# polarsignals/frostdb

Hardware: AMD Instinct MI355X
Metric: rows/sec filter+group-by on 1B-row Prometheus Arrow (HBM-resident); achieved HBM GB/s vs peak (higher is better)
Workload: dtype f64; 1 GPU; headline: Prometheus schema, labels.code=='200' + SUM(value) GROUP BY labels.path; total_rows=1000000000, rows_per_gpu=1000000000, records_per_gpu=40, groups=1025, parallelism=1 GPU

## Files before the change

frostdb_amd/csrc/fdb_dense.cpp:

```cpp
#include "fdb_plan.h"
#include "fdb_jit.h"

#include "fdb_context.h"
#include "fdb_launch_plan.h"
#include "fdb_plan_internal.h"

#include <optional>

namespace fdb {

struct Plan::DenseLaunch {
  Plan& P;
  const DeviceBatch* const* bs;
  std::vector<Resolved>& Rs;
  std::vector<std::vector<int>>& part_gcols;
  const std::vector<int>& live;
  const bool fixed_order;
  PhaseTimer& pt;
  const bool jit_possible;
  const int sub;
  FdbScanArgs& args(int i) { return Rs[(size_t)i].args; }

  std::optional<StageScope> stage_scope;
  LutClasses luts;
  size_t lut_lds_max = 0;

  bool slots_ok = false;
  bool interp_ok = true;
  int two_phase = 0;

  LdsPlan lds;
  FoldFuncs funcs;

  struct Narrowed { int part, k, col; bool late; const void* wide; int64_t saved; const uint8_t* validity; bool folded; };
  std::vector<Narrowed> narrowed;

  hipFunction_t jit_fn = nullptr;
  std::string shape_key;
  int jit_block = 0;
  bool slot_kernel = false;
  int per_cu = 1;
  int tile_rows = 0;

  DenseLaunch(Plan& p, const DeviceBatch* const* b, std::vector<Resolved>& rs, std::vector<std::vector<int>>& gc, const std::vector<int>& lv, bool fixed, PhaseTimer& t)
      : P(p), bs(b), Rs(rs), part_gcols(gc), live(lv), fixed_order(fixed), pt(t), jit_possible(p.jit_possible()), sub(p.sub_tiles == 4 ? 0 : p.sub_tiles) {}

  void bind_group_columns();
  void stage_luts();
  void assign_all_slots();
  void plan_lds();
  bool specialisable() const { return slots_ok && P.sub_tiles != 4 && lds.lds_bytes <= 150 * 1024; }
  void narrow_slots();
  void narrow_pool(bool late);
  void widen_slots();
  bool choose_kernel();
  bool split_by_shape();
  void launch();
  void launch_slots();
  void launch_sequential();
  unsigned long long* alloc_partials(int grid);
  void fold_partials(unsigned long long* partials, int grid);
};

void Plan::DenseLaunch::bind_group_columns() {
  for (int i : live) {
    Resolved& R = Rs[(size_t)i];
    FdbScanArgs& a = R.args;
    for (const GroupRes& gr : R.groups) {
      FdbGroupCol& G = a.gcols[a.n_gcols];
      const DevColumn& c = bs[i]->cols[(size_t)gr.ci];
      G.idx = (const uint32_t*)c.d_values;
      G.validity = c.d_validity;
      const size_t null_entry = scan_cache_folded(*bs[i], (size_t)gr.ci) && gr.lut->size() <= c.dict->values.size() ? 1 : 0;
      G.lut_len = (uint32_t)(gr.lut->size() + null_entry);
      G.lut_lds = FDB_NO_LDS;
      G.slot = -1;
      R.gcol_col[a.n_gcols] = gr.ci;
      const size_t off = R.blob.add(gr.lut->data(), gr.lut->size() * 4);
      R.blob.bytes.resize(R.blob.bytes.size() + null_entry * 4, 0);
      R.luts.push_back(PendingLut{1, a.n_gcols, off, (gr.lut->size() + null_entry) * 4});
      part_gcols[(size_t)i].push_back(gr.gi);
      a.n_gcols++;
    }
  }
  std::vector<uint32_t> caps;
  for (const GroupColState& g : P.gcols_) caps.push_back((uint32_t)g.values.size() + 1);
  P.ensure_layout(caps);
  pt.mark("layout");
}

void Plan::DenseLaunch::stage_luts() {
  for (int i : live) luts.add(Rs[(size_t)i]);
  stage_scope.emplace(P.ctx_);
  unsigned char* d_blob = luts.blob.bytes.empty() ? nullptr : (unsigned char*)P.upload(luts.blob.bytes.data(), luts.blob.bytes.size());
  size_t k = 0;
  for (int i : live) lut_lds_max = std::max(lut_lds_max, luts.place(k++, d_blob, Rs[(size_t)i]));
}

void Plan::DenseLaunch::assign_all_slots() {
  slots_ok = P.rows_per_thread == 0;
  std::vector<int> layouts;
  for (int i : live) {
    Resolved& R = Rs[(size_t)i];
    FdbScanArgs& a = R.args;
    for (int g = 0; g < a.n_gcols; g++) a.gcols[g].stride = P.gcols_[(size_t)part_gcols[(size_t)i][(size_t)g]].stride;
    for (size_t j = 0; j < P.aggs_.size(); j++) a.aggs[j].acc = P.aggs_[j].d_acc;
    a.cnt = P.d_cnt_;
    a.n_slots = P.n_slots_;
    a.need_count = 0;
    for (size_t j = 0; j < P.aggs_.size(); j++) if (a.aggs[j].func == FDB_AGG_COUNT) a.need_count = 1;
    if (slots_ok) {
      bool strict = true;
      const int layout = assign_slots(*bs[i], R, 1, jit_possible, &strict);
      if (layout == 0) slots_ok = false;
      interp_ok = interp_ok && strict;
      layouts.push_back(layout);
    }
  }
  if (!slots_ok) return;
  for (int l : layouts) if (l == 2) two_phase = 1;
  if (two_phase) {
    size_t k = 0;
    for (int i : live)
      if (layouts[k++] == 1 && assign_slots(*bs[i], Rs[(size_t)i], 2, jit_possible) != 2) throw Error(FDB_ERR_INVALID, "internal: slot re-assignment failed");
  }
}

void Plan::DenseLaunch::plan_lds() {
  const size_t acc_bytes = align_up((size_t)P.n_slots_ * 4, 16) + (size_t)P.n_slots_ * 8 * P.aggs_.size();
  lds = fdb::plan_lds(lut_lds_max, acc_bytes, P.aggs_.size(), jit_possible, slots_ok, fixed_order, P.use_partials, P.grid_override,
                      P.grid_override > 0 ? P.grid_override : fdb_scan_default_grid(P.device_));
  if (!lds.refusal.empty()) throw Error(FDB_ERR_UNSUPPORTED, lds.refusal);
  int32_t func[FDB_MAX_AGGS], type[FDB_MAX_AGGS];
  for (size_t j = 0; j < P.aggs_.size(); j++) { func[j] = args(live[0]).aggs[j].func; type[j] = P.aggs_[j].type; }
  funcs = fold_funcs(func, type, P.aggs_.size());
  for (int i : live) { args(i).lds_lut_bytes = (uint32_t)lut_lds_max; args(i).lds_acc = lds.lds_acc; args(i).cache_slots = lds.cache_slots; }
  pt.mark("lut upload");
}

void Plan::DenseLaunch::narrow_slots() {
  if (!specialisable() || !jit_possible) return;
  narrow_pool(false);
  if (two_phase) narrow_pool(true);
}
static bool validity_leaf_reads(const FdbScanArgs& a, int k) {
  for (int l = 0; l < a.n_leaves; l++)
    if (a.leaves[l].kind == FDB_LEAF_VALIDITY && !a.leaves[l].wide && a.leaves[l].slot == k) return true;
  return false;
}
void Plan::DenseLaunch::narrow_pool(bool late) {
  const FdbScanArgs& a0 = args(live[0]);
  const int n4 = late ? a0.n_l4 : a0.n_c4;
  for (int i : live) if ((late ? args(i).n_l4 : args(i).n_c4) != n4) return;
  for (int k = 0; k < n4; k++) {
    int w = 0;
    for (int i : live) {
      const Resolved& R = Rs[(size_t)i];
      const int ci = late ? R.l4_col[k] : R.c4_col[k];
      const int wi = (late ? R.args.l4[k] : R.args.c4[k]).values == nullptr || ci < 0 ? 4 : scan_cache_width(*bs[i], (size_t)ci);
      w = w == 0 || w == wi ? wi : 4;
      if (w == 4) break;
    }
    if (w >= 4) continue;
    for (int i : live) {
      Resolved& R = Rs[(size_t)i];
      const int ci = late ? R.l4_col[k] : R.c4_col[k];
      FdbColSlot& sl = late ? R.args.l4[k] : R.args.c4[k];
      bool counted = false;
      for (const Narrowed& nw : narrowed) if (nw.part == i && nw.col == ci) counted = true;
      const int64_t saved = counted ? 0 : bs[i]->rows * (int64_t)(4 - w);
      const bool fold = sl.validity != nullptr && scan_cache_folded(*bs[i], (size_t)ci) && !(!late && validity_leaf_reads(R.args, k));
      narrowed.push_back(Narrowed{i, k, ci, late, sl.values, saved, sl.validity, fold});
      sl.values = scan_cache_get(*bs[i], (size_t)ci, P.stream_);
      if (fold) sl.validity = nullptr;
      (late ? R.args.wl4 : R.args.w4)[k] = (uint8_t)w;
      R.bytes -= saved;
    }
  }
}
void Plan::DenseLaunch::widen_slots() {
  for (const Narrowed& nw : narrowed) {
    Resolved& R = Rs[(size_t)nw.part];
    (nw.late ? R.args.l4 : R.args.c4)[nw.k].values = nw.wide;
    (nw.late ? R.args.l4 : R.args.c4)[nw.k].validity = nw.validity;
    (nw.late ? R.args.wl4 : R.args.w4)[nw.k] = 0;
    R.bytes += nw.saved;
  }
  narrowed.clear();
}

bool Plan::DenseLaunch::choose_kernel() {
  jit_block = fixed_order ? 256 : sub == 1 ? 512 : sub == 2 ? 256 : sub == 3 ? 1024 : 0;
  if (specialisable()) {
    JitShape shape;
    bool same = true, first = true;
    const FdbScanArgs& args0 = args(live[0]);
    for (int i : live) {
      if (first) { shape = jit_shape(args0, two_phase != 0, jit_block ? jit_block : 256); first = false; }
      else if (!jit_shape_merge_args(&shape, args0, args(i), two_phase != 0)) { same = false; break; }
    }
    if (!same && live.size() > 1 && jit_possible && split_by_shape()) return false;
    {
      int regs_per_slot = 2;
      for (const AggState& A : P.aggs_) if (A.func != FDB_AGG_COUNT || P.final_stage_) regs_per_slot += 2;
      if (P.n_slots_ >= 1 && P.n_slots_ <= 8 && (int)P.n_slots_ * regs_per_slot <= 48) shape.reg_slots = (int)P.n_slots_;
    }
    shape.wave_tables = fixed_order;
    shape.uniform_fold = !P.knobs_.no_uniform_fold;
    if (same) {
      JitDeferScope defer(interp_ok && !fixed_order);
      if (jit_block != 0) { jit_fn = jit_get(shape); if (jit_fn != nullptr) per_cu = jit_blocks_per_cu(jit_fn, jit_block, lds.lds_bytes); }
      else jit_fn = jit_select(shape, lds.lds_bytes, shape.row_bytes(), P.ordered_, &jit_block, &per_cu);
      if (jit_fn != nullptr) tile_rows = jit_block * (shape.quad ? 16 : 4);
      if (pt.on && jit_fn != nullptr) shape_key = shape.key(true);
    }
  }
  if (slots_ok && jit_fn == nullptr) widen_slots();
  slot_kernel = slots_ok && (jit_fn != nullptr || interp_ok);
  if (fixed_order && jit_fn == nullptr) throw Error(FDB_ERR_UNSUPPORTED, "deterministic float sums need the run-time specialised dense kernel (records of one shape, hiprtc available)");
  pt.mark("kernel select");
  if (slot_kernel && jit_fn == nullptr) fdb_slot_geometry(two_phase, sub, lds.lds_acc, lds.lds_bytes, P.device_, &tile_rows, &per_cu);
  return true;
}

bool Plan::DenseLaunch::split_by_shape() {
  std::vector<std::string> keys;
  std::vector<std::vector<const DeviceBatch*>> groups;
  for (int i : live) {
    const std::string k = jit_shape(args(i), two_phase != 0, 256).key(false);
    size_t g = 0;
    for (; g < keys.size(); g++) if (keys[g] == k) break;
    if (g == keys.size()) { keys.push_back(k); groups.emplace_back(); }
    groups[g].push_back(bs[i]);
  }
  if (groups.size() <= 1) return false;
  P.ctx_->defer_staging(false);
  for (auto& g : groups) P.push_batches(g.data(), (int)g.size());
  return true;
}

unsigned long long* Plan::DenseLaunch::alloc_partials(int grid) {
  if (!lds.lds_acc || !P.use_partials || grid <= 0) return nullptr;
  void* p = P.ctx_->dev_alloc((size_t)grid * (1 + P.aggs_.size()) * P.n_slots_ * 8);
  P.scratch_.push_back(p);
  return (unsigned long long*)p;
}

void Plan::DenseLaunch::fold_partials(unsigned long long* partials, int grid) {
  if (partials == nullptr) return;
  unsigned long long* host_out = P.mirror_target();
  hip_check(fdb_launch_reduce_partials(partials, grid, (int)(1 + P.aggs_.size()), P.n_slots_, P.d_state_, P.slots_alloc_, funcs.f, host_out, P.stream_), "reduce partials");
  P.mirror_valid_ = host_out != nullptr;
}

void Plan::DenseLaunch::launch() {
  if (slot_kernel) launch_slots(); else launch_sequential();
  pt.mark("reduce launch");
}

void Plan::DenseLaunch::launch_slots() {
  int grid = P.grid_override > 0 ? P.grid_override : (fdb_scan_default_grid(P.device_) / 2) * per_cu;
  std::vector<FdbScanArgs> parts;
  parts.reserve(live.size());
  for (int i : live) parts.push_back(args(i));
  const int64_t total_tiles = assign_tiles(parts.data(), parts.size(), tile_rows);
  if (grid > total_tiles) grid = (int)total_tiles;
  unsigned long long* partials = alloc_partials(grid);
  for (FdbScanArgs& a : parts) a.partials = partials;
  bool fill_rides = false;
  if (P.state_virgin_ && jit_fn != nullptr && partials != nullptr && (uint64_t)P.slots_alloc_ * (1 + P.aggs_.size()) < (1ull << 32)) {
    FdbScanArgs& a0 = parts[0];
    a0.fill_state = P.d_state_;
    a0.fill_words = (uint32_t)(P.slots_alloc_ * (1 + P.aggs_.size()));
    a0.fill_alloc = (uint32_t)P.slots_alloc_;
    P.state_idents(a0.fill_idents);
    fill_rides = true;
  } else {
    P.materialize_state();
  }
  P.trace("before scan");
  pt.mark("parts build");
  const FdbScanArgs* d_parts = (const FdbScanArgs*)P.upload(parts.data(), parts.size() * sizeof(FdbScanArgs));
  P.ctx_->flush_staging();
  pt.mark("parts upload");
  P.trace("after upload");
  if (pt.on) {
    std::vector<uint32_t> folded(parts.size(), 0u);
    for (const Narrowed& nw : narrowed)
      if (nw.folded) folded[(size_t)(std::find(live.begin(), live.end(), nw.part) - live.begin())] |= 1u << ((nw.late ? 16 : 0) + nw.k);
    print_dense_launch(jit_fn != nullptr ? "fdb_plan_kernel" : "scan_slots_kernel", shape_key, parts.data(), parts.size(), total_tiles, grid, jit_fn != nullptr ? jit_block : 0, lds.lds_bytes,
                       two_phase, lds.lds_acc, lds.cache_slots, lut_lds_max, per_cu, tile_rows, fill_rides, partials != nullptr, folded);
  }
  P.timed([&] {
    if (jit_fn != nullptr) hip_check(jit_launch(jit_fn, d_parts, (int)parts.size(), total_tiles, parts[0], grid, jit_block, lds.lds_bytes, P.stream_), "scan launch");
    else hip_check(fdb_launch_scan_slots(d_parts, (int)parts.size(), parts[0], total_tiles, grid, lds.lds_bytes, two_phase, sub, P.stream_), "scan launch");
  });
  if (fill_rides) P.state_virgin_ = false;
  P.last_kernel_ = jit_fn != nullptr ? "fdb_plan_kernel" : "scan_slots_kernel";
  pt.mark("scan launch");
  P.trace("after scan");
  fold_partials(partials, grid);
  P.trace("after reduce");
  P.stat_launches += 1;
}

void Plan::DenseLaunch::launch_sequential() {
  const int rpt = P.rows_per_thread == 8 ? 8 : 4;
  P.materialize_state();
  P.ctx_->flush_staging();
  for (int i : live) {
    FdbScanArgs& a = args(i);
    if (a.n_expr > 0) throw Error(FDB_ERR_UNSUPPORTED, "computed (projected) columns are not supported by the sequential kernel (too many referenced columns)");
    a.n_c4 = a.n_c8 = 0;
    const int grid = fdb_scan_grid(a, lds.base_grid, rpt);
    a.partials = alloc_partials(grid);
    if (pt.on) print_dense_launch("scan_dense_kernel", "", &a, 1, 0, grid, 0, lds.lds_bytes, 0, lds.lds_acc, lds.cache_slots, lut_lds_max, 0, rpt, false, a.partials != nullptr);
    P.timed([&] { hip_check(fdb_launch_scan_dense(a, grid, lds.lds_bytes, rpt, P.stream_), "scan launch"); });
    P.last_kernel_ = "scan_dense_kernel";
    P.mirror_valid_ = false;
    fold_partials(a.partials, grid);
    P.stat_launches += 1;
  }
}

bool Plan::push_dense(const DeviceBatch* const* bs, std::vector<Resolved>& Rs, std::vector<std::vector<int>>& part_gcols, const std::vector<int>& live, bool fixed_order,
                      PhaseTimer& pt) {
  DenseLaunch D(*this, bs, Rs, part_gcols, live, fixed_order, pt);
  D.bind_group_columns();
  D.stage_luts();
  D.assign_all_slots();
  D.plan_lds();
  D.narrow_slots();
  if (!D.choose_kernel()) return false;
  D.launch();
  return true;
}

}
```

frostdb_amd/csrc/fdb_jit.cpp:

```cpp
#include <hip/hip_runtime_api.h>
#include <hip/hiprtc.h>
#include <sys/stat.h>
#include <unistd.h>

#include <algorithm>
#include <chrono>
#include <atomic>
#include <cstdio>
#include <cstdlib>
#include <cstring>
#include <fstream>
#include <condition_variable>
#include <functional>
#include <memory>
#include <mutex>
#include <thread>
#include <sstream>
#include <string>
#include <unordered_map>
#include <vector>

#include "fdb_jit.h"
#include "../../include/frostdb_amd.h"

// ... 115 lines not shown
    if (!compiled) {
      std::fprintf(stderr, "[frostdb_amd] %s specialisation failed, using the interpreting kernel: %s\n", kernel_name, log.c_str());
      if (std::getenv("FDB_JIT_DEBUG")) std::fprintf(stderr, "%s\n", src.c_str());
      return nullptr;
    }
    if (!path.empty()) {
      const std::string tmp = path + "." + std::to_string((long)getpid());
      bool ok = false;
      {
        std::ofstream f(tmp, std::ios::binary);
        if (f) { f.write(code.data(), (std::streamsize)code.size()); f.close(); ok = !f.fail(); }
      }
      if (!ok || ::rename(tmp.c_str(), path.c_str()) != 0) (void)::unlink(tmp.c_str());
    }
  }
  if (fn == nullptr && !load(&fn)) {
    std::fprintf(stderr, "[frostdb_amd] could not load a specialised %s, using the interpreting kernel\n", kernel_name);
    fn = nullptr;
  }
  publish.fn = fn;
  return fn;
}

thread_local bool t_may_defer = false;
struct Builders {
  struct Slot { std::thread t; std::shared_ptr<std::atomic<bool>> done; };
  std::mutex m;
  std::vector<Slot> slots;
  void spawn(std::function<void()> job) {
    std::lock_guard<std::mutex> lk(m);
    for (size_t k = 0; k < slots.size();) {
      if (slots[k].done->load(std::memory_order_acquire)) { slots[k].t.join(); slots[k] = std::move(slots.back()); slots.pop_back(); }
      else k++;
    }
    auto done = std::make_shared<std::atomic<bool>>(false);
    slots.push_back(Slot{std::thread([job = std::move(job), done] { job(); done->store(true, std::memory_order_release); }), done});
  }
  ~Builders() { for (Slot& s : slots) if (s.t.joinable()) s.t.join(); }
} g_builders;

template <typename F>
hipFunction_t get_kernel(const std::string& key, const char* kernel_name, F make_source) {
  if (g_disabled || std::getenv("FDB_NO_JIT") != nullptr) return nullptr;
  int dev = 0;
  (void)hipGetDevice(&dev);
  const std::string ckey = std::to_string(dev) + "|" + kernel_name + "|" + key;
  std::shared_ptr<KernelEntry> entry;
  bool builder = false;
  {
    std::lock_guard<std::mutex> lk(g_mu);
    auto it = g_cache.find(ckey);
    if (it == g_cache.end()) { entry = std::make_shared<KernelEntry>(); g_cache.emplace(ckey, entry); builder = true; }
    else entry = it->second;
  }
  const char* as = t_may_defer ? std::getenv("FDB_JIT_ASYNC") : nullptr;
  const bool defer = as != nullptr && std::atoi(as) != 0;
  if (!builder) {
    std::unique_lock<std::mutex> lk(entry->m);
    if (defer && !entry->ready) return nullptr;
    entry->cv.wait(lk, [&] { return entry->ready; });
    return entry->fn;
  }
  std::string src;
  try { src = make_source(); }
  catch (...) { { std::lock_guard<std::mutex> lk(entry->m); entry->ready = true; } entry->cv.notify_all(); throw; }
  if (defer) {
    const std::string kn = kernel_name;
    g_builders.spawn([entry, kn, src, dev] { (void)hipSetDevice(dev); (void)build_kernel(entry.get(), kn, src); });
    return nullptr;
  }
  return build_kernel(entry.get(), kernel_name, src);
}
}

hipFunction_t jit_select_kernel_get(const JitShape& shape) {
  return get_kernel("select|" + shape.key() + "|f" + std::to_string(shape.fuse4) + "," + std::to_string(shape.fuse8), "fdb_select_kernel", [&] { return jit_select_source(shape); });
}
hipError_t jit_select_launch(hipFunction_t fn, const FdbScanArgs* d_parts, int n_parts, int64_t total_super_tiles, const FdbScanArgs& common, int grid, size_t lds_bytes,
                             uint32_t* masks, uint32_t* offsets, const FdbSelectArgs& sel, hipStream_t stream) {
  long long tt = total_super_tiles;
  void* args[] = {(void*)&d_parts, (void*)&n_parts, (void*)&tt, (void*)&common, (void*)&masks, (void*)&offsets, (void*)&sel};
  return hipModuleLaunchKernel(fn, (unsigned)grid, 1, 1, (unsigned)jit_select_block(), 1, 1, (unsigned)lds_bytes, stream, args, nullptr);
}

hipFunction_t jit_flags_get(const JitShape& shape) {
  return get_kernel("flags|" + shape.key(), "fdb_flags_kernel", [&] { return jit_flags_source(shape); });
}

hipError_t jit_flags_launch(hipFunction_t fn, const FdbScanArgs* d_parts, int n_parts, int64_t total_super_tiles, const FdbScanArgs& common, int grid, size_t lds_bytes,
                            uint32_t* masks, uint32_t* tile_counts, hipStream_t stream) {
  long long tt = total_super_tiles;
  void* args[] = {(void*)&d_parts, (void*)&n_parts, (void*)&tt, (void*)&common, (void*)&masks, (void*)&tile_counts};
  return hipModuleLaunchKernel(fn, (unsigned)grid, 1, 1, 256u, 1, 1, (unsigned)lds_bytes, stream, args, nullptr);
}

hipFunction_t jit_project_get(const JitShape& shape) {
  std::string roots;
  for (int r : shape.proj_roots) roots += std::to_string(r) + ",";
  return get_kernel("project|" + shape.key() + "|r" + roots, "fdb_project_kernel", [&] { return jit_project_source(shape); });
}
hipError_t jit_project_launch(hipFunction_t fn, const FdbScanArgs* d_parts, int n_parts, int64_t total_tiles, int grid, size_t lds_bytes, const FdbProjectPart* d_outs,
                              unsigned long long* d_nulls, hipStream_t stream) {
  long long tt = total_tiles;
  void* args[] = {(void*)&d_parts, (void*)&n_parts, (void*)&tt, (void*)&d_outs, (void*)&d_nulls};
  return hipModuleLaunchKernel(fn, (unsigned)grid, 1, 1, 256u, 1, 1, (unsigned)lds_bytes, stream, args, nullptr);
}

void jit_stats(int64_t* n_compiled, double* compile_ms, int64_t* n_disk_loads) {
  if (n_compiled) *n_compiled = g_stat_compiled.load();
  if (compile_ms) *compile_ms = (double)g_stat_compile_us.load() / 1000.0;
  if (n_disk_loads) *n_disk_loads = g_stat_disk_loads.load();
}

JitDeferScope::JitDeferScope(bool may_defer) : prev_(t_may_defer) { t_may_defer = may_defer; }
JitDeferScope::~JitDeferScope() { t_may_defer = prev_; }

hipFunction_t jit_get(const JitShape& shape) {
  return get_kernel(shape.key(), "fdb_plan_kernel", [&] { return jit_source(shape); });
}

hipFunction_t jit_hash_get(const JitHashShape& shape) {
  return get_kernel(shape.key(), "fdb_hash_kernel", [&] { return jit_hash_source(shape); });
}

hipError_t jit_hash_launch(hipFunction_t fn, const FdbHashArgs& args, int grid, size_t lds_bytes, hipStream_t stream) {
  void* kargs[] = {(void*)&args};
  return hipModuleLaunchKernel(fn, (unsigned)grid, 1, 1, 256, 1, 1, (unsigned)lds_bytes, stream, kargs, nullptr);
}

hipFunction_t jit_select(JitShape shape, size_t lds_bytes, int row_bytes, bool sorted_input, int* block_out, int* blocks_per_cu_out) {
  int waves = row_bytes > 0 ? (65536 / (64 * 4)) / row_bytes : 16;
  waves = std::max(8, std::min(32, waves));
  if (shape.quad) waves = std::max(8, std::min(16, row_bytes > 0 ? (sorted_input ? 144 : 96) / row_bytes : 8));
  const int block = shape.quad ? 256 : waves % 8 == 0 ? 512 : 256;
  shape.block = block;
  hipFunction_t fn = jit_get(shape);
  if (fn == nullptr) return nullptr;
  const int fit = jit_blocks_per_cu(fn, block, lds_bytes);
  *block_out = block;
  *blocks_per_cu_out = std::max(1, std::min(fit, (waves + block / 128) / (block / 64)));
  if (std::getenv("FDB_JIT_DEBUG"))
    std::fprintf(stderr, "[frostdb_amd] plan kernel %s: %d B/row, %zu B LDS -> %d-thread workgroups, %d per CU (%d fit)\n", shape.key().c_str(), row_bytes,
                 lds_bytes, block, *blocks_per_cu_out, fit);
  return fn;
}

hipError_t jit_launch(hipFunction_t fn, const FdbScanArgs* d_parts, int n_parts, int64_t total_tiles, const FdbScanArgs& common, int grid, int block,
                      size_t lds_bytes, hipStream_t stream) {
  long long tt = total_tiles;
  void* args[] = {(void*)&d_parts, (void*)&n_parts, (void*)&tt, (void*)&common};
  return hipModuleLaunchKernel(fn, (unsigned)grid, 1, 1, (unsigned)block, 1, 1, (unsigned)lds_bytes, stream, args, nullptr);
}

}
```

frostdb_amd/csrc/fdb_jit.h:

```cpp
#pragma once
#include <cstdlib>

#include <hip/hip_runtime_api.h>

#include <cstdint>
#include <string>
#include <vector>

#include "fdb_kernels.h"

namespace fdb {

struct JitSlot { bool has_values = false; int has_validity = 0; int width = 4; };
struct JitLeaf { int kind = 0, slot = -1, wide = 0, op = 0; bool lut_in_lds = false; };
struct JitGroup { int slot = -1; bool lut_in_lds = false; };
struct JitAgg { int func = 0, type = 0, slot = -1; int expr = 0; };
struct JitExprNode { int kind = 0, op = 0, left = -1, right = -1, slot = -1, type = 0; };

struct JitShape {
  int block = 512;
  bool lds_acc = true, need_count = false, two_phase = false;
  int n_c4 = 0, n_c8 = 0, n_l4 = 0, n_l8 = 0;
  JitSlot c4[FDB_ARG_C4], c8[FDB_ARG_C8], l4[FDB_ARG_L4], l8[FDB_ARG_L8];
  std::vector<JitLeaf> leaves;
  std::vector<uint8_t> code;
  std::vector<JitGroup> gcols;
  std::vector<JitAgg> aggs;
  std::vector<JitExprNode> exprs;
  int reg_slots = 0;
  bool cache = false;
  bool wave_tables = false;
  bool uniform_fold = true;
  bool quad = false;
  int fuse4 = 0, fuse8 = 0;
  std::vector<int> proj_roots;
  std::string key(bool with_validity = true) const;
  int row_bytes() const {
    int b = 0;
    for (int k = 0; k < n_c4; k++) b += c4[k].has_values ? c4[k].width : 0;
    for (int k = 0; k < n_l4; k++) b += l4[k].has_values ? l4[k].width : 0;
    for (int k = 0; k < n_c8; k++) b += c8[k].has_values ? 8 : 0;
    for (int k = 0; k < n_l8; k++) b += l8[k].has_values ? 8 : 0;
    return b;
  }
};

struct JitHashCol { int kind = 0; bool has_validity = false, lut_in_lds = false; int expr_root = -1; bool lut_identity = false; };
struct JitHashShape {
  std::vector<JitHashCol> cols;
  std::vector<JitLeaf> leaves;
  std::vector<bool> leaf_validity;
  std::vector<uint8_t> code;
  std::vector<JitAgg> aggs;
  std::vector<bool> agg_validity;
  std::vector<JitExprNode> exprs;
  int n_expr_cols = 0;
  bool need_count = true;
  int runs = 0;
  bool exact = false;
  std::string key() const;
};
JitHashShape jit_hash_shape(const FdbHashArgs& args, const FdbHashCol* hcols);
std::string jit_hash_source(const JitHashShape& shape);
hipFunction_t jit_hash_get(const JitHashShape& shape);
hipError_t jit_hash_launch(hipFunction_t fn, const FdbHashArgs& args, int grid, size_t lds_bytes, hipStream_t stream);

JitShape jit_shape(const FdbScanArgs& a, bool two_phase, int block);
bool jit_shape_merge(JitShape* into, const JitShape& other);
bool jit_shape_merge_args(JitShape* into, const FdbScanArgs& a, const FdbScanArgs& b, bool two_phase);
int jit_blocks_per_cu(hipFunction_t fn, int block, size_t lds_bytes);

void jit_stats(int64_t* n_compiled, double* compile_ms, int64_t* n_disk_loads);

std::string jit_flags_source(const JitShape& shape);
hipFunction_t jit_flags_get(const JitShape& shape);
hipError_t jit_flags_launch(hipFunction_t fn, const FdbScanArgs* d_parts, int n_parts, int64_t total_super_tiles, const FdbScanArgs& common, int grid, size_t lds_bytes,
                            uint32_t* masks, uint32_t* tile_counts, hipStream_t stream);

std::string jit_select_source(const JitShape& shape);
hipFunction_t jit_select_kernel_get(const JitShape& shape);
size_t jit_select_stage_bytes(const JitShape& shape);
int jit_select_block();
hipError_t jit_select_launch(hipFunction_t fn, const FdbScanArgs* d_parts, int n_parts, int64_t total_super_tiles, const FdbScanArgs& common, int grid, size_t lds_bytes,
                             uint32_t* masks, uint32_t* offsets, const FdbSelectArgs& sel, hipStream_t stream);

std::string jit_project_source(const JitShape& shape);
hipFunction_t jit_project_get(const JitShape& shape);
hipError_t jit_project_launch(hipFunction_t fn, const FdbScanArgs* d_parts, int n_parts, int64_t total_tiles, int grid, size_t lds_bytes, const FdbProjectPart* d_outs,
                              unsigned long long* d_nulls, hipStream_t stream);

std::string jit_source(const JitShape& shape);
class JitDeferScope {
 public:
  explicit JitDeferScope(bool may_defer);
  ~JitDeferScope();
  JitDeferScope(const JitDeferScope&) = delete;
  JitDeferScope& operator=(const JitDeferScope&) = delete;
 private:
  bool prev_;
};
hipFunction_t jit_get(const JitShape& shape);
hipFunction_t jit_select(JitShape shape, size_t lds_bytes, int row_bytes, bool sorted_input, int* block_out, int* blocks_per_cu_out);
hipError_t jit_launch(hipFunction_t fn, const FdbScanArgs* d_parts, int n_parts, int64_t total_tiles, const FdbScanArgs& common, int grid, int block,
                      size_t lds_bytes, hipStream_t stream);

}
```

frostdb_amd/csrc/fdb_jitgen.cpp:

```cpp
#include <algorithm>
#include <cstring>
#include <functional>
#include <sstream>
#include <string>
#include <vector>

#include "fdb_jit.h"
#include "../../include/frostdb_amd.h"

namespace fdb {

namespace {

const char* kPreamble = R"HIP(
typedef uint32_t u32x4 __attribute__((ext_vector_type(4)));
typedef unsigned long long u64x2 __attribute__((ext_vector_type(2)));
typedef uint32_t u32x2 __attribute__((ext_vector_type(2)));
#define G1 __attribute__((address_space(1)))
template <typename T> __device__ __forceinline__ const G1 T* as_global(const T* p) { return (const G1 T*)p; }
__device__ __forceinline__ long long f64_to_ordered(double d) { long long b = __double_as_longlong(d); return b ^ ((b >> 63) & 0x7FFFFFFFFFFFFFFFLL); }
// (a NaN contributes the identity of MIN / MAX, −0.0 counts as +0.0: see f64_minmax_key in fdb_kernels.hip)
__device__ __forceinline__ long long f64_minmax_key(double d, bool is_min) {
  d += 0.0;
  const long long k = f64_to_ordered(d);
  return d != d ? (is_min ? 0x7FFFFFFFFFFFFFFFLL : (-0x7FFFFFFFFFFFFFFFLL - 1)) : k;
}
// (FDB_LD_TEMPORAL: the kernel reads its columns twice — wide run records — so the first pass must leave them in the L2)
#ifdef FDB_LD_TEMPORAL
__device__ __forceinline__ u32x4 ld4(const void* base, uint32_t byte_off) {
  return *as_global(reinterpret_cast<const u32x4*>(reinterpret_cast<const char*>(base) + byte_off));
}
__device__ __forceinline__ u64x2 ld8(const void* base, uint32_t byte_off) {
  return *as_global(reinterpret_cast<const u64x2*>(reinterpret_cast<const char*>(base) + byte_off));
}
// (narrow-index caches, fdb_record.h: a lane's four indices at 1 / 2 bytes each — one 4- / 8-byte load, contiguous across the wave)
__device__ __forceinline__ uint32_t ld1raw(const void* base, uint32_t byte_off) {
  return *as_global(reinterpret_cast<const uint32_t*>(reinterpret_cast<const char*>(base) + byte_off));
}
__device__ __forceinline__ u32x2 ld2raw(const void* base, uint32_t byte_off) {
  return *as_global(reinterpret_cast<const u32x2*>(reinterpret_cast<const char*>(base) + byte_off));
}
#else
__device__ __forceinline__ uint32_t ld1raw(const void* base, uint32_t byte_off) {
  return __builtin_nontemporal_load(as_global(reinterpret_cast<const uint32_t*>(reinterpret_cast<const char*>(base) + byte_off)));
}
__device__ __forceinline__ u32x2 ld2raw(const void* base, uint32_t byte_off) {
  return __builtin_nontemporal_load(as_global(reinterpret_cast<const u32x2*>(reinterpret_cast<const char*>(base) + byte_off)));
}
__device__ __forceinline__ u32x4 ld4(const void* base, uint32_t byte_off) {
  return __builtin_nontemporal_load(as_global(reinterpret_cast<const u32x4*>(reinterpret_cast<const char*>(base) + byte_off)));
}
__device__ __forceinline__ u64x2 ld8(const void* base, uint32_t byte_off) {
  return __builtin_nontemporal_load(as_global(reinterpret_cast<const u64x2*>(reinterpret_cast<const char*>(base) + byte_off)));
}
#endif
// … unpacked into the register form the rest of the kernel consumes
__device__ __forceinline__ u32x4 ld1x4(const void* base, uint32_t byte_off) {
  const uint32_t v = ld1raw(base, byte_off);
  u32x4 r; r.x = v & 0xFFu; r.y = (v >> 8) & 0xFFu; r.z = (v >> 16) & 0xFFu; r.w = v >> 24;
  return r;
}
__device__ __forceinline__ u32x4 ld2x4(const void* base, uint32_t byte_off) {
  const u32x2 v = ld2raw(base, byte_off);
  u32x4 r; r.x = v.x & 0xFFFFu; r.y = v.x >> 16; r.z = v.y & 0xFFFFu; r.w = v.y >> 16;
  return r;
}
__device__ __forceinline__ uint32_t ldv(const uint8_t* bm, uint32_t byte_off, uint32_t shift) { return (as_global(bm)[byte_off] >> shift) & 0xFu; }
// dictionary truth table in a 64-bit immediate: 4 rows → 4-bit mask (NULL rows look up entry `null_at`)
__device__ __forceinline__ uint32_t leaf_bits(u32x4 idx, uint32_t valid, unsigned long long bits, uint32_t null_at) {
  const uint32_t i0 = (valid & 1u) ? idx.x : null_at, i1 = (valid & 2u) ? idx.y : null_at, i2 = (valid & 4u) ? idx.z : null_at, i3 = (valid & 8u) ? idx.w : null_at;
  return (uint32_t)((bits >> i0) & 1ull) | ((uint32_t)((bits >> i1) & 1ull) << 1) | ((uint32_t)((bits >> i2) & 1ull) << 2) | ((uint32_t)((bits >> i3) & 1ull) << 3);
}
template <typename LUT>
__device__ __forceinline__ uint32_t leaf_lut(u32x4 idx, uint32_t valid, LUT lut, uint32_t null_at) {
  const uint32_t i0 = (valid & 1u) ? idx.x : null_at, i1 = (valid & 2u) ? idx.y : null_at, i2 = (valid & 4u) ? idx.z : null_at, i3 = (valid & 8u) ? idx.w : null_at;
  return (uint32_t)lut[i0] | ((uint32_t)lut[i1] << 1) | ((uint32_t)lut[i2] << 2) | ((uint32_t)lut[i3] << 3);
}
// pre-aggregate arithmetic (project.go:163-399): Go int64 semantics — wrap-around, quotient truncated toward zero,
// MinInt64 / -1 wraps; a division by zero yields NULL, whose raw slot reads 0.
__device__ __forceinline__ long long i64_add(long long a, long long b) { return (long long)((unsigned long long)a + (unsigned long long)b); }
__device__ __forceinline__ long long i64_sub(long long a, long long b) { return (long long)((unsigned long long)a - (unsigned long long)b); }
__device__ __forceinline__ long long i64_mul(long long a, long long b) { return (long long)((unsigned long long)a * (unsigned long long)b); }
__device__ __forceinline__ long long i64_div(long long a, long long b) { return b == 0 ? 0 : b == -1 ? (long long)(0ull - (unsigned long long)a) : a / b; }
__device__ __forceinline__ long long u64_div(long long a, long long b) { return b == 0 ? 0 : (long long)((unsigned long long)a / (unsigned long long)b); }  // DivUint64s (project.go:379-395)
__device__ __forceinline__ double f64_div(double a, double b) { return b == 0.0 ? 0.0 : a / b; }
template <int OP, typename T> __device__ __forceinline__ bool cmp1(T a, T b) {
  return OP == 1 ? a == b : OP == 2 ? a != b : OP == 3 ? a < b : OP == 4 ? a <= b : OP == 5 ? a > b : a >= b;
}
template <int OP, typename T> __device__ __forceinline__ uint32_t cmp4(T a, T b, T c, T d, T lit, uint32_t valid) {
  return ((uint32_t)cmp1<OP, T>(a, lit) | ((uint32_t)cmp1<OP, T>(b, lit) << 1) | ((uint32_t)cmp1<OP, T>(c, lit) << 2) | ((uint32_t)cmp1<OP, T>(d, lit) << 3)) & valid;
}
)HIP";

const char* kQuadPreamble = R"HIP(
__device__ __forceinline__ u32x4 ldblock(const void* base, uint32_t byte_off) {
#ifdef FDB_LD_TEMPORAL
  return *as_global(reinterpret_cast<const u32x4*>(reinterpret_cast<const char*>(base) + byte_off));
#else
  return __builtin_nontemporal_load(as_global(reinterpret_cast<const u32x4*>(reinterpret_cast<const char*>(base) + byte_off)));
#endif
}
__device__ __forceinline__ uint32_t dword_of(u32x4 q, int k) { return k == 0 ? q.x : k == 1 ? q.y : k == 2 ? q.z : q.w; }
__device__ __forceinline__ u32x4 idx1x4(uint32_t v) {
  u32x4 r; r.x = v & 0xFFu; r.y = (v >> 8) & 0xFFu; r.z = (v >> 16) & 0xFFu; r.w = v >> 24;
  return r;
}
__device__ __forceinline__ u32x4 idx2x4(uint32_t lo, uint32_t hi) {
  u32x4 r; r.x = lo & 0xFFFFu; r.y = lo >> 16; r.z = hi & 0xFFFFu; r.w = hi >> 16;
  return r;
}
)HIP";

template <typename F, typename V>
std::string expr_valid(const std::vector<JitExprNode>& ex, int root, F col, V colvalid);
template <typename F, typename V>
std::string expr_value(const std::vector<JitExprNode>& ex, int ni, F col, V colvalid) {
  const JitExprNode& n = ex[(size_t)ni];
  const bool f = n.type == FDB_T_F64;
  if (n.kind == 0) return f ? ("__longlong_as_double((long long)" + col(ni) + ")") : ("(long long)" + col(ni));
  if (n.kind == 1) return f ? ("__longlong_as_double(K_elit" + std::to_string(ni) + ")") : ("K_elit" + std::to_string(ni));
  if (n.kind == 7) return "(long long)" + col(ni);
  if (n.kind == 4) return "(double)(" + expr_value(ex, n.left, col, colvalid) + ")";
  if (n.kind == 5) return "(" + colvalid(n.left) + " ? 0ll : 1ll)";
  if (n.kind == 6)
    return "((" + expr_value(ex, n.op, col, colvalid) + " != 0ll) ? " + expr_value(ex, n.left, col, colvalid) + " : " + expr_value(ex, n.right, col, colvalid) + ")";
  std::string a = expr_value(ex, n.left, col, colvalid), b = expr_value(ex, n.right, col, colvalid);
  if (n.kind == 3) {
    if (n.op == FDB_OP_AND || n.op == FDB_OP_OR) return "((" + a + (n.op == FDB_OP_AND ? " & " : " | ") + b + ") & 1ll)";
    if (ex[(size_t)n.left].type != ex[(size_t)n.right].type) { a = "(double)" + a; b = "(double)" + b; }
    const char* op = n.op == FDB_OP_EQ ? " == " : n.op == FDB_OP_NOT_EQ ? " != " : n.op == FDB_OP_LT ? " < " : n.op == FDB_OP_LT_EQ ? " <= " : n.op == FDB_OP_GT ? " > " : " >= ";
    return "((" + expr_valid(ex, n.left, col, colvalid) + " && " + expr_valid(ex, n.right, col, colvalid) + " && (" + a + op + b + ")) ? 1ll : 0ll)";
  }
  if (f) {
    if (n.op == FDB_OP_DIV) return "f64_div(" + a + ", " + b + ")";
    return "(" + a + (n.op == FDB_OP_ADD ? " + " : n.op == FDB_OP_SUB ? " - " : " * ") + b + ")";
  }
  return std::string(n.op == FDB_OP_ADD ? "i64_add(" : n.op == FDB_OP_SUB ? "i64_sub(" : n.op == FDB_OP_MUL ? "i64_mul(" : n.type == FDB_T_U64 ? "u64_div(" : "i64_div(") + a + ", " + b + ")";
}
template <typename F, typename V>
std::string expr_valid(const std::vector<JitExprNode>& ex, int root, F col, V colvalid) {
  const JitExprNode& n = ex[(size_t)root];
  if (n.kind == 0) return colvalid(root);
  if (n.kind == 2 && n.op == FDB_OP_DIV) {
    const std::string d = expr_value(ex, n.right, col, colvalid);
    return n.type == FDB_T_F64 ? ("(" + d + " != 0.0)") : ("(" + d + " != 0)");
  }
  return "true";
}
inline std::string expr_bits(const std::vector<JitExprNode>& ex, int root, const std::string& v) {
  if (ex[(size_t)root].type == FDB_T_BOOL) return "(unsigned long long)(" + v + " + 1ll)";
  return ex[(size_t)root].type == FDB_T_F64 ? ("(unsigned long long)__double_as_longlong(" + v + ")") : ("(unsigned long long)" + v);
}

inline std::string comp8(const std::string& r, int k) { return r + (k < 2 ? "a" : "b") + (k % 2 == 0 ? ".x" : ".y"); }

struct RowRefs {
  const std::vector<JitExprNode>& ex;
  int k;
  std::function<std::string(int)> reg8;
  std::string col(int ni) const {
    const JitExprNode& n = ex[(size_t)ni];
    return n.kind == 7 ? "((PM" + std::to_string(n.slot) + " >> " + std::to_string(k) + ") & 1u)" : comp8(reg8(n.slot), k);
  }
  std::string colvalid(int ni) const { return "((" + reg8(ex[(size_t)ni].slot) + "_m >> " + std::to_string(k) + ") & 1u)"; }
  std::string bits(int root) const {
    return expr_bits(ex, root, expr_value(ex, root, [&](int ni) { return col(ni); }, [&](int ni) { return colvalid(ni); }));
  }
  std::string valid(int root) const { return expr_valid(ex, root, [&](int ni) { return col(ni); }, [&](int ni) { return colvalid(ni); }); }
  std::string raw(int root) const { return "(" + valid(root) + " ? " + bits(root) + " : 0ull)"; }
};

struct AggCode {
  const bool sum, f64, is_min;
  explicit AggCode(const JitAgg& A) : sum(A.func == FDB_AGG_SUM), f64(A.type == FDB_T_F64), is_min(A.func == FDB_AGG_MIN) {}
  bool sum_f64() const { return sum && f64; }
  const char* ctype() const { return sum_f64() ? "double" : sum ? "unsigned long long" : "long long"; }
  const char* ident() const { return sum_f64() ? "0.0" : sum ? "0ull" : is_min ? "0x7FFFFFFFFFFFFFFFLL" : "(-0x7FFFFFFFFFFFFFFFLL - 1)"; }
  const char* ident_word() const { return sum ? "0ull" : is_min ? "0x7FFFFFFFFFFFFFFFull" : "0x8000000000000000ull"; }
  std::string from_word(const std::string& w) const { return sum_f64() ? "__longlong_as_double((long long)" + w + ")" : sum ? w : "(long long)" + w; }
  std::string to_word(const std::string& v) const { return sum_f64() ? "(unsigned long long)__double_as_longlong(" + v + ")" : sum ? v : "(unsigned long long)" + v; }
  std::string typed(const std::string& raw) const {
    return !sum && f64 ? "f64_minmax_key(__longlong_as_double((long long)" + raw + "), " + (is_min ? "true" : "false") + ")" : from_word(raw);
  }
  std::string fold(const std::string& acc, const std::string& y) const {
    return sum ? acc + " += " + y + ";" : acc + " = " + y + (is_min ? " < " : " > ") + acc + " ? " + y + " : " + acc + ";";
  }
  std::string fold_of(const std::string& acc, const std::string& y) const { return sum ? fold(acc, y) : "{ const long long y = " + y + "; " + fold(acc, "y") + " }"; }
  std::string fold_if(const std::string& acc, const std::string& on, const std::string& y) const {
    return sum ? acc + " += " + on + " ? " + y + " : " + ident() + ";" : acc + " = (" + on + " && " + y + (is_min ? " < " : " > ") + acc + ") ? " + y + " : " + acc + ";";
  }
  std::string shuffle_fold(const std::string& v) const {
    return fold_of(v, sum && !f64 ? "(unsigned long long)__shfl_xor((long long)" + v + ", sh, 64)" : "__shfl_xor(" + v + ", sh, 64)");
  }
  std::string atomic(const std::string& where, const std::string& v) const {
    return sum_f64() ? "atomicAdd(reinterpret_cast<double*>" + where + ", " + v + ");" : sum ? "atomicAdd(" + where + ", " + v + ");"
                     : std::string(is_min ? "atomicMin" : "atomicMax") + "(reinterpret_cast<long long*>" + where + ", " + v + ");";
  }
};

struct Gen {
  std::ostringstream o;
  const JitShape& s;
  explicit Gen(const JitShape& sh) : s(sh) {}

  static std::string reg(bool wide, bool late, int slot) { return std::string(late ? "l" : "e") + (wide ? "8_" : "4_") + std::to_string(slot); }

  bool full_block = false;
  void block_loads() {
    auto narrow = [&](const JitSlot& c, const std::string& r) {
      if (!c.has_values || c.width >= 4) return;
      if (c.width == 1) o << "      const u32x4 Q_" << r << " = ldblock(P_" << r << "_v + (size_t)wb, lane * 16u);\n";
      else o << "      const u32x4 Q_" << r << "a = ldblock(P_" << r << "_v + (size_t)wb * 2, lane * 16u), Q_" << r << "b = ldblock(P_" << r << "_v + (size_t)wb * 2 + 1024, lane * 16u);\n";
    };
    for (int i = 0; i < s.n_c4; i++) narrow(s.c4[i], reg(false, false, i));
    for (int i = 0; i < s.n_l4; i++) narrow(s.l4[i], reg(false, true, i));
    for (int i = 0; i < s.n_c4; i++) {
      const std::string r = reg(false, false, i);
      if (s.c4[i].has_values && s.c4[i].width >= 4) o << "      u32x4 A_" << r << "[4];\n";
      if (s.c4[i].has_validity != 0) o << "      uint32_t M_" << r << "[4];\n";
    }
    for (int i = 0; i < s.n_c8; i++) {
      const std::string r = reg(true, false, i);
      if (s.c8[i].has_values) o << "      u64x2 A_" << r << "a[4], A_" << r << "b[4];\n";
      if (s.c8[i].has_validity != 0) o << "      uint32_t M_" << r << "[4];\n";
    }
    o << "#pragma unroll\n      for (int u = 0; u < 4; u++) {\n        const size_t o0 = (size_t)(wb + 256 * u); (void)o0;\n";
    auto valid = [&](const JitSlot& c, const std::string& r) {
      if (c.has_validity == 1) o << "        M_" << r << "[u] = ldv(P_" << r << "_b + (o0 >> 3), lane_offb, lane_shb);\n";
      else if (c.has_validity == 2) o << "        M_" << r << "[u] = P_" << r << "_b != nullptr ? ldv(P_" << r << "_b + (o0 >> 3), lane_offb, lane_shb) : 0xFu;\n";
    };
    for (int i = 0; i < s.n_c4; i++) {
      const std::string r = reg(false, false, i);
      if (s.c4[i].has_values && s.c4[i].width >= 4) o << "        A_" << r << "[u] = ld4(P_" << r << "_v + o0 * 4, lane_off4);\n";
      valid(s.c4[i], r);
    }
    for (int i = 0; i < s.n_c8; i++) {
      const std::string r = reg(true, false, i);
      if (s.c8[i].has_values) o << "        A_" << r << "a[u] = ld8(P_" << r << "_v + o0 * 8, lane_off8);\n        A_" << r << "b[u] = ld8(P_" << r << "_v + o0 * 8, lane_off8 + 16u);\n";
      valid(s.c8[i], r);
    }
    o << "      }\n";
    std::string keep;
    auto use = [&](const std::string& v) { keep += (keep.empty() ? "\"v\"(" : ", \"v\"(") + v + ")"; };
    for (int i = 0; i < s.n_c4; i++) {
      const std::string r = reg(false, false, i);
      if (s.c4[i].has_values && s.c4[i].width >= 4) use("A_" + r + "[0]");
      if (s.c4[i].has_validity != 0) use("M_" + r + "[0]");
    }
    for (int i = 0; i < s.n_c8; i++) {
      const std::string r = reg(true, false, i);
      if (s.c8[i].has_values) { use("A_" + r + "a[0]"); use("A_" + r + "b[0]"); }
      if (s.c8[i].has_validity != 0) use("M_" + r + "[0]");
    }
    if (!keep.empty()) o << "      asm volatile(\"\" :: " << keep << ");\n";
  }

  void loads(bool late) {
    const int n4 = late ? s.n_l4 : s.n_c4, n8 = late ? s.n_l8 : s.n_c8;
    for (int i = 0; i < n4; i++) {
      const JitSlot& c = late ? s.l4[i] : s.c4[i];
      const std::string r = reg(false, late, i);
      if (full_block && c.has_values && c.width == 1) o << "    const u32x4 " << r << " = idx1x4(dword_of(Q_" << r << ", u));\n";
      else if (full_block && c.has_values && c.width == 2)
        o << "    const u32x4 " << r << " = idx2x4(dword_of(u < 2 ? Q_" << r << "a : Q_" << r << "b, 2 * (u & 1)), dword_of(u < 2 ? Q_" << r << "a : Q_" << r << "b, 2 * (u & 1) + 1));\n";
      else if (full_block && !late && c.has_values) o << "    const u32x4 " << r << " = A_" << r << "[u];\n";
      else if (c.has_values && c.width == 1) o << "    const u32x4 " << r << " = ld1x4(P_" << r << "_v + tile_off1, lane_off1);\n";
      else if (c.has_values && c.width == 2) o << "    const u32x4 " << r << " = ld2x4(P_" << r << "_v + tile_off2, lane_off2);\n";
      else if (c.has_values) o << "    const u32x4 " << r << " = ld4(P_" << r << "_v + tile_off4, lane_off4);\n";
      mask(c, r, late);
    }
    for (int i = 0; i < n8; i++) {
      const JitSlot& c = late ? s.l8[i] : s.c8[i];
      const std::string r = reg(true, late, i);
      if (full_block && !late && c.has_values) {
        o << "    const u64x2 " << r << "a = A_" << r << "a[u], " << r << "b = A_" << r << "b[u];\n";
      } else if (c.has_values) {
        o << "    const u64x2 " << r << "a = ld8(P_" << r << "_v + tile_off8, lane_off8);\n";
        o << "    const u64x2 " << r << "b = ld8(P_" << r << "_v + tile_off8, lane_off8 + 16u);\n";
      }
      mask(c, r, late);
    }
  }

  bool live_mask = false;
  void mask(const JitSlot& c, const std::string& r, bool late = false) {
    if (full_block && !late && c.has_validity != 0) { o << "    const uint32_t " << r << "_m = M_" << r << "[u];\n"; return; }
    const char* all = live_mask ? "live" : "0xFu";
    const char* cut = live_mask ? " & live" : "";
    if (c.has_validity == 1) o << "    const uint32_t " << r << "_m = ldv(P_" << r << "_b + tile_offb, lane_offb, lane_shb)" << cut << ";\n";
    else if (c.has_validity == 2) o << "    const uint32_t " << r << "_m = P_" << r << "_b != nullptr ? ldv(P_" << r << "_b + tile_offb, lane_offb, lane_shb)" << cut << " : " << all << ";\n";
    else o << "    const uint32_t " << r << "_m = " << all << ";\n";
  }

  std::string leaf_expr(int l) { return leaf_expr_of(s.leaves[l], l, reg(s.leaves[l].wide, false, s.leaves[l].slot)); }

  static std::string leaf_expr_of(const JitLeaf& L, int l, const std::string& r) {
    const std::string li = std::to_string(l);
    std::ostringstream e;
    switch (L.kind) {
      case FDB_LEAF_CONST: e << "(K_op" << li << " ? 0xFu : 0u)"; break;
      case FDB_LEAF_VALIDITY: e << "(K_op" << li << " ? " << r << "_m : (~" << r << "_m & 0xFu))"; break;
      case FDB_LEAF_DICT_BITS: e << "leaf_bits(" << r << ", " << r << "_m, (unsigned long long)K_lit" << li << ", K_len" << li << " - 1u)"; break;
      case FDB_LEAF_DICT_LUT:
        if (L.lut_in_lds) e << "leaf_lut(" << r << ", " << r << "_m, smem + K_lds" << li << ", K_len" << li << " - 1u)";
        else e << "leaf_lut(" << r << ", " << r << "_m, as_global(K_lut" << li << "), K_len" << li << " - 1u)";
        break;
      case FDB_LEAF_CMP_I64:
        e << "cmp4<" << L.op << ", long long>((long long)" << r << "a.x, (long long)" << r << "a.y, (long long)" << r << "b.x, (long long)" << r << "b.y, K_lit" << li << ", " << r << "_m)";
        break;
      case FDB_LEAF_CMP_U64:
        e << "cmp4<" << L.op << ", unsigned long long>(" << r << "a.x, " << r << "a.y, " << r << "b.x, " << r << "b.y, (unsigned long long)K_lit" << li << ", " << r << "_m)";
        break;
      case FDB_LEAF_CMP_F64:
        e << "cmp4<" << L.op << ", double>(__longlong_as_double((long long)" << r << "a.x), __longlong_as_double((long long)" << r << "a.y), __longlong_as_double((long long)"
          << r << "b.x), __longlong_as_double((long long)" << r << "b.y), __longlong_as_double(K_lit" << li << "), " << r << "_m)";
        break;
      case FDB_LEAF_CMP_I64_F64:
        e << "cmp4<" << L.op << ", double>((double)(long long)" << r << "a.x, (double)(long long)" << r << "a.y, (double)(long long)" << r << "b.x, (double)(long long)" << r
          << "b.y, __longlong_as_double(K_lit" << li << "), " << r << "_m)";
        break;
    }
    return e.str();
  }

  std::string filter_expr() {
    return filter_expr_of(s.code, [&](int l) { return leaf_expr(l); });
  }
  template <typename F>
  static std::string filter_expr_of(const std::vector<uint8_t>& code, F leaf) {
    std::vector<std::string> st;
    for (uint8_t c : code) {
      if (c < 0x80) { st.push_back(leaf(c)); continue; }
      const std::string b = st.back(); st.pop_back();
      const std::string a = st.back(); st.pop_back();
      st.push_back("(" + a + (c == FDB_CODE_AND ? " & " : " | ") + b + ")");
    }
    return st.empty() ? "0xFu" : st.back();
  }

  RowRefs row(int k, bool late) const { return {s.exprs, k, [late](int slot) { return reg(true, late, slot); }}; }
  template <typename F> void each_agg(F f) const {
    for (size_t j = 0; j < s.aggs.size(); j++) if (s.aggs[j].func != FDB_AGG_COUNT) f(j, AggCode(s.aggs[j]));
  }

  template <typename R>
  static void match_bits(std::ostringstream& o, const std::vector<JitExprNode>& exprs, const std::vector<JitLeaf>& leaves, R leaf_reg) {
    std::vector<int> seen;
    for (const JitExprNode& e : exprs)
      if (e.kind == 7 && std::find(seen.begin(), seen.end(), e.slot) == seen.end()) {
        seen.push_back(e.slot);
        o << "    const uint32_t PM" << e.slot << " = " << leaf_expr_of(leaves[(size_t)e.slot], e.slot, leaf_reg(e.slot)) << "; (void)PM" << e.slot << ";\n";
      }
  }

  struct Entry {
    bool late_pools;
    const char* var;
    int block;
    bool out_tile;
  };
  template <typename F> void each_slot(const Entry& e, F f) const {
    for (bool late : {false, true}) {
      if (late && !e.late_pools) break;
      const int n4 = late ? s.n_l4 : s.n_c4, n8 = late ? s.n_l8 : s.n_c8;
      for (int i = 0; i < n4; i++) f(reg(false, late, i), late ? "l4" : "c4", i);
      for (int i = 0; i < n8; i++) f(reg(true, late, i), late ? "l8" : "c8", i);
    }
  }
  void entry_decls(const Entry& e, const std::function<void()>& more = nullptr) {
    each_slot(e, [&](const std::string& r, const char*, int) { o << "  const char* P_" << r << "_v = nullptr; const uint8_t* P_" << r << "_b = nullptr;\n"; });
    for (size_t l = 0; l < s.leaves.size(); l++)
      o << "  long long K_lit" << l << " = 0; uint32_t K_len" << l << " = 1, K_lds" << l << " = 0; int K_op" << l << " = 0; const uint8_t* K_lut" << l << " = nullptr;\n";
    if (more) more();
    o << "  long long n_rows = 0, tile_begin = 0, tile_end = 0" << (e.out_tile ? ", out_tile = 0" : "") << "; int part = -1, lut_class = -1;\n";
  }
  void enter_record(const Entry& e, const std::function<void()>& per_record = nullptr, const std::function<void()>& luts = nullptr, const std::string& leaving = "") {
    o << "    if (part < 0 || " << e.var << " >= tile_end) {\n" << leaving;
    o << "      int np = part < 0 ? 0 : part;\n      while (np + 1 < n_parts && " << e.var << " >= parts[np].tile_end) np++;\n      part = np;\n";
    o << "      const FdbScanArgs& pa = parts[part];\n      n_rows = pa.n_rows; tile_begin = pa.tile_begin; tile_end = pa.tile_end;" << (e.out_tile ? " out_tile = pa.out_tile_base;" : "") << "\n";
    each_slot(e, [&](const std::string& r, const char* pool, int i) {
      o << "      P_" << r << "_v = (const char*)pa." << pool << "[" << i << "].values; P_" << r << "_b = pa." << pool << "[" << i << "].validity;\n";
    });
    for (size_t l = 0; l < s.leaves.size(); l++)
      o << "      K_lit" << l << " = pa.leaves[" << l << "].lit; K_len" << l << " = pa.leaves[" << l << "].lut_len; K_lds" << l << " = pa.leaves[" << l << "].lut_lds; K_op" << l
        << " = pa.leaves[" << l << "].op; K_lut" << l << " = pa.leaves[" << l << "].lut;\n";
    if (per_record) per_record();
    o << "      if (pa.lut_class != lut_class) {\n        lut_class = pa.lut_class;\n        __syncthreads();\n";
    for (size_t l = 0; l < s.leaves.size(); l++)
      if (s.leaves[l].kind == FDB_LEAF_DICT_LUT && s.leaves[l].lut_in_lds)
        o << "        for (uint32_t i = tid; i < K_len" << l << "; i += " << e.block << ") smem[K_lds" << l << " + i] = as_global(K_lut" << l << ")[i];\n";
    if (luts) luts();
    o << "        __syncthreads();\n      }\n    }\n";
  }

  std::string source() {
    const int BLK = s.block;
    const Entry entry{true, "tile", BLK, false};
    o << "#include \"fdb_kernels.h\"\n" << kPreamble;
    if (s.quad) o << kQuadPreamble;
    o << "extern \"C\" __global__ __launch_bounds__(" << BLK << ") void fdb_plan_kernel(const FdbScanArgs* __restrict__ parts, const int n_parts, const long long total_tiles, const FdbScanArgs c) {\n";
    o << "  extern __shared__ __align__(16) unsigned char smem[];\n  const uint32_t tid = threadIdx.x;\n  const uint32_t n_slots = c.n_slots;\n";
    o << "  if (c.fill_state != nullptr)  // (a fresh table: its identity fill rides on this launch, see FdbScanArgs)\n";
    o << "    for (uint32_t i = blockIdx.x * " << BLK << "u + tid; i < c.fill_words; i += gridDim.x * " << BLK << "u) c.fill_state[i] = c.fill_idents[i / c.fill_alloc];\n";
    table_setup();
    entry_decls(entry, [&] {
      for (size_t g = 0; g < s.gcols.size(); g++) o << "  uint32_t G_lds" << g << " = 0, G_stride" << g << " = 0; const uint32_t* G_lut" << g << " = nullptr;\n";
      for (size_t i = 0; i < s.exprs.size(); i++) if (s.exprs[i].kind == 1) o << "  long long K_elit" << i << " = 0;\n";
      for (int t = 0; t < s.reg_slots; t++) {
        o << "  unsigned long long R_cnt" << t << " = 0ull;\n";
        each_agg([&](size_t j, const AggCode& A) { o << "  " << A.ctype() << " R_a" << j << "_" << t << " = " << A.ident() << ";\n"; });
      }
    });
    if (s.quad) {
      o << "  const uint32_t lane = tid & 63u, wave = (uint32_t)__builtin_amdgcn_readfirstlane((int)(tid >> 6));\n";
      o << "  const uint32_t lane_off4 = lane * 16u, lane_off8 = lane * 32u, lane_offb = lane >> 1, lane_shb = (lane & 1u) * 4u; (void)lane_off4;\n";
      o << "  const uint32_t lane_off1 = lane * 4u, lane_off2 = lane * 8u; (void)lane_off1; (void)lane_off2;\n";
    } else {
      o << "  const uint32_t lane_off4 = tid * 16u, lane_off8 = tid * 32u, lane_offb = tid >> 1, lane_shb = (tid & 1u) * 4u;\n";
      o << "  const uint32_t lane_off1 = tid * 4u, lane_off2 = tid * 8u; (void)lane_off1; (void)lane_off2;\n";
    }
    o << "  for (long long tile = blockIdx.x; tile < total_tiles; tile += gridDim.x) {\n";
    enter_record(entry, [&] {
      for (size_t g = 0; g < s.gcols.size(); g++)
        o << "      G_lds" << g << " = pa.gcols[" << g << "].lut_lds; G_stride" << g << " = pa.gcols[" << g << "].stride; G_lut" << g << " = pa.gcols[" << g << "].lut;\n";
      for (size_t i = 0; i < s.exprs.size(); i++) if (s.exprs[i].kind == 1) o << "      K_elit" << i << " = pa.expr[" << i << "].lit;\n";
    }, [&] {
      for (size_t g = 0; g < s.gcols.size(); g++)
        if (s.gcols[g].lut_in_lds)
          o << "        for (uint32_t i = tid; i < pa.gcols[" << g << "].lut_len; i += " << BLK << ") reinterpret_cast<uint32_t*>(smem + G_lds" << g << ")[i] = as_global(G_lut" << g << ")[i];\n";
    });
    if (!s.quad) {
      tile_header("(tile - tile_begin) * " + std::to_string(BLK * 4) + "LL", "tid");
      live_mask = true;
      tile_body();
    } else {
      o << "    const long long wb = (tile - tile_begin) * " << BLK * 16 << "LL + (long long)wave * 1024;\n";
      o << "    if (wb + 1024 <= n_rows) {\n";
      full_block = true; live_mask = false;
      block_loads();
      o << "#pragma unroll\n      for (int u = 0; u < 4; u++) {\n";
      tile_header("wb + 256 * u", nullptr);
      tile_body();
      o << "      }\n    } else {\n";
      full_block = false; live_mask = true;
      o << "#pragma unroll 1\n      for (int u = 0; u < 4; u++) {\n";
      tile_header("wb + 256 * u", "lane");
      tile_body();
      o << "      }\n    }\n";
    }
    o << "  }\n";
    if (s.reg_slots > 0) wave_reduction();
    if (s.cache) cache_flush();
    if (s.lds_acc) lds_flush();
    o << "}\n";
    return o.str();
  }

  void table_setup() {
    o << "  const size_t TB = (((size_t)n_slots * 4 + 15) & ~(size_t)15) + (size_t)n_slots * 8 * (size_t)c.n_aggs;\n  (void)TB;\n";
    const std::string tbl = s.wave_tables ? "smem + c.lds_lut_bytes + (size_t)(tid >> 6) * TB" : "smem + c.lds_lut_bytes";
    o << "  uint32_t* l_cnt = reinterpret_cast<uint32_t*>(" << tbl << ");\n";
    o << "  unsigned long long* l_acc = reinterpret_cast<unsigned long long*>(" << tbl << " + (((size_t)n_slots * 4 + 15) & ~(size_t)15));\n";
    if (s.lds_acc) {
      const std::string i0 = s.wave_tables ? "(tid & 63u)" : "tid", step = s.wave_tables ? "64" : std::to_string(s.block);
      o << "  for (uint32_t i = " << i0 << "; i < n_slots; i += " << step << ") l_cnt[i] = 0;\n";
      each_agg([&](size_t j, const AggCode& A) {
        o << "  for (uint32_t i = " << i0 << "; i < n_slots; i += " << step << ") l_acc[(size_t)" << j << " * n_slots + i] = " << A.ident_word() << ";\n";
      });
    }
    if (s.cache) {
      o << "  const uint32_t CS = (uint32_t)c.cache_slots;\n";
      o << "  uint32_t* t_tag = reinterpret_cast<uint32_t*>(smem + c.lds_lut_bytes);\n  uint32_t* t_cnt = t_tag + CS;\n";
      o << "  unsigned long long* t_acc = reinterpret_cast<unsigned long long*>(t_cnt + CS);\n";
      o << "  for (uint32_t i = tid; i < CS; i += " << s.block << ") { t_tag[i] = 0u; t_cnt[i] = 0u; }\n";
      each_agg([&](size_t j, const AggCode& A) { o << "  for (uint32_t i = tid; i < CS; i += " << s.block << ") t_acc[(size_t)" << j << " * CS + i] = " << A.ident_word() << ";\n"; });
    }
  }

  void tile_header(const std::string& r0, const char* lane) {
    o << "    const long long r0 = " << r0 << ";\n";
    if (lane) o << "    const long long left = n_rows - r0 - (long long)" << lane << " * 4;\n    if (left <= 0) continue;\n";
    o << "    const size_t tile_off4 = (size_t)r0 * 4, tile_off8 = (size_t)r0 * 8, tile_offb = (size_t)(r0 >> 3);" << (lane ? "" : " (void)tile_off4; (void)tile_off8; (void)tile_offb;") << "\n";
    o << "    const size_t tile_off1 = (size_t)r0, tile_off2 = (size_t)r0 * 2; (void)tile_off1; (void)tile_off2;\n";
    o << "    const uint32_t live = " << (lane ? "left >= 4 ? 0xFu : ((1u << (int)left) - 1u)" : "0xFu") << ";\n";
  }

  std::string raw_input(size_t j, int k) const {
    const JitAgg& A = s.aggs[j];
    if (A.expr != 0) return row(k, s.two_phase).raw(A.expr - 1);
    const std::string r = reg(true, s.two_phase, A.slot);
    return "((" + r + "_m >> " + std::to_string(k) + ") & 1u ? " + comp8(r, k) + " : c.aggs[" + std::to_string(j) + "].null_value)";
  }

  bool uniform_fold() const { return s.uniform_fold && s.lds_acc && !s.cache && s.reg_slots == 0 && !s.wave_tables && !s.two_phase && !s.gcols.empty(); }

  void tile_body() {
    loads(false);
    o << "    uint32_t sel = live;\n";
    if (!s.code.empty()) o << "    sel &= " << filter_expr() << ";\n";
    match_bits(o, s.exprs, s.leaves, [&](int l) { return reg(s.leaves[(size_t)l].wide, false, s.leaves[(size_t)l].slot); });
    if (uniform_fold()) o << "    const unsigned long long has = __ballot(sel != 0u);\n    if (has == 0ull) continue;\n";
    else o << "    if (sel == 0u) continue;\n";
    loads(true);
    o << "    uint32_t gid0 = 0, gid1 = 0, gid2 = 0, gid3 = 0;\n";
    for (size_t g = 0; g < s.gcols.size(); g++) {
      const JitGroup& G = s.gcols[g];
      const std::string r = reg(false, s.two_phase, G.slot);
      const std::string lut = G.lut_in_lds ? ("reinterpret_cast<const uint32_t*>(smem + G_lds" + std::to_string(g) + ")") : ("as_global(G_lut" + std::to_string(g) + ")");
      const char* comp[4] = {"x", "y", "z", "w"};
      for (int k = 0; k < 4; k++)
        o << "    gid" << k << " += ((" << r << "_m >> " << k << ") & 1u ? " << lut << "[" << r << "." << comp[k] << "] : 0u) * G_stride" << g << ";\n";
    }
    if (uniform_fold()) fold_uniform();
    if (s.reg_slots > 0) fold_registers();
    else fold_rows();
  }

  void fold_uniform() {
    o << "    {\n      const uint32_t my_first = (sel & 1u) ? gid0 : (sel & 2u) ? gid1 : (sel & 4u) ? gid2 : gid3;\n";
    o << "      const uint32_t g0 = (uint32_t)__builtin_amdgcn_readlane((int)my_first, __builtin_ctzll(has));\n";
    o << "      if (__ballot(sel != 0u && my_first != g0) == 0ull && __ballot(1) == ~0ull &&\n";
    o << "          __ballot(((sel & 1u) && gid0 != g0) || ((sel & 2u) && gid1 != g0) || ((sel & 4u) && gid2 != g0) || ((sel & 8u) && gid3 != g0)) == 0ull) {\n";
    o << "        uint32_t u_cnt = (uint32_t)__builtin_popcount(sel);\n";
    each_agg([&](size_t j, const AggCode& A) {
      const std::string v = "u" + std::to_string(j);
      o << "        " << A.ctype() << " " << v << " = " << A.ident() << ";\n";
      for (int k = 0; k < 4; k++) o << "        if ((sel >> " << k << ") & 1u) " << A.fold_of(v, A.typed(raw_input(j, k))) << "\n";
    });
    o << "#pragma unroll\n        for (int sh = 32; sh > 0; sh >>= 1) {\n          u_cnt += (uint32_t)__shfl_xor((int)u_cnt, sh, 64);\n";
    each_agg([&](size_t j, const AggCode& A) { o << "          " << A.shuffle_fold("u" + std::to_string(j)) << "\n"; });
    o << "        }\n        if ((tid & 63u) == 0u) {\n";
    if (s.need_count) o << "          atomicAdd(&l_cnt[g0], u_cnt);\n";
    else o << "          l_cnt[g0] = 1u;\n";
    each_agg([&](size_t j, const AggCode& A) { o << "          " << A.atomic("(l_acc + (size_t)" + std::to_string(j) + " * n_slots + g0)", "u" + std::to_string(j)) << "\n"; });
    o << "        }\n        continue;\n      }\n    }\n";
  }

  void fold_registers() {
    for (int k = 0; k < 4; k++) {
      o << "    {\n      const bool on = (sel >> " << k << ") & 1u;\n";
      each_agg([&](size_t j, const AggCode& A) { o << "      const " << A.ctype() << " v" << j << " = " << A.typed(raw_input(j, k)) << ";\n"; });
      for (int t = 0; t < s.reg_slots; t++) {
        const std::string m = s.reg_slots == 1 ? std::string("on") : ("(on && gid" + std::to_string(k) + " == " + std::to_string(t) + "u)");
        o << "      R_cnt" << t << " += " << m << " ? 1ull : 0ull;\n";
        each_agg([&](size_t j, const AggCode& A) { o << "      " << A.fold_if("R_a" + std::to_string(j) + "_" + std::to_string(t), m, "v" + std::to_string(j)) << "\n"; });
      }
      o << "    }\n";
    }
  }

  void fold_rows() {
    for (int k = 0; k < 4; k++) {
      const std::string gidk = "gid" + std::to_string(k);
      o << "    if ((sel >> " << k << ") & 1u) {\n";
      if (s.cache) {
        o << "      const uint32_t ch = ((gid" << k << " * 0x9E3779B1u) >> 12) & (CS - 1u);\n";
        o << "      uint32_t tg = t_tag[ch];\n      if (tg == 0u) { tg = atomicCAS(&t_tag[ch], 0u, gid" << k << " + 1u); if (tg == 0u) tg = gid" << k << " + 1u; }\n";
        o << "      const bool cached = tg == gid" << k << " + 1u;\n";
        o << "      if (cached) atomicAdd(&t_cnt[ch], 1u);\n";
        if (s.need_count) o << "      else atomicAdd(&c.cnt[gid" << k << "], 1ull);\n";
        else o << "      else c.cnt[gid" << k << "] = 1ull;\n";
      } else if (s.lds_acc) {
        if (s.need_count) o << "      atomicAdd(&l_cnt[" << gidk << "], 1u);\n";
        else o << "      l_cnt[" << gidk << "] = 1u;\n";
      } else {
        o << "      atomicAdd(&c.cnt[gid" << k << "], 1ull);\n";
      }
      each_agg([&](size_t j, const AggCode& A) {
        const std::string v = A.typed(raw_input(j, k));
        const std::string gacc = "(c.aggs[" + std::to_string(j) + "].acc + gid" + std::to_string(k) + ")";
        if (s.cache) {
          o << "      if (cached) {\n        " << A.atomic("(t_acc + (size_t)" + std::to_string(j) + " * CS + ch)", v) << "\n      } else {\n        " << A.atomic(gacc, v) << "\n      }\n";
        } else {
          o << "      " << A.atomic(s.lds_acc ? "(l_acc + (size_t)" + std::to_string(j) + " * n_slots + " + gidk + ")" : gacc, v) << "\n";
        }
      });
      o << "    }\n";
    }
  }

  void wave_reduction() {
    o << "  for (int sh = 32; sh > 0; sh >>= 1) {\n";
// ... 559 lines not shown
      o << "        }\n";
      for (size_t c = c0; c < c1; c++) {
        const JitHashCol& C = s.cols[c];
        const std::string r = "w" + std::to_string(c);
        o << "        " << (in_quad[c] ? "if (!canon) " : "") << "{\n          const int W = hc[" << c << "].word;\n";
        if (C.kind == 0) {
          for (int k = 0; k < 4; k++) o << "          if (ins_mask & " << (1 << k) << "u) d_" << k << "[W] = i" << c << "_" << k << ";\n";
        } else if (C.kind == 1) {
          for (int k = 0; k < 4; k++)
            o << "          if (ins_mask & " << (1 << k) << "u) { const unsigned long long y = ((" << r << "_m >> " << k << ") & 1u) ? " << comp8(r, k) << " : 0ull; d_" << k << "[W] = (uint32_t)y; d_" << k
              << "[W + 1] = (uint32_t)(y >> 32); }\n";
        } else {
          for (int k = 0; k < 4; k++)
            o << "          if (ins_mask & " << (1 << k) << "u) { const unsigned long long y = " << row(k).valid(C.expr_root) << " ? " << row(k).bits(C.expr_root) << " : 0ull; d_" << k << "[W] = (uint32_t)y; d_" << k
              << "[W + 1] = (uint32_t)(y >> 32); }\n";
        }
        o << "        }\n";
      }
      o << "        asm volatile(\"\" ::: \"memory\");\n      }\n";
    }
    if (for_runs) {
      int used = 4;
      for (size_t c = 0; c < s.cols.size(); c++) used += s.cols[c].kind == 0 ? 1 : 2;
      if (used % 4 != 0) {
        o << "      if (canon) {\n";
        for (int k = 0; k < 4; k++) {
          o << "        if (ins_mask & " << (1 << k) << "u) {";
          for (int w = used; w < ((used + 3) & ~3); w++) o << " d_" << k << "[" << w << "] = 0u;";
          o << " }\n";
        }
        o << "      }\n";
      }
      for (int k = 0; k < 4; k++)
        o << "      if (ins_mask & " << (1 << k) << "u) *reinterpret_cast<u64x2*>(d_" << k << " + h.key_words) = u64x2{cnt_" << k << ", " << run_value(k) << "};\n";
    }
    o << "    }\n";
    };
    if (wide || medium) {
      o << "    {\n      const unsigned long long act2 = __ballot(1);\n      const int wl2 = (int)(tid & 63u), wv = (int)(tid >> 6), first2 = __builtin_ctzll(act2);\n";
      o << "      const unsigned long long b0 = __ballot((sel & 1u) != 0u), b1 = __ballot((sel & 2u) != 0u), b2 = __ballot((sel & 4u) != 0u), b3 = __ballot((sel & 8u) != 0u);\n";
      o << "      const uint32_t n_w = (uint32_t)(__popcll(b0) + __popcll(b1) + __popcll(b2) + __popcll(b3));\n";
      o << "      if (n_w != 0u) {\n        const unsigned long long lt = (1ull << wl2) - 1ull;\n";
      o << "        const uint32_t before = (uint32_t)(__popcll(b0 & lt) + __popcll(b1 & lt) + __popcll(b2 & lt) + __popcll(b3 & lt));\n";
      o << "        uint32_t rb = s_runs[wv * 4], rp = s_runs[wv * 4 + 1], ps = s_runs[wv * 4 + 2];\n";
      o << "        const uint32_t RW = " << (medium ? std::to_string(FDB_RUN_MEDIUM_BYTES / 4) + "u" : std::string("(uint32_t)h.runs.run_words")) << ", RQ = RW >> 2, CAP = (uint32_t)h.runs.stage_cap;\n";
      o << "        u32x4* stage = reinterpret_cast<u32x4*>(smem + a.lds_lut_bytes + (size_t)wv * " << FDB_RUN_WAVE_LDS << ");\n";
      o << "        const uint32_t n_act = (uint32_t)__popcll(act2), my_act = (uint32_t)__popcll(act2 & lt);\n";
      o << "        const bool sw = rp + n_w > " << FDB_RUN_CHUNK << "u, direct = n_w > CAP;\n";
      o << "        if (sw || direct || (rp - ps) + n_w > CAP) {\n";
      o << "          u32x4* out = reinterpret_cast<u32x4*>(h.runs.tuples) + (size_t)(rb + ps) * RQ;\n";
      o << "          for (uint32_t q = my_act; q < (rp - ps) * RQ; q += n_act) out[q] = stage[q];\n";
      o << "          __builtin_amdgcn_wave_barrier();\n          ps = rp;\n        }\n";
      o << "        if (sw) {\n          uint32_t nc = 0u;\n          if (wl2 == first2) nc = atomicAdd(h.runs.chunk_cursor, 1u);\n          rb = (uint32_t)__shfl((int)nc, first2, 64) * " << FDB_RUN_CHUNK
        << "u; rp = 0u; ps = 0u;\n        }\n";
      o << "        const uint32_t base = rb + rp, sbase = rp - ps;\n        __builtin_amdgcn_wave_barrier();\n";
      o << "        if (wl2 == first2) { s_runs[wv * 4] = rb; s_runs[wv * 4 + 1] = rp + n_w; s_runs[wv * 4 + 2] = direct ? rp + n_w : ps; *reinterpret_cast<uint2*>(h.runs.dir + ((size_t)tile * 4 + wv) * 2) = make_uint2(base, n_w); }\n";
      for (int k = 0; k < 4; k++)
        o << "        uint32_t* d_" << k << " = direct ? reinterpret_cast<uint32_t*>(h.runs.tuples) + (size_t)(base + before + (uint32_t)__builtin_popcount(sel & " << ((1 << k) - 1) << "u)) * RW"
          << " : reinterpret_cast<uint32_t*>(stage) + (size_t)(sbase + before + (uint32_t)__builtin_popcount(sel & " << ((1 << k) - 1) << "u)) * RW;\n";
      if (wide) {
        o << "        const uint32_t ins_mask = sel;\n";
        emit_tuple_stores(true);
      } else {
        for (int k = 0; k < 4; k++) {
          o << "        if (sel & " << (1 << k) << "u) {\n          u32x4* d = reinterpret_cast<u32x4*>(d_" << k << ");\n";
          o << "          d[0] = ta_" << k << "; d[1] = tb_" << k << "; d[2] = tc_" << k << "; d[3] = td_" << k << ";\n";
          o << "          *reinterpret_cast<u64x2*>(d + 4) = u64x2{cnt_" << k << ", " << run_value(k) << "};\n        }\n";
        }
      }
      o << "        __builtin_amdgcn_wave_barrier();\n      }\n    }\n    continue;\n";
    }
    if (narrow) {
      o << "    {\n      const unsigned long long act2 = __ballot(1);\n      const int wl2 = (int)(tid & 63u), wv = (int)(tid >> 6), first2 = __builtin_ctzll(act2);\n";
      o << "      const unsigned long long b0 = __ballot((sel & 1u) != 0u), b1 = __ballot((sel & 2u) != 0u), b2 = __ballot((sel & 4u) != 0u), b3 = __ballot((sel & 8u) != 0u);\n";
      o << "      const uint32_t n_w = (uint32_t)(__popcll(b0) + __popcll(b1) + __popcll(b2) + __popcll(b3));\n";
      o << "      if (n_w != 0u) {\n        const unsigned long long lt = (1ull << wl2) - 1ull;\n";
      o << "        const uint32_t before = (uint32_t)(__popcll(b0 & lt) + __popcll(b1 & lt) + __popcll(b2 & lt) + __popcll(b3 & lt));\n";
      o << "        uint32_t rb = s_runs[wv * 4], rp = s_runs[wv * 4 + 1], ps = s_runs[wv * 4 + 2];\n";
      o << "        u32x4* stage = reinterpret_cast<u32x4*>(smem + a.lds_lut_bytes + (size_t)wv * " << FDB_RUN_WAVE_LDS << ");\n";
      o << "        const uint32_t n_act = (uint32_t)__popcll(act2), my_act = (uint32_t)__popcll(act2 & lt);\n";
      o << "        const bool sw = rp + n_w > " << FDB_RUN_CHUNK << "u;\n";
      o << "        if (sw || (rp - ps) + n_w > " << FDB_RUN_STAGE << "u) {\n";
      o << "          u32x4* out = reinterpret_cast<u32x4*>(h.runs.tuples) + (size_t)(rb + ps) * 3;\n";
      o << "          for (uint32_t q = my_act; q < (rp - ps) * 3u; q += n_act) out[q] = stage[q];\n";
      o << "          __builtin_amdgcn_wave_barrier();\n          ps = rp;\n        }\n";
      o << "        if (sw) {\n          uint32_t nc = 0u;\n          if (wl2 == first2) nc = atomicAdd(h.runs.chunk_cursor, 1u);\n          rb = (uint32_t)__shfl((int)nc, first2, 64) * " << FDB_RUN_CHUNK
        << "u; rp = 0u; ps = 0u;\n        }\n";
      o << "        const uint32_t base = rb + rp, sbase = rp - ps;\n        __builtin_amdgcn_wave_barrier();\n";
      o << "        if (wl2 == first2) { s_runs[wv * 4] = rb; s_runs[wv * 4 + 1] = rp + n_w; s_runs[wv * 4 + 2] = ps; *reinterpret_cast<uint2*>(h.runs.dir + ((size_t)tile * 4 + wv) * 2) = make_uint2(base, n_w); }\n";
      for (int k = 0; k < 4; k++) {
        o << "        if (sel & " << (1 << k) << "u) {\n          const uint32_t at = sbase + before + (uint32_t)__builtin_popcount(sel & " << ((1 << k) - 1) << "u);\n";
        o << "          stage[at * 3] = ta_" << k << "; stage[at * 3 + 1] = tb_" << k << ";\n";
        o << "          *reinterpret_cast<u64x2*>(stage + at * 3 + 2) = u64x2{cnt_" << k << ", " << run_value(k) << "};\n        }\n";
      }
      o << "        __builtin_amdgcn_wave_barrier();\n      }\n    }\n    continue;\n";
    }
    for (int k = 0; k < 4; k++) o << "    uint64_t slot_" << k << " = h1_" << k << " & h.mask; unsigned long long p_" << k << " = 0, q_" << k << " = 0;\n";
    for (int k = 0; k < 4; k++)
      o << "    if ((sel >> " << k << ") & 1u) { const u64x2 pq = *as_global(reinterpret_cast<const u64x2*>(h.table + slot_" << k << " * (uint64_t)ew)); p_" << k << " = pq.x; q_" << k
        << " = pq.y; }\n";
    o << "    uint32_t ins_mask = 0;\n";
    for (int k = 0; k < 4; k++) o << "    unsigned long long c_" << k << " = ~0ull;\n";
    for (int k = 0; k < 4; k++)
      o << "    if (((sel >> " << k << ") & 1u) && p_" << k << " == 0ull) c_" << k << " = atomicCAS(h.table + slot_" << k << " * (uint64_t)ew, 0ull, h1_" << k << ");\n";
    for (int k = 0; k < 4; k++)
      o << "    if (c_" << k << " == 0ull) { __hip_atomic_store(h.table + slot_" << k << " * (uint64_t)ew + 1, h2_" << k << ", __ATOMIC_RELAXED, __HIP_MEMORY_SCOPE_AGENT); ins_mask |= " << (1 << k) << "u; }\n";
    for (int k = 0; k < 4; k++) {
      o << "    if ((sel >> " << k << ") & 1u) {\n";
      o << "      if (c_" << k << " != 0ull && !(p_" << k << " == h1_" << k << " && q_" << k << " == h2_" << k << ")) { bool ins; slot_" << k << " = hash_find_or_insert(h.table, h.mask, ew, h1_" << k << ", h2_" << k
        << ", ins); if (ins) ins_mask |= " << (1 << k) << "u; }\n";
      o << "      unsigned long long* e = h.table + slot_" << k << " * (uint64_t)ew;\n";
      if (s.need_count) o << "      atomicAdd(e + 2, cnt_" << k << ");\n";
      for (size_t j : folded)
        if (!exact_agg(j)) o << "      " << agg(j).atomic("(e + " + std::to_string(3 + j) + ")", val(j, k)) << "\n";
      o << "    }\n";
    }
    emit_tuple_stores(false);
    if (s.exact) {
      o << "    x_slot0 = slot_0; x_slot1 = slot_1; x_slot2 = slot_2; x_slot3 = slot_3; x_sel = sel;\n";
      o << "    } while (0);\n";
      for (size_t j = 0; j < s.aggs.size(); j++) {
        if (!exact_agg(j)) continue;
        o << "    {\n      unsigned long long* XL = a.aggs[" << j << "].acc;\n";
        for (int k = 0; k < 4; k++) o << "      fdb_exact_add_wave(XL, x_slot" << k << ", xv" << j << "_" << k << ", ((x_sel >> " << k << ") & 1u) != 0u);\n";
        o << "    }\n";
      }
    }
    o << "  }\n";
    if (wide || medium) {
      o << "  {  // the runs that still wait in the waves' stages\n    const int wv = (int)(tid >> 6), wl2 = (int)(tid & 63u);\n    __builtin_amdgcn_wave_barrier();\n";
      o << "    const uint32_t rb = s_runs[wv * 4], rp = s_runs[wv * 4 + 1], ps = s_runs[wv * 4 + 2], RQ = " << (medium ? std::to_string(FDB_RUN_MEDIUM_BYTES / 16) + "u" : std::string("(uint32_t)h.runs.run_words >> 2")) << ";\n";
      o << "    if (rp != " << FDB_RUN_CHUNK << "u || ps != " << FDB_RUN_CHUNK << "u) {\n";
      o << "      const u32x4* stage = reinterpret_cast<const u32x4*>(smem + a.lds_lut_bytes + (size_t)wv * " << FDB_RUN_WAVE_LDS << ");\n";
      o << "      u32x4* out = reinterpret_cast<u32x4*>(h.runs.tuples) + (size_t)(rb + ps) * RQ;\n";
      o << "      for (uint32_t q = (uint32_t)wl2; q < (rp - ps) * RQ; q += 64u) out[q] = stage[q];\n    }\n  }\n";
    }
    if (narrow) {
      o << "  {  // the runs that still wait in the waves' stages\n    const int wv = (int)(tid >> 6), wl2 = (int)(tid & 63u);\n    __builtin_amdgcn_wave_barrier();\n";
      o << "    const uint32_t rb = s_runs[wv * 4], rp = s_runs[wv * 4 + 1], ps = s_runs[wv * 4 + 2];\n";
      o << "    if (rp != " << FDB_RUN_CHUNK << "u || ps != " << FDB_RUN_CHUNK << "u) {\n";
      o << "      const u32x4* stage = reinterpret_cast<const u32x4*>(smem + a.lds_lut_bytes + (size_t)wv * " << FDB_RUN_WAVE_LDS << ");\n";
      o << "      u32x4* out = reinterpret_cast<u32x4*>(h.runs.tuples) + (size_t)(rb + ps) * 3;\n";
      o << "      for (uint32_t q = (uint32_t)wl2; q < (rp - ps) * 3u; q += 64u) out[q] = stage[q];\n    }\n  }\n";
    }
    o << "  __syncthreads();\n  if (tid == 0 && s_new != 0) atomicAdd(h.n_groups, (unsigned long long)s_new);\n}\n";
    return o.str();
  }
};

}

std::string JitShape::key(bool with_validity) const {
  std::ostringstream k;
  k << "b" << block << "l" << lds_acc << "c" << need_count << "t" << two_phase << "r" << reg_slots << "h" << cache << (wave_tables ? "w" : "") << (uniform_fold ? "u" : "") << (quad ? "q" : "") << "|";
  auto slots = [&](const JitSlot* p, int n) { for (int i = 0; i < n; i++) { k << (p[i].has_values ? 'v' : '-') << (with_validity ? p[i].has_validity : 0); if (p[i].width != 4) k << 'w' << p[i].width; } k << '|'; };
  slots(c4, n_c4); slots(c8, n_c8); slots(l4, n_l4); slots(l8, n_l8);
  for (const JitLeaf& L : leaves) k << L.kind << ',' << L.slot << ',' << L.wide << ',' << (L.kind >= FDB_LEAF_CMP_I64 && L.kind <= FDB_LEAF_CMP_I64_F64 ? L.op : 0) << ',' << L.lut_in_lds << ';';
  k << '|';
  for (uint8_t c : code) k << (int)c << ',';
  k << '|';
  for (const JitGroup& G : gcols) k << G.slot << ',' << G.lut_in_lds << ';';
  k << '|';
  for (const JitAgg& A : aggs) k << A.func << ',' << A.type << ',' << A.slot << ',' << A.expr << ';';
  k << '|';
  for (const JitExprNode& e : exprs) k << e.kind << ',' << e.op << ',' << e.left << ',' << e.right << ',' << e.slot << ',' << e.type << ';';
  return k.str();
}

std::string jit_source(const JitShape& shape) { return Gen(shape).source(); }

JitShape jit_shape(const FdbScanArgs& a, bool two_phase, int block) {
  JitShape s;
  s.block = block;
  s.lds_acc = a.lds_acc != 0;
  s.need_count = a.need_count != 0;
  s.two_phase = two_phase;
  s.n_c4 = a.n_c4; s.n_c8 = a.n_c8;
  s.n_l4 = two_phase ? a.n_l4 : 0; s.n_l8 = two_phase ? a.n_l8 : 0;
  auto slots = [](JitSlot* dst, const FdbColSlot* src, int n) {
    for (int i = 0; i < n; i++) { dst[i].has_values = src[i].values != nullptr; dst[i].has_validity = src[i].validity != nullptr ? 1 : 0; }
  };
  slots(s.c4, a.c4, s.n_c4); slots(s.c8, a.c8, s.n_c8); slots(s.l4, a.l4, s.n_l4); slots(s.l8, a.l8, s.n_l8);
  for (int i = 0; i < s.n_c4; i++) s.c4[i].width = a.w4[i] == 1 || a.w4[i] == 2 ? a.w4[i] : 4;
  for (int i = 0; i < s.n_l4; i++) s.l4[i].width = a.wl4[i] == 1 || a.wl4[i] == 2 ? a.wl4[i] : 4;
  for (int i = 0; i < s.n_c4; i++) s.quad |= s.c4[i].has_values && s.c4[i].width < 4;
  for (int i = 0; i < s.n_l4; i++) s.quad |= s.l4[i].has_values && s.l4[i].width < 4;
  for (int l = 0; l < a.n_leaves; l++) {
    const FdbLeaf& L = a.leaves[l];
    s.leaves.push_back({L.kind, L.slot, L.wide, L.op, L.kind == FDB_LEAF_DICT_LUT && L.lut_lds != FDB_NO_LDS});
  }
  s.code.assign(a.code, a.code + a.n_code);
  for (int g = 0; g < a.n_gcols; g++) s.gcols.push_back({a.gcols[g].slot, a.gcols[g].lut_lds != FDB_NO_LDS});
  for (int j = 0; j < a.n_aggs; j++) s.aggs.push_back({a.aggs[j].func, a.aggs[j].type, a.aggs[j].slot, a.aggs[j].expr});
  for (int i = 0; i < a.n_expr; i++) s.exprs.push_back({a.expr[i].kind, a.expr[i].op, a.expr[i].left, a.expr[i].right, a.expr[i].slot, a.expr[i].type});
  s.cache = !s.lds_acc && a.cache_slots > 0;
  return s;
}

bool jit_shape_merge(JitShape* into, const JitShape& other) {
  if (into->key(false) != other.key(false)) return false;
  auto slots = [](JitSlot* a, const JitSlot* b, int n) { for (int i = 0; i < n; i++) if (a[i].has_validity != b[i].has_validity) a[i].has_validity = 2; };
  slots(into->c4, other.c4, into->n_c4); slots(into->c8, other.c8, into->n_c8); slots(into->l4, other.l4, into->n_l4); slots(into->l8, other.l8, into->n_l8);
  return true;
}

bool jit_shape_merge_args(JitShape* into, const FdbScanArgs& a, const FdbScanArgs& b, bool two_phase) {
  if (a.lds_acc != b.lds_acc || a.need_count != b.need_count || a.n_c4 != b.n_c4 || a.n_c8 != b.n_c8) return false;
  if (two_phase && (a.n_l4 != b.n_l4 || a.n_l8 != b.n_l8)) return false;
  if ((a.lds_acc == 0 && a.cache_slots > 0) != (b.lds_acc == 0 && b.cache_slots > 0)) return false;
  auto values_same = [](const FdbColSlot* x, const FdbColSlot* y, int n) { for (int i = 0; i < n; i++) if ((x[i].values != nullptr) != (y[i].values != nullptr)) return false; return true; };
  if (!values_same(a.c4, b.c4, a.n_c4) || !values_same(a.c8, b.c8, a.n_c8)) return false;
  if (two_phase && (!values_same(a.l4, b.l4, a.n_l4) || !values_same(a.l8, b.l8, a.n_l8))) return false;
  if (std::memcmp(a.w4, b.w4, sizeof a.w4) != 0 || (two_phase && std::memcmp(a.wl4, b.wl4, sizeof a.wl4) != 0)) return false;
  if (a.n_leaves != b.n_leaves || a.n_code != b.n_code || a.n_gcols != b.n_gcols || a.n_aggs != b.n_aggs || a.n_expr != b.n_expr) return false;
  for (int l = 0; l < a.n_leaves; l++) {
    const FdbLeaf& x = a.leaves[l]; const FdbLeaf& y = b.leaves[l];
    if (x.kind != y.kind || x.slot != y.slot || x.wide != y.wide) return false;
    if (x.kind >= FDB_LEAF_CMP_I64 && x.kind <= FDB_LEAF_CMP_I64_F64 && x.op != y.op) return false;
    if ((x.kind == FDB_LEAF_DICT_LUT && x.lut_lds != FDB_NO_LDS) != (y.kind == FDB_LEAF_DICT_LUT && y.lut_lds != FDB_NO_LDS)) return false;
  }
  if (std::memcmp(a.code, b.code, (size_t)a.n_code) != 0) return false;
  for (int g = 0; g < a.n_gcols; g++)
    if (a.gcols[g].slot != b.gcols[g].slot || (a.gcols[g].lut_lds != FDB_NO_LDS) != (b.gcols[g].lut_lds != FDB_NO_LDS)) return false;
  for (int j = 0; j < a.n_aggs; j++)
    if (a.aggs[j].func != b.aggs[j].func || a.aggs[j].type != b.aggs[j].type || a.aggs[j].slot != b.aggs[j].slot || a.aggs[j].expr != b.aggs[j].expr) return false;
  for (int i = 0; i < a.n_expr; i++) {
    const auto& x = a.expr[i]; const auto& y = b.expr[i];
    if (x.kind != y.kind || x.op != y.op || x.left != y.left || x.right != y.right || x.slot != y.slot || x.type != y.type) return false;
  }
  auto merge = [](JitSlot* s, const FdbColSlot* y, int n) { for (int i = 0; i < n; i++) if (s[i].has_validity != (y[i].validity != nullptr ? 1 : 0)) s[i].has_validity = 2; };
  merge(into->c4, b.c4, into->n_c4); merge(into->c8, b.c8, into->n_c8); merge(into->l4, b.l4, into->n_l4); merge(into->l8, b.l8, into->n_l8);
  return true;
}

std::string jit_select_source(const JitShape& shape) { return Gen(shape).select_source(); }
size_t jit_select_stage_bytes(const JitShape& shape) { size_t n = 0; (void)Gen(shape).fused(&n); return n; }
int jit_select_block() { return Gen::kSelectBlock; }

std::string jit_flags_source(const JitShape& shape) { return Gen(shape).flags_source(); }
std::string jit_project_source(const JitShape& shape) { return Gen(shape).project_source(); }

std::string JitHashShape::key() const {
  std::ostringstream k;
  k << "c" << need_count << (runs == 1 ? "R" : runs == 2 ? "W" : runs == 3 ? "M" : "") << (exact ? "X" : "") << "|";
  for (const JitHashCol& C : cols) k << C.kind << (C.has_validity ? 'n' : '-') << (C.lut_identity ? 'i' : C.lut_in_lds ? 'l' : 'g') << (C.kind == 2 ? std::to_string(C.expr_root) : std::string());
  k << '|';
  for (size_t l = 0; l < leaves.size(); l++) {
    const JitLeaf& L = leaves[l];
    k << L.kind << ',' << L.wide << ',' << (L.kind >= FDB_LEAF_CMP_I64 && L.kind <= FDB_LEAF_CMP_I64_F64 ? L.op : 0) << ',' << L.lut_in_lds << ',' << leaf_validity[l] << ';';
  }
  k << '|';
  for (uint8_t c : code) k << (int)c << ',';
  k << '|';
  for (size_t j = 0; j < aggs.size(); j++) k << aggs[j].func << ',' << aggs[j].type << ',' << agg_validity[j] << ',' << aggs[j].expr << ';';
  k << '|' << n_expr_cols << '|';
  for (const JitExprNode& e : exprs) k << e.kind << ',' << e.op << ',' << e.left << ',' << e.right << ',' << e.slot << ',' << e.type << ';';
  return k.str();
}

JitHashShape jit_hash_shape(const FdbHashArgs& h, const FdbHashCol* hcols) {
  JitHashShape s;
  const FdbScanArgs& a = h.base;
  for (int c = 0; c < h.n_hcols; c++)
    s.cols.push_back({hcols[c].kind, hcols[c].validity != nullptr, hcols[c].kind == 0 && hcols[c].lut_lds != FDB_NO_LDS, hcols[c].kind == 2 ? hcols[c].src_word : -1,
                      hcols[c].kind == 0 && hcols[c].lut == nullptr});
  for (int i = 0; i < a.n_expr; i++) s.exprs.push_back({a.expr[i].kind, a.expr[i].op, a.expr[i].left, a.expr[i].right, a.expr[i].slot, a.expr[i].type});
  s.n_expr_cols = a.n_l8;
  s.need_count = a.need_count != 0;
  s.runs = h.runs.tuples == nullptr ? 0 : h.runs.run_words == 0 ? 1 : h.runs.run_words == FDB_RUN_MEDIUM_WORDS ? 3 : 2;
  for (int l = 0; l < a.n_leaves; l++) {
    const FdbLeaf& L = a.leaves[l];
    const bool wide = L.kind >= FDB_LEAF_CMP_I64 && L.kind <= FDB_LEAF_CMP_I64_F64;
    s.leaves.push_back({L.kind, 0, wide ? 1 : 0, L.op, L.kind == FDB_LEAF_DICT_LUT && L.lut_lds != FDB_NO_LDS});
    s.leaf_validity.push_back(L.validity != nullptr);
  }
  s.code.assign(a.code, a.code + a.n_code);
  for (int j = 0; j < a.n_aggs; j++) {
    s.aggs.push_back({a.aggs[j].func, a.aggs[j].type, -1, a.aggs[j].expr});
    s.agg_validity.push_back(a.aggs[j].validity != nullptr);
    if (AggCode(s.aggs.back()).sum_f64() && a.aggs[j].acc != nullptr) s.exact = true;
  }
  return s;
}

std::string jit_hash_source(const JitHashShape& shape) { return HashGen(shape).source(); }

}
```

frostdb_amd/csrc/fdb_launch_plan.h:

```cpp
#pragma once

#include <cstddef>
#include <cstdint>
#include <string>

#include "../../include/frostdb_amd.h"
#include "fdb_kernels.h"

namespace fdb {

struct LdsPlan {
  int lds_acc = 0;
  size_t lds_bytes = 0;
  int cache_slots = 0;
  int base_grid = 0;
  std::string refusal;
};
inline LdsPlan plan_lds(size_t lut_lds_max, size_t acc_bytes, size_t n_aggs, bool jit_possible, bool slots_ok, bool fixed_order, bool use_partials, int grid_override, int base_grid) {
  LdsPlan p;
  p.lds_bytes = lut_lds_max;
  p.base_grid = base_grid;
  if (fixed_order) {
    if (!jit_possible || !slots_ok || !use_partials) { p.refusal = "deterministic float sums need the run-time specialised dense kernel"; return p; }
    if (lut_lds_max + 4 * acc_bytes > 150 * 1024) { p.refusal = "deterministic float sums: four per-wave tables of " + std::to_string(acc_bytes) + " bytes do not fit LDS"; return p; }
    p.lds_acc = 1; p.lds_bytes += 4 * acc_bytes;
  }
  else if (lut_lds_max + acc_bytes <= FDB_LDS_BUDGET) { p.lds_acc = 1; p.lds_bytes += acc_bytes; }
  else if (lut_lds_max + acc_bytes <= 150 * 1024) { p.lds_acc = 1; p.lds_bytes += acc_bytes; if (grid_override <= 0) p.base_grid /= 2; }
  if (!p.lds_acc && jit_possible) {
    const size_t entry = 8 + 8 * n_aggs;
    p.cache_slots = 1;
    while ((size_t)p.cache_slots * 2 * entry <= 48 * 1024) p.cache_slots *= 2;
    p.lds_bytes = lut_lds_max + (size_t)p.cache_slots * entry;
  }
  return p;
}

inline int64_t assign_tiles(FdbScanArgs* parts, size_t n, int64_t tile_rows) {
  int64_t total_tiles = 0;
  for (size_t k = 0; k < n; k++) {
    parts[k].tile_begin = total_tiles;
    total_tiles += (parts[k].n_rows + tile_rows - 1) / tile_rows;
    parts[k].tile_end = total_tiles;
  }
  return total_tiles;
}

struct FoldFuncs { int32_t f[1 + FDB_MAX_AGGS]; };
inline FoldFuncs fold_funcs(const int32_t* func, const int32_t* type, size_t n_aggs) {
  FoldFuncs F = {{0}};
  F.f[0] = 1;
  for (size_t j = 0; j < n_aggs; j++)
    F.f[1 + j] = func[j] == FDB_AGG_COUNT ? 0 : func[j] == FDB_AGG_SUM ? (type[j] == FDB_T_F64 ? 2 : 1) : func[j] == FDB_AGG_MIN ? 3 : 4;
  return F;
}

}
```

frostdb_amd/csrc/fdb_plan.cpp:

```cpp
#include "fdb_plan.h"
#include "fdb_jit.h"

#include "fdb_context.h"
#include "fdb_hostpool.h"
#include "fdb_plan_internal.h"

#include <algorithm>
#include <cstring>
#include <functional>

#include <atomic>
#include <chrono>
#include <cstdio>
#include <cstdlib>

namespace fdb {


void hip_check(hipError_t e, const char* what) {
  if (e != hipSuccess) throw Error(e == hipErrorOutOfMemory ? FDB_ERR_OOM : FDB_ERR_DEVICE, std::string(what) + ": " + hipGetErrorString(e));
}

void copy_stream(void* dst, const void* src, size_t n);
uint32_t copy_stream_max_u32(uint32_t* dst, const uint32_t* src, size_t n);
// ... 553 lines not shown
void Plan::trace(const char* what) {
  if (std::getenv("FDB_PROFILE") == nullptr) return;
  hipEvent_t e = nullptr;
  if (hipEventCreate(&e) != hipSuccess) return;
  if (hipEventRecord(e, stream_) != hipSuccess) { (void)hipEventDestroy(e); return; }
  trace_.emplace_back(what, e);
}

void Plan::collect_timing() {
  if (!trace_.empty()) {
    for (size_t i = 1; i < trace_.size(); i++) {
      float ms = 0;
      if (hipEventElapsedTime(&ms, trace_[i - 1].second, trace_[i].second) == hipSuccess)
        std::fprintf(stderr, "[fdb] stream: %-24s → %-24s %8.1f us\n", trace_[i - 1].first, trace_[i].first, ms * 1e3);
    }
    for (auto& t : trace_) (void)hipEventDestroy(t.second);
    trace_.clear();
  }
  for (auto& p : pending_events_) {
    float ms = 0;
    if (hipEventElapsedTime(&ms, p.first, p.second) == hipSuccess) stat_ms += ms;
    ctx_->put_event(p.first);
    ctx_->put_event(p.second);
  }
  pending_events_.clear();
  for (auto& p : merge_events_) {
    float ms = 0;
    if (hipEventElapsedTime(&ms, p.first, p.second) == hipSuccess) stat_merge_ms += ms;
    ctx_->put_event(p.first);
    ctx_->put_event(p.second);
  }
  merge_events_.clear();
}

void* Plan::upload(const void* host, size_t bytes) { return ctx_->stage(host, bytes); }

const char* Plan::draw() {
  if (draw_.empty()) {
    std::function<std::string(int)> show = [&](int i) -> std::string {
      const ExprNode& e = filter_[(size_t)i];
      if (e.op == FDB_OP_AND) return "(" + show(e.left) + " AND " + show(e.right) + ")";
      if (e.op == FDB_OP_OR) return "(" + show(e.left) + " OR " + show(e.right) + ")";
      if (e.op == FDB_OP_REGEX_MATCH) return e.column + " =~ \"" + e.lit.bytes + "\"";
      if (e.op == FDB_OP_REGEX_NOT_MATCH) return e.column + " !~ \"" + e.lit.bytes + "\"";
      return e.column + " " + op_str(e.op) + " " + e.lit.str();
    };
    std::string s;
    if (filter_root_ >= 0) s += "PredicateFilter (" + show(filter_root_) + ")";
    if (!aggs_.empty() && ordered_) {
      if (!s.empty()) s += " - ";
      s += "OrderedAggregate (" + aggs_[0].column + " by ";
      for (size_t i = 0; i < matchers_.size(); i++) s += (i ? "," : "") + matchers_[i].name;
      s += ")";
    } else if (!aggs_.empty()) {
      if (!s.empty()) s += " - ";
      s += "HashAggregate (";
      for (size_t i = 0, shown = 0; i < aggs_.size(); i++) if (aggs_[i].role != 2) s += (shown++ ? "," : "") + aggs_[i].result_name;
      s += " by ";
      for (size_t i = 0; i < matchers_.size(); i++) s += (i ? "," : "") + matchers_[i].name;
      s += ")";
    } else if (!matchers_.empty()) {
      if (!s.empty()) s += " - ";
      s += "Distinction (";
      for (size_t i = 0; i < matchers_.size(); i++) s += (i ? "," : "") + matchers_[i].name;
      s += ")";
    }
    draw_ = s + (exact_ ? " [gfx950, exact float64 sums]" : " [gfx950]");
  }
  return draw_.c_str();
}

namespace {

typedef std::vector<uint8_t> Truth;

Truth leaf_truth(const ExprNode& e, const HostDict& dict) {
  const size_t n = dict.values.size();
  Truth t(n + 1, 0);
  if (!dict.plain && !e.lit.valid() && (e.op == FDB_OP_EQ || e.op == FDB_OP_NOT_EQ || e.op == FDB_OP_CONTAINS || e.op == FDB_OP_NOT_CONTAINS)) {
    const bool on_value = e.op != FDB_OP_EQ;
    for (size_t i = 0; i < n; i++) t[i] = on_value;
    t[n] = e.op == FDB_OP_EQ;
    return t;
  }
  for (size_t i = 0; i < n; i++) {
    const std::string& v = dict.values[i];
    bool m = false;
    switch (e.op) {
      case FDB_OP_EQ: m = (v == e.lit.bytes); break;
      case FDB_OP_NOT_EQ: m = (v != e.lit.bytes); break;
      case FDB_OP_CONTAINS: m = v.find(e.lit.bytes) != std::string::npos; break;
      case FDB_OP_NOT_CONTAINS: m = v.find(e.lit.bytes) == std::string::npos; break;
      case FDB_OP_LT: m = v.compare(e.lit.bytes) < 0; break;
      case FDB_OP_LT_EQ: m = v.compare(e.lit.bytes) <= 0; break;
      case FDB_OP_GT: m = v.compare(e.lit.bytes) > 0; break;
      case FDB_OP_GT_EQ: m = v.compare(e.lit.bytes) >= 0; break;
      case FDB_OP_REGEX_MATCH: m = e.regex_matches(v); break;
      case FDB_OP_REGEX_NOT_MATCH: m = !e.regex_matches(v); break;
    }
    t[i] = m ? 1 : 0;
  }
  t[n] = 0;
  return t;
}

bool dict_leaf_op(int32_t op) {
  return op == FDB_OP_EQ || op == FDB_OP_NOT_EQ || op == FDB_OP_CONTAINS || op == FDB_OP_NOT_CONTAINS || op == FDB_OP_REGEX_MATCH ||
         op == FDB_OP_REGEX_NOT_MATCH;
}

bool single_dict_subtree(const std::vector<ExprNode>& nodes, int idx, const DeviceBatch& b, int* col, int* n_leaves) {
  const ExprNode& e = nodes[(size_t)idx];
  if (e.op == FDB_OP_AND || e.op == FDB_OP_OR)
    return single_dict_subtree(nodes, e.left, b, col, n_leaves) && single_dict_subtree(nodes, e.right, b, col, n_leaves);
  if (!dict_leaf_op(e.op)) return false;
  const int ci = b.find(e.column);
  if (ci < 0 || b.cols[(size_t)ci].kind != ColKind::DICT || b.cols[(size_t)ci].d_values == nullptr) return false;
  const bool is_regex = e.op == FDB_OP_REGEX_MATCH || e.op == FDB_OP_REGEX_NOT_MATCH;
  const HostDict& d = *b.cols[(size_t)ci].dict;
  if (is_regex && !d.plain && d.utf8()) return false;
  if (d.plain && (e.op == FDB_OP_EQ || e.op == FDB_OP_NOT_EQ) && e.lit.type != FDB_LIT_STRING && e.lit.type != FDB_LIT_BINARY) return false;
  if (*col >= 0 && *col != ci) return false;
  *col = ci;
  (*n_leaves)++;
  return true;
}

Truth subtree_truth(const std::vector<ExprNode>& nodes, int idx, const HostDict& dict) {
  const ExprNode& e = nodes[(size_t)idx];
  if (e.op == FDB_OP_AND || e.op == FDB_OP_OR) {
    Truth l = subtree_truth(nodes, e.left, dict);
    const Truth r = subtree_truth(nodes, e.right, dict);
    for (size_t i = 0; i < l.size(); i++) l[i] = e.op == FDB_OP_AND ? (l[i] & r[i]) : (l[i] | r[i]);
    return l;
  }
  return leaf_truth(e, dict);
}

}

static void resolve_leaf(const ExprNode& e, const DeviceBatch& b, Plan::Resolved* R, FdbLeaf* L);

template <typename F>
static std::shared_ptr<const Truth> cached_truth(Plan::Resolved* R, int node, const std::shared_ptr<HostDict>& dict, F make) {
  if (R->truths != nullptr && node >= 0) {
    std::shared_ptr<const Truth> t = R->truths->find(node, dict.get());
    if (t) return t;
  }
  std::shared_ptr<const Truth> t = std::make_shared<const Truth>(make());
  if (R->truths != nullptr && node >= 0) R->truths->put(node, dict, t);
  return t;
}

static void emit_truth_leaf(const Truth& t, const DeviceBatch& b, int ci, Plan::Resolved* R, FdbLeaf* L) {
  const int li = (int)(L - R->args.leaves);
  const DevColumn& c = b.cols[(size_t)ci];
  L->values = c.d_values;
  L->validity = c.d_validity;
  L->wide = 0;
  L->lut_len = (uint32_t)t.size();
  R->leaf_col[li] = ci;
  R->count(b, ci);
  if (t.size() <= 64) {
    unsigned long long bits = 0;
    for (size_t i = 0; i < t.size(); i++) if (t[i]) bits |= 1ull << i;
    L->kind = FDB_LEAF_DICT_BITS;
    L->lit = (int64_t)bits;
    return;
  }
  L->kind = FDB_LEAF_DICT_LUT;
  const size_t off = R->blob.add(t.data(), t.size());
  R->luts.push_back(PendingLut{0, li, off, t.size()});
}

static void emit_filter(const std::vector<ExprNode>& nodes, int idx, const DeviceBatch& b, Plan::Resolved* R, int depth, int* max_depth) {
  const ExprNode& e = nodes[(size_t)idx];
  FdbScanArgs& a = R->args;
  if (e.op == FDB_OP_AND || e.op == FDB_OP_OR) {
    int col = -1, n_sub = 0;
    if (single_dict_subtree(nodes, idx, b, &col, &n_sub) && n_sub >= 2) {
      if (a.n_leaves >= FDB_MAX_LEAVES || a.n_code >= FDB_MAX_CODE) throw Error(FDB_ERR_UNSUPPORTED, "filter expression too large");
      if (depth + 1 > *max_depth) *max_depth = depth + 1;
      if (*max_depth > 8) throw Error(FDB_ERR_UNSUPPORTED, "filter expression too deep");
      const int li = a.n_leaves++;
      FdbLeaf& L = a.leaves[li];
      std::memset(&L, 0, sizeof(L));
      L.lut_lds = FDB_NO_LDS;
      L.slot = -1;
      const std::shared_ptr<HostDict>& dict = b.cols[(size_t)col].dict;
      emit_truth_leaf(*cached_truth(R, idx, dict, [&] { return subtree_truth(nodes, idx, *dict); }), b, col, R, &L);
      a.code[a.n_code++] = (uint8_t)li;
      return;
    }
    const int leaves0 = a.n_leaves, code0 = a.n_code;
    const size_t luts0 = R->luts.size();
    emit_filter(nodes, e.left, b, R, depth, max_depth);
    try {
      emit_filter(nodes, e.right, b, R, depth + 1, max_depth);
    } catch (const Error& err) {
      if (e.op != FDB_OP_AND || err.code != FDB_ERR_UNSUPPORTED || !R->count_selected || b.rows == 0 || R->count_selected(e.left) != 0) throw;
      a.n_leaves = leaves0; a.n_code = code0;
      R->luts.resize(luts0);
      if (a.n_leaves >= FDB_MAX_LEAVES || a.n_code >= FDB_MAX_CODE) throw Error(FDB_ERR_UNSUPPORTED, "filter expression too large");
      FdbLeaf& L = a.leaves[a.n_leaves];
      std::memset(&L, 0, sizeof(L));
      L.lut_lds = FDB_NO_LDS; L.slot = -1; L.kind = FDB_LEAF_CONST; L.op = 0;
      a.code[a.n_code++] = (uint8_t)a.n_leaves++;
      return;
    }
    if (a.n_code >= FDB_MAX_CODE) throw Error(FDB_ERR_UNSUPPORTED, "filter expression too large");
    a.code[a.n_code++] = e.op == FDB_OP_AND ? FDB_CODE_AND : FDB_CODE_OR;
    return;
  }
  if (a.n_leaves >= FDB_MAX_LEAVES || a.n_code >= FDB_MAX_CODE) throw Error(FDB_ERR_UNSUPPORTED, "filter expression too large");
  if (depth + 1 > *max_depth) *max_depth = depth + 1;
  if (*max_depth > 8) throw Error(FDB_ERR_UNSUPPORTED, "filter expression too deep");
  FdbLeaf L;
  std::memset(&L, 0, sizeof(L));
  L.lut_lds = FDB_NO_LDS;
  L.slot = -1;
  const int li = a.n_leaves;
  a.leaves[li] = L;
  a.n_leaves++;
  R->cur_node = idx;
  resolve_leaf(e, b, R, &a.leaves[li]);
  a.code[a.n_code++] = (uint8_t)li;
}

static void resolve_leaf(const ExprNode& e, const DeviceBatch& b, Plan::Resolved* R, FdbLeaf* L) {
  const int li = (int)(L - R->args.leaves);
  const bool is_regex = e.op == FDB_OP_REGEX_MATCH || e.op == FDB_OP_REGEX_NOT_MATCH;
  const int ci = b.find(e.column);
  auto set_const = [&](bool v) { L->kind = FDB_LEAF_CONST; L->op = v ? 1 : 0; };
  if (ci < 0) {
    if (is_regex) {
      const bool empty_match = e.regex_matches(std::string());
      const bool neg = e.op == FDB_OP_REGEX_NOT_MATCH;
      set_const((neg && !empty_match) || (!neg && empty_match));
      return;
    }
    switch (e.op) {
      case FDB_OP_EQ:
        if (e.lit.valid() && (e.lit.type == FDB_LIT_STRING || e.lit.type == FDB_LIT_BINARY) && !e.lit.bytes.empty()) { set_const(false); return; }
        break;
      case FDB_OP_NOT_EQ:
        if (!e.lit.valid()) { set_const(false); return; }
        break;
      case FDB_OP_LT: case FDB_OP_LT_EQ: case FDB_OP_GT: case FDB_OP_GT_EQ:
        set_const(false);
        return;
    }
    set_const(true);
    return;
  }
  const DevColumn& c = b.cols[(size_t)ci];
  const bool is_contains = e.op == FDB_OP_CONTAINS || e.op == FDB_OP_NOT_CONTAINS;
  if (c.kind == ColKind::DICT && c.dict->plain) {
    if (c.d_values == nullptr && b.rows > 0) throw Error(FDB_ERR_INVALID, "column not staged: " + c.name);
    if (!is_regex && !is_contains) {
      if (!(e.op >= FDB_OP_EQ && e.op <= FDB_OP_GT_EQ)) throw Error(FDB_ERR_UNSUPPORTED, "unsupported binary operation");
      if (!e.lit.valid()) { set_const(false); return; }
      if (e.lit.type != FDB_LIT_STRING && e.lit.type != FDB_LIT_BINARY)
        throw Error(FDB_ERR_UNSUPPORTED, "unsupported binary operation (column/literal type combination) on " + c.name);
    }
    emit_truth_leaf(*cached_truth(R, R->cur_node, c.dict, [&] { return leaf_truth(e, *c.dict); }), b, ci, R, L);
    return;
  }
  if (c.kind == ColKind::DICT) {
    if (c.d_values == nullptr && b.rows > 0) throw Error(FDB_ERR_INVALID, "column not staged: " + c.name);
    if (is_regex && c.dict->utf8())
      throw Error(FDB_ERR_UNSUPPORTED, "ArrayScalarRegexMatch: unsupported dictionary type: *array.String");
    if (!is_regex && !is_contains && e.op != FDB_OP_EQ && e.op != FDB_OP_NOT_EQ)
      throw Error(FDB_ERR_UNSUPPORTED, std::string("unsupported operator: ") + op_str(e.op));
    L->values = c.d_values;
    L->validity = c.d_validity;
    L->wide = 0;
    R->leaf_col[li] = ci;
    if (!is_regex && !e.lit.valid()) {
      if (c.d_validity == nullptr) { R->leaf_col[li] = -1; set_const(e.op != FDB_OP_EQ); return; }
      L->kind = FDB_LEAF_VALIDITY;
      L->op = (e.op == FDB_OP_EQ) ? 0 : 1;
      R->count(b, ci, false);
      return;
    }
    emit_truth_leaf(*cached_truth(R, R->cur_node, c.dict, [&] { return leaf_truth(e, *c.dict); }), b, ci, R, L);
    return;
  }
  if (is_regex) throw Error(FDB_ERR_UNSUPPORTED, "ArrayScalarRegexMatch: unsupported type on the device path: " + c.format);
  if (is_contains) throw Error(FDB_ERR_UNSUPPORTED, "contains on a non-dictionary column is not supported on the device path: " + c.name);
  if (!(e.op >= FDB_OP_EQ && e.op <= FDB_OP_GT_EQ)) throw Error(FDB_ERR_UNSUPPORTED, "unsupported binary operation");
  if (c.kind != ColKind::I64 && c.kind != ColKind::U64 && c.kind != ColKind::F64 && c.kind != ColKind::BOOL)
    throw Error(FDB_ERR_UNSUPPORTED, "unsupported binary operation: compare on column type " + c.format + " (" + c.name + ")");
  if (c.d_values == nullptr && b.rows > 0) throw Error(FDB_ERR_INVALID, "column not staged: " + c.name);
  if (!e.lit.valid()) { set_const(false); return; }
  R->count(b, ci);
  L->values = c.d_values;
  L->validity = c.d_validity;
  L->op = e.op;
  L->wide = 1;
  R->leaf_col[li] = ci;
  auto dbits = [](double d) { int64_t v; std::memcpy(&v, &d, 8); return v; };
  if (c.kind == ColKind::BOOL) {
    if (e.lit.type == FDB_LIT_BOOL) { L->kind = FDB_LEAF_CMP_I64; L->lit = e.lit.i64 ? 2 : 1; return; }
  } else if (c.kind == ColKind::I64) {
    if (e.lit.type == FDB_LIT_INT64) { L->kind = FDB_LEAF_CMP_I64; L->lit = e.lit.i64; return; }
    if (e.lit.type == FDB_LIT_FLOAT64) { L->kind = FDB_LEAF_CMP_I64_F64; L->lit = dbits(e.lit.f64); return; }
  } else if (c.kind == ColKind::U64) {
    if (e.lit.type == FDB_LIT_UINT64) { L->kind = FDB_LEAF_CMP_U64; L->lit = (int64_t)e.lit.u64; return; }
    if (e.lit.type == FDB_LIT_INT64 && e.lit.i64 >= 0) { L->kind = FDB_LEAF_CMP_U64; L->lit = e.lit.i64; return; }
  } else {
    if (e.lit.type == FDB_LIT_FLOAT64) { L->kind = FDB_LEAF_CMP_F64; L->lit = dbits(e.lit.f64); return; }
    if (e.lit.type == FDB_LIT_INT64) { L->kind = FDB_LEAF_CMP_F64; L->lit = dbits((double)e.lit.i64); return; }
  }
  throw Error(FDB_ERR_UNSUPPORTED, "unsupported binary operation (column/literal type combination) on " + c.name);
}

void GroupColState::build_ids() {
  if (ids_built_ == values.size()) return;
  ids_.reserve(values.size() * 2);
  for (; ids_built_ < values.size(); ids_built_++) ids_.emplace(values[ids_built_], (uint32_t)ids_built_ + 1);
}

uint32_t GroupColState::intern(std::string_view v) {
  build_ids();
  auto it = ids_.find(v);
  if (it != ids_.end()) return it->second;
  values.push_back(v);
  ids_.emplace(v, (uint32_t)values.size());
  ids_built_ = values.size();
  return (uint32_t)values.size();
}

std::shared_ptr<const std::vector<uint32_t>> GroupColState::lut_for(const std::shared_ptr<HostDict>& d) {
  auto range = lut_cache_.equal_range(d->hash);
  for (auto it = range.first; it != range.second; ++it)
    if (it->second.dict.get() == d.get() || it->second.dict->same_content(*d)) return it->second.lut;
  auto lut = std::make_shared<std::vector<uint32_t>>(std::max<size_t>(d->values.size(), 1), 0u);
  owners.push_back(d);
  if (values.empty() && d->unique) {
    values.reserve(d->values.size());
    for (size_t e = 0; e < d->values.size(); e++) { values.emplace_back(d->values[e]); (*lut)[e] = (uint32_t)e + 1; }
    adopted = d;
  } else {
    for (size_t e = 0; e < d->values.size(); e++) (*lut)[e] = intern(std::string_view(d->values[e]));
  }
  lut_cache_.emplace(d->hash, Cached{d, lut});
  return lut;
}

void Plan::ensure_layout(const std::vector<uint32_t>& new_caps) {
  uint64_t n_new = 1;
  std::vector<uint32_t> new_strides(new_caps.size());
  for (size_t c = 0; c < new_caps.size(); c++) {
    new_strides[c] = (uint32_t)n_new;
    n_new *= new_caps[c];
    if (n_new > (1ull << 26)) throw Error(FDB_ERR_UNSUPPORTED, "group-key space exceeds the dense table limit (2^26 slots); high-cardinality hash path not built yet");
  }
  bool remap = false;
  for (size_t c = 0; c < gcols_.size(); c++)
    if (gcols_[c].cap > 1 && gcols_[c].stride != new_strides[c]) remap = true;
  const bool need_alloc = n_new > slots_alloc_ || d_state_ == nullptr || (remap && state_dirty_);
  if (need_alloc) {
    const uint64_t cap = std::max<uint64_t>(n_new, 64);
    const uint64_t alloc = (remap && state_dirty_) ? cap : std::max<uint64_t>(cap, slots_alloc_ * 2);
    const size_t n_arrays = 1 + aggs_.size();
    unsigned long long* n_state = (unsigned long long*)ctx_->dev_alloc(alloc * 8 * n_arrays);
    mirror_valid_ = false;
    const bool carry = state_dirty_ && d_state_ != nullptr;
    if (carry) {
      unsigned long long idents[1 + FDB_MAX_AGGS];
      state_idents(idents);
      hip_check(fdb_launch_fill_state(n_state, (int64_t)alloc, (int)n_arrays, idents, stream_), "fill state");
    }
    state_virgin_ = !carry;
    if (carry) {
      const uint32_t* d_map = nullptr;
      std::vector<uint32_t> map;
      if (remap) {
        map.resize(n_slots_);
        for (uint32_t s = 0; s < n_slots_; s++) {
          uint64_t t = 0;
          for (size_t c = 0; c < gcols_.size(); c++) {
            if (gcols_[c].cap <= 1) continue;
            const uint32_t digit = (s / gcols_[c].stride) % gcols_[c].cap;
            t += (uint64_t)digit * new_strides[c];
          }
          map[s] = (uint32_t)t;
        }
        d_map = (const uint32_t*)upload(map.data(), map.size() * 4);
      }
      hip_check(fdb_launch_merge_u64(n_state, d_cnt_, d_map, n_slots_, FDB_AGG_SUM, 0, stream_), "remap cnt");
      for (size_t j = 0; j < aggs_.size(); j++) {
        const int32_t f = (aggs_[j].func == FDB_AGG_COUNT) ? FDB_AGG_SUM : aggs_[j].func;
        hip_check(fdb_launch_merge_u64(n_state + (1 + j) * alloc, aggs_[j].d_acc, d_map, n_slots_, f,
                                       aggs_[j].type == FDB_T_F64 && f == FDB_AGG_SUM, stream_), "remap acc");
      }
      hip_check(hipStreamSynchronize(stream_), "sync(remap)");
    }
    ctx_->dev_free(d_state_);
    d_state_ = n_state;
    d_cnt_ = n_state;
    for (size_t j = 0; j < aggs_.size(); j++) aggs_[j].d_acc = n_state + (1 + j) * alloc;
    slots_alloc_ = alloc;
  }
  for (size_t c = 0; c < gcols_.size(); c++) { gcols_[c].cap = new_caps[c]; gcols_[c].stride = new_strides[c]; }
  n_slots_ = (uint32_t)n_new;
}

namespace {
constexpr size_t kCoalesceMaxBytes = (size_t)8 << 20;
constexpr int64_t kFlushRows = 2 << 20;
constexpr size_t kFlushBytes = (size_t)96 << 20;
constexpr size_t kFlushRecords = 1024;
}

bool Plan::jit_possible() const { return sub_tiles != 4 && !knobs_.no_jit; }

Plan::Knobs::Knobs() {
  no_jit = std::getenv("FDB_NO_JIT") != nullptr;
  runs_always = std::getenv("FDB_RUNS_ALWAYS") != nullptr;
  runs_no_sort = std::getenv("FDB_RUNS_NO_SORT") != nullptr;
  no_uniform_fold = std::getenv("FDB_NO_UNIFORM_FOLD") != nullptr;
  no_present_ids = std::getenv("FDB_NO_PRESENT_IDS") != nullptr;
  const char* w = std::getenv("FDB_RUNS_WIDE");
  runs_wide = w != nullptr ? (w[0] == '1' ? '1' : 'm') : 0;
  const char* e = std::getenv("FDB_ORDERED_SORT_MIN");
  ordered_sort_min = e != nullptr ? std::max<long long>(0, std::atoll(e)) : 4096;
  const char* pm = std::getenv("FDB_PRESENT_IDS_MIN_BYTES");
  present_ids_min_bytes = pm != nullptr ? std::max<long long>(0, std::atoll(pm)) : (long long)32 << 20;
  const char* mk = std::getenv("FDB_TEST_MAX_KEY_BYTES");
  max_key_bytes = mk != nullptr ? std::max<long long>(1, std::atoll(mk)) : 0x7FFFFFFFll;
  const char* fs = std::getenv("FDB_FINISH_SLICE_SHIFT");
  finish_slice_shift = fs != nullptr ? std::max(6, std::min(20, std::atoi(fs))) : 20;
  const char* en = std::getenv("FDB_TEST_EXACT_NORMALIZE_ROWS");
  exact_normalize_rows = en != nullptr ? std::max<long long>(1024, std::min<long long>(std::atoll(en), (1ll << 31) - (1ll << 24))) : (1ll << 31) - (1ll << 24);
}

void Plan::push(const ArrowArray* array, const ArrowSchema* schema) {
  if (finished_) throw Error(FDB_ERR_STATE, "push after finish");
  if (aggs_.empty() && matchers_.empty()) throw Error(FDB_ERR_STATE, "filter-only plan: use fdb_plan_filter / fdb_plan_select");
  started_ = true;
  static const bool prof = std::getenv("FDB_PROFILE_PUSH") != nullptr;
  auto now = [] { return std::chrono::steady_clock::now(); };
  auto lap = [&](std::chrono::steady_clock::time_point& t, double& acc) { if (prof) { const auto n = now(); acc += std::chrono::duration<double, std::micro>(n - t).count(); t = n; } };
  std::chrono::steady_clock::time_point tp = now();
  HostRecordView view;
  view_record(array, schema, &view);
  std::function<bool(const std::string&)> want = [this](const std::string& n) { return references(n); };
  hip_check(hipSetDevice(device_), "hipSetDevice");
  lap(tp, prof_push_[0]);
  size_t payload = 0;
  for (const HostColView& c : view.cols)
    if (want(c.name)) payload += (size_t)c.length * (c.kind == ColKind::DICT ? 4 : 8) + (size_t)(c.length + 7) / 8;
  if (payload > kCoalesceMaxBytes) {
    settle();
    std::unique_ptr<DeviceBatch> b = import_batch(view, device_, &want, stream_, ctx_);
    push_batch(*b);
    sync();
    return;
  }
  const RecordSink sink = [this](size_t bytes, void** dev, unsigned char** pinned) { slab_reserve(bytes, dev, pinned); };
  std::unique_ptr<DeviceBatch> b = import_batch(view, device_, &want, stream_, ctx_, true, &sink);
  constexpr size_t kShipBytes = (size_t)2 << 20;
  if (slab_.used - slab_.shipped >= kShipBytes) slab_ship();
  lap(tp, prof_push_[1]);
  {
    Resolved R;
    std::vector<int> gc;
    resolve_batch(*b, &R, &gc);
    if (R.args.n_expr > 0 && !jit_possible())
      throw Error(FDB_ERR_UNSUPPORTED, "computed (projected) columns need the run-time specialised kernel (hiprtc unavailable or disabled)");
  }
  lap(tp, prof_push_[2]);
  pending_rows_ += b->rows;
  pending_bytes_ += b->arena_bytes;
  pending_.push_back(std::move(b));
  if (pending_rows_ >= kFlushRows || pending_bytes_ >= kFlushBytes || pending_.size() >= kFlushRecords) settle();
  lap(tp, prof_push_[3]);
  prof_push_n_++;
}

void Plan::slab_reserve(size_t bytes, void** dev, unsigned char** pinned) {
  constexpr size_t kSlabBytes = (size_t)32 << 20;
  bytes = (bytes + 255) / 256 * 256;
  if (slab_.d != nullptr && slab_.used + bytes > slab_.cap) {
    settle();
    inflight_slabs_.push_back(slab_);
    slab_ = RecordSlab();
    if (inflight_slabs_.size() >= 8) sync();
  }
  if (slab_.d == nullptr) {
    slab_.cap = std::max(kSlabBytes, bytes);
    slab_.d = ctx_->dev_alloc(slab_.cap);
    slab_.h = (unsigned char*)ctx_->host_alloc(slab_.cap);
    slab_.used = slab_.shipped = 0;
  }
  *dev = (unsigned char*)slab_.d + slab_.used;
  *pinned = slab_.h + slab_.used;
  slab_.used += bytes;
}

void Plan::slab_ship() {
  if (slab_.d == nullptr || slab_.used <= slab_.shipped) return;
  hip_check(hipMemcpyAsync((unsigned char*)slab_.d + slab_.shipped, slab_.h + slab_.shipped, slab_.used - slab_.shipped, hipMemcpyHostToDevice, stream_), "hipMemcpyAsync(record slab)");
  slab_.shipped = slab_.used;
}

void Plan::settle() {
  if (pending_.empty()) return;
  slab_ship();
  std::vector<std::unique_ptr<DeviceBatch>> batch = std::move(pending_);
  pending_.clear();
  pending_rows_ = 0;
  pending_bytes_ = 0;
  std::vector<const DeviceBatch*> ptrs;
  for (const auto& b : batch) ptrs.push_back(b.get());
  try {
    push_batches(ptrs.data(), (int)ptrs.size());
  } catch (...) {
    (void)hipStreamSynchronize(stream_);
    throw;
  }
  for (auto& b : batch) inflight_.push_back(std::move(b));
}

void Plan::push_batch(const DeviceBatch& b) {
  const DeviceBatch* p = &b;
  push_batches(&p, 1);
}

void Plan::resolve_predicate(const DeviceBatch& b, int root, Resolved* R) {
  std::memset(&R->args, 0, sizeof(R->args));
  R->args.n_rows = b.rows;
  R->truths = &truth_cache_;
  R->count_selected = [this, &b](int n) { return count_subtree(b, n); };
  int max_depth = 0;
  if (root >= 0) emit_filter(filter_, root, b, R, 0, &max_depth);
}

void Plan::resolve_batch(const DeviceBatch& b, Resolved* Rp, std::vector<int>* batch_gcols) {
  Resolved& R = *Rp;
  resolve_predicate(b, filter_root_, &R);
  FdbScanArgs& a = R.args;

  for (size_t ci = 0; ci < b.cols.size(); ci++) {
    const DevColumn& c = b.cols[ci];
    bool matched = false;
    for (const GroupMatcher& m : matchers_) if (match_group(m, c.name)) { matched = true; break; }
    if (!matched) continue;
    if (c.kind != ColKind::DICT && c.kind != ColKind::I64 && c.kind != ColKind::U64 && c.kind != ColKind::BOOL)
      throw Error(FDB_ERR_UNSUPPORTED, "group by on column type " + c.format + " (" + c.name + ") is not supported");
    if (c.d_values == nullptr) throw Error(FDB_ERR_INVALID, "column not staged: " + c.name);
    const int kind = c.kind == ColKind::DICT ? 0 : 1;
    const bool key_bool = c.kind == ColKind::BOOL, key_u64 = c.kind == ColKind::U64;
    size_t gi = 0;
    for (; gi < gcols_.size(); gi++) if (gcols_[gi].name == c.name) break;
    if (gi == gcols_.size()) {
      if (gcols_.size() >= FDB_MAX_HASH_GCOLS) throw Error(FDB_ERR_UNSUPPORTED, "more than 64 group-by columns");
      GroupColState g;
      g.name = c.name;
      g.kind = kind;
      if (kind == 0) { g.value_format = c.dict->value_format; g.plain = c.dict->plain; }
      g.is_bool = key_bool; g.is_u64 = key_u64;
      g.cap = 1;
      g.stride = 0;
      gcols_.push_back(std::move(g));
    }
    GroupColState& g = gcols_[gi];
    if (g.kind != kind || g.is_bool != key_bool || g.is_u64 != key_u64 || (kind == 0 && g.plain != c.dict->plain))
      throw Error(FDB_ERR_UNSUPPORTED, "group column " + c.name + " changed type between batches");
    GroupRes gr;
    gr.gi = (int)gi; gr.ci = (int)ci; gr.kind = kind;
    if (kind == 0) gr.lut = g.lut_for(c.dict);
    R.groups.push_back(std::move(gr));
    R.count(b, (int)ci);
    (void)batch_gcols;
  }

  for (const GroupMatcher& m : matchers_) {
    if (m.dynamic) continue;
    const Projection* P = find_projection(m.name);
    if (P == nullptr) continue;
    const int root = resolve_projection(*P, b, &R);
    if (a.expr[root].type != FDB_T_I64 && a.expr[root].type != FDB_T_BOOL && a.expr[root].type != FDB_T_U64)
      throw Error(FDB_ERR_UNSUPPORTED, "group by on a float64 expression (" + m.name + ") is not supported");
    const bool is_bool = a.expr[root].type == FDB_T_BOOL, is_u64 = a.expr[root].type == FDB_T_U64;
// ... 657 lines not shown
```

frostdb_amd/csrc/fdb_plan.h:

```cpp
#pragma once

#include <hip/hip_runtime_api.h>

#include <cstdint>
#include <functional>
#include <memory>
#include <mutex>
#include <string>
#include <string_view>
#include <unordered_map>
#include <vector>

#include "fdb_arrow.h"
#include "fdb_regex.h"
#include "fdb_kernels.h"
#include "fdb_record.h"

namespace fdb {

void hip_check(hipError_t e, const char* what);
void check_desc_shape(const fdb_plan_desc* d);

struct DeviceBatch {
  int device = 0;
// ... 127 lines not shown
  int kind = 0;
  bool is_bool = false, is_u64 = false, plain = false;
  std::string value_format = "z";
  std::vector<std::string> values;
};
struct GroupSchema { std::vector<GroupSchemaCol> cols; std::vector<int32_t> agg_types; };

struct PhaseTimer;

class Plan {
 public:
  Plan(const fdb_plan_desc* desc, int device, bool explain_only = false);
  struct CloneTag {};
  Plan(const Plan& proto, CloneTag);
  Plan(const Plan&) = delete;
  Plan& operator=(const Plan&) = delete;
  ~Plan();

  void push(const ArrowArray* array, const ArrowSchema* schema);
  void settle();
  void push_batch(const DeviceBatch& batch);
  void push_batches(const DeviceBatch* const* batches, int n);
  void finish(ArrowArray* out, ArrowSchema* out_schema, int64_t* n_rows);
  bool finish_next(ArrowArray* out, ArrowSchema* out_schema, int64_t* n_rows);
  std::vector<std::pair<std::vector<OutColumn>, int64_t>> pending_out_;
  std::unique_ptr<DeviceBatch> finish_batch(int64_t* n_rows);
  int64_t finish_columns(std::vector<OutColumn>* cols);
  size_t n_key_columns() const { return gcols_.size(); }
  void merge_from(Plan& src);
  void select(const ArrowArray* array, const ArrowSchema* schema, uint32_t* indices, int64_t capacity, int64_t* n_selected);
  void filter(const ArrowArray* array, const ArrowSchema* schema, ArrowArray* out, ArrowSchema* out_schema, int64_t* n_selected);
  std::unique_ptr<DeviceBatch> filter_batch(const DeviceBatch& in, int64_t* n_selected);
  int64_t select_batch(const DeviceBatch& in, uint32_t* d_indices, int64_t capacity);
  std::vector<std::unique_ptr<DeviceBatch>> filter_batches(const DeviceBatch* const* in, int n, int64_t* n_selected);
  std::unique_ptr<DeviceBatch> project_batch(const fdb_project_col* cols, int n_cols, const DeviceBatch& in);
  std::vector<std::unique_ptr<DeviceBatch>> project_batches(const fdb_project_col* cols, int n_cols, const DeviceBatch* const* in, int n);
  void project(const fdb_project_col* cols, int n_cols, const ArrowArray* array, const ArrowSchema* schema, ArrowArray* out, ArrowSchema* out_schema);
  const char* draw();
  int64_t num_groups();
  void partial_keys(ArrowArray* out, ArrowSchema* out_schema);
  void partial_state(int32_t agg, void* dst, int64_t capacity_bytes);
  char agg_format(int32_t agg) const;
  uint64_t state_signature(int64_t* n_slots);
  void state_read(int32_t array, void* dst, int64_t capacity_bytes);
  void state_pointers(void** base, int64_t* array_stride, int64_t* n_slots);
  void state_write(int32_t array, const void* src, int64_t bytes);
  int32_t state_array_op(int32_t array) const;
  int32_t num_state_arrays() const { return (int32_t)(1 + aggs_.size()); }
  bool has_composite_aggs() const { for (const AggState& a : aggs_) if (a.role != 0) return true; return false; }

  void group_schema(ArrowArray* out, ArrowSchema* out_schema);
  void seed_groups(const ArrowArray* array, const ArrowSchema* schema);
  void hash_export(Plan& layout, int n_parts, void** dev_rows, int64_t* counts, int32_t* row_words32);
  void hash_import(const void* dev_rows, int64_t n_rows, bool unique_rows = false);
  bool comm_allreduce(Comm& comm);
  void comm_exchange(Comm& comm, Plan& shard);
  GroupSchema export_schema() const;
  void adopt_schema(const GroupSchema& s);

  std::string error;
  int device() const { return device_; }
  hipStream_t stream() const { return stream_; }
  bool timing = false;
  int64_t stat_bytes = 0, stat_launches = 0, stat_rows = 0;
  double stat_ms = 0;
  double stat_merge_ms = 0;
  int rows_per_thread = 0;
  int grid_override = 0;
  int sub_tiles = 0;
  const char* last_kernel() const { return last_kernel_; }
  bool deterministic = false;
  bool use_partials = true;
  void set_exact_sums(bool on);
  bool exact_sums() const { return exact_; }
  bool started() const { return started_; }
  void refuse_exact(const char* what) const;
  struct Resolved;
  void sync();

 private:
  const char* last_kernel_ = "";
  bool started_ = false;
  bool exact_ = false;
  unsigned long long* d_limbs_ = nullptr;
  int n_exact_ = 0;
  int exact_q(size_t j) const;
  bool exact_f64(size_t j) const;
  uint64_t exact_adds_ = 0;
  void exact_finalize();
  void exact_normalize_now();
  unsigned long long* exact_limbs_alloc(uint64_t capacity);
  bool references(const std::string& column) const;
  TruthCache truth_cache_;
  std::vector<Projection> projs_;
  const Projection* find_projection(const std::string& name) const;
  int resolve_projection(const Projection& p, const DeviceBatch& b, Resolved* R);
  void resolve_batch(const DeviceBatch& b, Resolved* R, std::vector<int>* batch_gcols);
  void resolve_predicate(const DeviceBatch& b, int root, Resolved* R);
  void resolve_filter_only(const DeviceBatch& b, int root, Resolved* R);
  int64_t count_subtree(const DeviceBatch& b, int node);
  int64_t run_flags(const FdbScanArgs& a, uint8_t** d_masks, uint32_t** d_offsets);
  std::unique_ptr<DeviceBatch> filter_batch_interp(const DeviceBatch& in, int64_t* n_selected);
  struct SelectStall {};
  struct FilterRun;
  struct DenseLaunch;
  std::vector<std::unique_ptr<DeviceBatch>> filter_batches_impl(const DeviceBatch* const* in, int n, int64_t* n_selected, bool force_two_pass);
  template <class F> void timed(F&& launch, bool merge = false);
  void ensure_layout(const std::vector<uint32_t>& new_caps);
  void collect_timing();
  void fetch_state(std::vector<unsigned long long>* cnt, std::vector<std::vector<unsigned long long>>* acc);
  void fetch_compact(CompactState* cs);
  void build_key_columns(const CompactState& cs, std::vector<OutColumn>* cols) const;
  void build_agg_columns(const CompactState& cs, std::vector<OutColumn>* cols) const;
  void sort_compact(CompactState* cs) const;
  void switch_to_hash();
  void hash_layout();
  void hash_reserve(uint64_t extra_groups, uint64_t expected_groups = 0);
  bool push_dense(const DeviceBatch* const* bs, std::vector<Resolved>& Rs, std::vector<std::vector<int>>& part_gcols, const std::vector<int>& live, bool fixed_order, PhaseTimer& pt);
  void push_hash(const DeviceBatch* const* bs, std::vector<Resolved>& Rs, const std::vector<int>& live, bool runs = false);
  struct RunSegment {
    void* block = nullptr;
    unsigned char* tuples = nullptr; uint32_t* dir = nullptr; uint32_t* cursor = nullptr;
    int64_t n_entries = 0, capacity = 0;
    int32_t run_words = 0;
  };
  struct RunsView {
    FdbRunSegs segs;
    unsigned long long* phys = nullptr; uint32_t* flags = nullptr; uint32_t* out_idx = nullptr;
    int64_t n_runs = 0, n_groups = 0;
    const FdbRunCol* d_cols = nullptr; const uint32_t* d_rank32 = nullptr;
  };
  struct RecordSlab { void* d = nullptr; unsigned char* h = nullptr; size_t cap = 0, used = 0, shipped = 0; };
  RecordSlab slab_;
  std::vector<RecordSlab> inflight_slabs_;
  void slab_reserve(size_t bytes, void** dev, unsigned char** pinned);
  void slab_ship();
  double prof_push_[4] = {0, 0, 0, 0};
  int64_t prof_push_n_ = 0;
  std::vector<RunSegment> runs_;
  bool runs_wanted(const DeviceBatch* const* bs, const std::vector<Resolved>& Rs, const std::vector<int>& live) const;
  int runs_format(const Resolved& R) const;
  void runs_free();
  void runs_to_table();
  bool runs_prepare(RunsView* v, bool check_order, std::vector<void*>* owned);
  void runs_rank_tables(RunsView* v, std::vector<void*>* owned);
  bool runs_sort(RunsView* v, std::vector<void*>* owned);
  struct Knobs {
    bool no_jit, runs_always, runs_no_sort, no_uniform_fold, no_present_ids;
    char runs_wide;
    long long ordered_sort_min;
    long long present_ids_min_bytes;
    long long max_key_bytes;
    int finish_slice_shift;
    long long exact_normalize_rows;
    Knobs();
  } knobs_;
  int64_t fresh_groups_ = -1;
  bool ordered_finish_on_device();
  unsigned long long* sort_by_group_columns(unsigned long long* order, int64_t n_things, const FdbRunSegs* segs, const uint32_t* rows, int row_kw, RunsView* tables,
                                            std::vector<void*>* owned);
  int32_t runs_func() const;
  void hash_merge_device(const unsigned long long* d_entries, const uint32_t* d_keys, int64_t n, int in_kw, const std::vector<FdbHashCol>& cols, bool unique_source);
  void hash_merge_args(FdbHashMergeArgs* m, const std::vector<FdbHashCol>& cols, int in_stride_words);
  void merge_hash_tables(Plan& src);
  bool merge_runs(Plan& src);
  int64_t finish_columns_runs(std::vector<OutColumn>* cols, DeviceBatch* resident, bool* ok);
  void fetch_compact_hash(CompactState* cs);
  int64_t finish_columns_hash(std::vector<OutColumn>* cols, DeviceBatch* resident = nullptr, const RunsView* runs = nullptr);
  void merge_hash(Plan& src);
  uint64_t hash_groups();
  void hash_insert_entries(const std::vector<unsigned long long>& entries, const std::vector<uint32_t>& keys, int64_t n, int in_kw,
                           const std::vector<FdbHashCol>& cols);
  void* upload(const void* host, size_t bytes);

  int device_;
  hipStream_t stream_ = nullptr;
  std::vector<ExprNode> filter_;
  int32_t filter_root_ = -1;
  std::vector<AggState> aggs_;
  std::vector<GroupMatcher> matchers_;
  bool final_stage_ = false;
  bool ordered_ = false;
  bool finished_ = false;

  std::vector<GroupColState> gcols_;
  uint32_t n_slots_ = 1;
  uint64_t slots_alloc_ = 0;
  unsigned long long* d_state_ = nullptr;
  unsigned long long* d_cnt_ = nullptr;
  bool state_dirty_ = false;
  bool state_virgin_ = false;
  void materialize_state();
  unsigned long long* h_mirror_ = nullptr;
  size_t mirror_bytes_ = 0;
  bool mirror_valid_ = false;
  unsigned long long* mirror_target();
  void state_idents(unsigned long long* idents) const;
  TableMode mode_ = TableMode::DENSE;
  unsigned long long* h_table_ = nullptr;
  uint32_t* h_keys_ = nullptr;
  unsigned long long* h_count_dev_ = nullptr;
  uint64_t h_capacity_ = 0;
  int h_entry_words_ = 0, h_key_words_ = 4, h_key_used_ = 4;
  uint64_t h_groups_bound_ = 0;
  bool h_bound_stale_ = false;
  uint64_t h_rows_seen_ = 0;

  Context* ctx_ = nullptr;
  std::vector<std::pair<hipEvent_t, hipEvent_t>> pending_events_;
  std::vector<std::pair<const char*, hipEvent_t>> trace_;
  void trace(const char* what);
  std::vector<std::pair<hipEvent_t, hipEvent_t>> merge_events_;
  std::vector<void*> scratch_;
  std::vector<std::unique_ptr<DeviceBatch>> pending_;
  std::vector<std::unique_ptr<DeviceBatch>> inflight_;
  int64_t pending_rows_ = 0;
  size_t pending_bytes_ = 0;
  bool jit_possible() const;
  std::string draw_;
};

}
```

frostdb_amd/csrc/fdb_plan_internal.h:

```cpp
#pragma once

#include <algorithm>
#include <chrono>
#include <cstdio>
#include <cstdlib>
#include <cstring>
#include <exception>
#include <functional>
#include <memory>
#include <string>
#include <vector>

#include "fdb_context.h"
#include "fdb_plan.h"

namespace fdb {

bool is_leaf_op(int32_t op);

struct PhaseTimer {
  bool on;
  std::chrono::steady_clock::time_point t;
  PhaseTimer() : on(std::getenv("FDB_PROFILE") != nullptr), t(std::chrono::steady_clock::now()) {}
  void mark(const char* what) {
    if (!on) return;
    auto n = std::chrono::steady_clock::now();
    std::fprintf(stderr, "[fdb] %-20s %8.1f us\n", what, std::chrono::duration<double, std::micro>(n - t).count());
    t = n;
  }
};

inline void print_dense_launch(const char* kernel, const std::string& shape_key, const FdbScanArgs* parts, size_t n_parts, int64_t total_tiles, int grid, int block,
                               size_t lds_bytes, int two_phase, int lds_acc, int cache_slots, size_t lut_lds_max, int per_cu, int tile_rows, bool fill_rides, bool partials,
                               const std::vector<uint32_t>& folded = std::vector<uint32_t>()) {
  std::string s;
  for (size_t p = 0; p < n_parts; p++) {
    s += " " + std::to_string(parts[p].lut_class) + ":";
    const uint32_t f = p < folded.size() ? folded[p] : 0u;
    for (int k = 0; k < parts[p].n_c4; k++) s += std::to_string((int)parts[p].w4[k]) + ((f >> k) & 1u ? "n" : "");
    s += "/";
    for (int k = 0; k < parts[p].n_l4; k++) s += std::to_string((int)parts[p].wl4[k]) + ((f >> (16 + k)) & 1u ? "n" : "");
  }
  std::fprintf(stderr, "[fdb] dense launch %s shape=%s parts=%zu total_tiles=%lld grid=%d block=%d lds_bytes=%zu two_phase=%d lds_acc=%d cache_slots=%d lut_lds_max=%zu "
               "per_cu=%d tile_rows=%d fill=%d partials=%d class:w4/wl4=%s\n", kernel, shape_key.empty() ? "-" : shape_key.c_str(), n_parts, (long long)total_tiles, grid, block,
               lds_bytes, two_phase, lds_acc, cache_slots, lut_lds_max, per_cu, tile_rows, (int)fill_rides, (int)partials, s.c_str());
}

struct Blob {
  std::vector<uint8_t> bytes;
  size_t add(const void* p, size_t n) {
    const size_t off = align_up(bytes.size(), 16);
    bytes.resize(off + std::max<size_t>(n, 1), 0);
    if (n) std::memcpy(bytes.data() + off, p, n);
    return off;
  }
};

struct PendingLut { int kind; int index; size_t blob_off; size_t len_bytes; };

inline size_t place_luts(const std::vector<PendingLut>& luts, unsigned char* d_blob, size_t lds_off, FdbScanArgs* a) {
  for (const PendingLut& p : luts) {
    const bool in_lds = p.len_bytes <= 16384 && lds_off + p.len_bytes <= 32768;
    uint32_t lds = FDB_NO_LDS;
    if (in_lds) { lds = (uint32_t)lds_off; lds_off = align_up(lds_off + p.len_bytes, 16); }
    unsigned char* at = d_blob + p.blob_off;
    if (p.kind == 0) { a->leaves[p.index].lut = at; a->leaves[p.index].lut_lds = lds; }
    else { a->gcols[p.index].lut = (const uint32_t*)at; a->gcols[p.index].lut_lds = lds; }
  }
  return align_up(lds_off, 16);
}

struct StageScope {
  Context* c;
  explicit StageScope(Context* ctx) : c(ctx) { c->defer_staging(true); }
  ~StageScope() { try { c->defer_staging(false); } catch (...) {} }
};

template <class F>
void Plan::timed(F&& launch, bool merge) {
  hipEvent_t e0 = nullptr, e1 = nullptr;
  if (timing) { e0 = ctx_->get_event(); e1 = ctx_->get_event(); hip_check(hipEventRecord(e0, stream_), "hipEventRecord"); }
  launch();
  if (timing) { hip_check(hipEventRecord(e1, stream_), "hipEventRecord"); (merge ? merge_events_ : pending_events_).emplace_back(e0, e1); }
}


struct GroupRes {
  int gi, ci, kind;
  int expr_root = -1;
  std::shared_ptr<const std::vector<uint32_t>> lut;
};

struct Plan::Resolved {
  TruthCache* truths = nullptr;
  int cur_node = -1;
  FdbScanArgs args;
  Blob blob;
  std::vector<PendingLut> luts;
  std::vector<char> counted;
  int64_t bytes = 0;
  int leaf_col[FDB_MAX_LEAVES];
  int gcol_col[FDB_MAX_DENSE_GCOLS];
  int agg_col[FDB_MAX_AGGS];
  int expr_col[FDB_MAX_EXPR_NODES];
  int c4_col[FDB_ARG_C4], l4_col[FDB_ARG_L4];
  std::vector<GroupRes> groups;
  std::function<int64_t(int node)> count_selected;
  Resolved() {
    for (int& v : leaf_col) v = -1;
    for (int& v : gcol_col) v = -1;
    for (int& v : agg_col) v = -1;
    for (int& v : expr_col) v = -1;
    for (int& v : c4_col) v = -1;
    for (int& v : l4_col) v = -1;
  }
  void count(const DeviceBatch& b, int ci, bool values = true) {
    if (counted.empty()) counted.assign(b.cols.size(), 0);
    char& c = counted[(size_t)ci];
    if (values && !(c & 1)) { c |= 1; bytes += b.cols[(size_t)ci].value_bytes; }
    if (!(c & 2)) { c |= 2; bytes += b.cols[(size_t)ci].validity_bytes; }
  }
};

inline bool same_lut_set(const Plan::Resolved& q, const Plan::Resolved& r) {
  if (q.blob.bytes != r.blob.bytes || q.luts.size() != r.luts.size()) return false;
  for (size_t k = 0; k < r.luts.size(); k++)
    if (q.luts[k].kind != r.luts[k].kind || q.luts[k].index != r.luts[k].index || q.luts[k].blob_off != r.luts[k].blob_off ||
        q.luts[k].len_bytes != r.luts[k].len_bytes)
      return false;
  return true;
}

struct LutClasses {
  Blob blob;
  std::vector<size_t> blob_base;
  std::vector<int> cls;
  void add(const Plan::Resolved& R) {
    size_t found = 0;
    while (found < reps_.size() && !same_lut_set(*reps_[found].first, R)) found++;
    if (found == reps_.size()) reps_.emplace_back(&R, R.blob.bytes.empty() ? 0 : blob.add(R.blob.bytes.data(), R.blob.bytes.size()));
    blob_base.push_back(reps_[found].second);
    cls.push_back((int)found);
  }
  size_t place(size_t k, unsigned char* d_blob, Plan::Resolved& R) const {
    R.args.lut_class = cls[k];
    return place_luts(R.luts, d_blob + blob_base[k], 0, &R.args);
  }
 private:
  std::vector<std::pair<const Plan::Resolved*, size_t>> reps_;
};

int assign_slots(const DeviceBatch& b, Plan::Resolved& R, int first_layout = 1, bool relaxed = false, bool* interp_ok = nullptr);


}
```

Before: 567.1 billion rows/s.

## Pack per-record kernel args into compact part table and dedupe LUT staging

Adds a compact packed per-record parameter table, used when the JIT kernel is uniform across more than one record. The kernel reads only the varying fields of each part, made wave-uniform via readfirstlane, so it no longer loads a full FdbScanArgs struct per record. It also skips rebuilding LUT blobs for records whose LUT sources match an earlier record, and replaces a quadratic search over narrowed slots with a per-part linked list. These cut host planning and upload cost and per-tile argument loads in the kernel, at the cost of more complex generated code and a new size-capped table path.

```diff
diff --git a/frostdb_amd/csrc/fdb_dense.cpp b/frostdb_amd/csrc/fdb_dense.cpp
--- a/frostdb_amd/csrc/fdb_dense.cpp
+++ b/frostdb_amd/csrc/fdb_dense.cpp
@@ -32,8 +32,9 @@
   LdsPlan lds;
   FoldFuncs funcs;
 
-  struct Narrowed { int part, k, col; bool late; const void* wide; int64_t saved; const uint8_t* validity; bool folded; };
+  struct Narrowed { int part, k, col; bool late; const void* wide; int64_t saved; const uint8_t* validity; bool folded; size_t prev_of_part; };
   std::vector<Narrowed> narrowed;
+  std::vector<size_t> narrowed_by_part;
 
   hipFunction_t jit_fn = nullptr;
   std::string shape_key;
@@ -41,6 +42,9 @@
   bool slot_kernel = false;
   int per_cu = 1;
   int tile_rows = 0;
+  JitShape shape;
+  int ptab_words = 0;
+  std::vector<PartField> part_fields;
 
   DenseLaunch(Plan& p, const DeviceBatch* const* b, std::vector<Resolved>& rs, std::vector<std::vector<int>>& gc, const std::vector<int>& lv, bool fixed, PhaseTimer& t)
       : P(p), bs(b), Rs(rs), part_gcols(gc), live(lv), fixed_order(fixed), pt(t), jit_possible(p.jit_possible()), sub(p.sub_tiles == 4 ? 0 : p.sub_tiles) {}
@@ -63,25 +67,52 @@
 };
 
 void Plan::DenseLaunch::bind_group_columns() {
+  struct Src {
+    const void* lut; bool null_entry;
+    bool operator==(const Src& o) const { return lut == o.lut && null_entry == o.null_entry; }
+  };
+  struct First { int rec; size_t n_leaf_luts; std::vector<Src> src; };
+  std::vector<First> firsts;
+  std::vector<Src> src;
   for (int i : live) {
     Resolved& R = Rs[(size_t)i];
     FdbScanArgs& a = R.args;
+    src.clear();
+    for (const auto& p : R.lut_src) src.push_back(Src{p.get(), false});
+    auto null_entry_of = [&](const GroupRes& gr) {
+      return scan_cache_folded(*bs[i], (size_t)gr.ci) && gr.lut->size() <= bs[i]->cols[(size_t)gr.ci].dict->values.size();
+    };
+    for (const GroupRes& gr : R.groups) src.push_back(Src{gr.lut.get(), null_entry_of(gr)});
+    const First* like = nullptr;
+    for (const First& f : firsts) {
+      const Resolved& Q = Rs[(size_t)f.rec];
+      if (f.src != src || f.n_leaf_luts != R.luts.size()) continue;
+      bool same = true;
+      for (size_t k = 0; same && k < R.luts.size(); k++)
+        same = Q.luts[k].kind == R.luts[k].kind && Q.luts[k].index == R.luts[k].index && Q.luts[k].blob_off == R.luts[k].blob_off && Q.luts[k].len_bytes == R.luts[k].len_bytes;
+      if (same) { like = &f; break; }
+    }
+    if (like == nullptr) firsts.push_back(First{i, R.luts.size(), src});
     for (const GroupRes& gr : R.groups) {
       FdbGroupCol& G = a.gcols[a.n_gcols];
       const DevColumn& c = bs[i]->cols[(size_t)gr.ci];
       G.idx = (const uint32_t*)c.d_values;
       G.validity = c.d_validity;
-      const size_t null_entry = scan_cache_folded(*bs[i], (size_t)gr.ci) && gr.lut->size() <= c.dict->values.size() ? 1 : 0;
+      const size_t null_entry = null_entry_of(gr) ? 1 : 0;
       G.lut_len = (uint32_t)(gr.lut->size() + null_entry);
       G.lut_lds = FDB_NO_LDS;
       G.slot = -1;
       R.gcol_col[a.n_gcols] = gr.ci;
-      const size_t off = R.blob.add(gr.lut->data(), gr.lut->size() * 4);
-      R.blob.bytes.resize(R.blob.bytes.size() + null_entry * 4, 0);
-      R.luts.push_back(PendingLut{1, a.n_gcols, off, (gr.lut->size() + null_entry) * 4});
+      if (like == nullptr) {
+        const size_t off = R.blob.add(gr.lut->data(), gr.lut->size() * 4);
+        R.blob.bytes.resize(R.blob.bytes.size() + null_entry * 4, 0);
+        R.luts.push_back(PendingLut{1, a.n_gcols, off, (gr.lut->size() + null_entry) * 4});
+        R.lut_src.push_back(gr.lut);
+      }
       part_gcols[(size_t)i].push_back(gr.gi);
       a.n_gcols++;
     }
+    if (like != nullptr) { R.lut_like = like->rec; R.luts = Rs[(size_t)like->rec].luts; }
   }
   std::vector<uint32_t> caps;
   for (const GroupColState& g : P.gcols_) caps.push_back((uint32_t)g.values.size() + 1);
@@ -90,7 +121,13 @@
 }
 
 void Plan::DenseLaunch::stage_luts() {
-  for (int i : live) luts.add(Rs[(size_t)i]);
+  std::vector<size_t> at(Rs.size(), 0);
+  size_t n_added = 0;
+  for (int i : live) {
+    const Resolved& R = Rs[(size_t)i];
+    if (R.lut_like >= 0) luts.add_like(at[(size_t)R.lut_like]); else luts.add(R);
+    at[(size_t)i] = n_added++;
+  }
   stage_scope.emplace(P.ctx_);
   unsigned char* d_blob = luts.blob.bytes.empty() ? nullptr : (unsigned char*)P.upload(luts.blob.bytes.data(), luts.blob.bytes.size());
   size_t k = 0;
@@ -140,6 +177,7 @@
 
 void Plan::DenseLaunch::narrow_slots() {
   if (!specialisable() || !jit_possible) return;
+  narrowed_by_part.assign(Rs.size(), SIZE_MAX);
   narrow_pool(false);
   if (two_phase) narrow_pool(true);
 }
@@ -167,10 +205,11 @@
       const int ci = late ? R.l4_col[k] : R.c4_col[k];
       FdbColSlot& sl = late ? R.args.l4[k] : R.args.c4[k];
       bool counted = false;
-      for (const Narrowed& nw : narrowed) if (nw.part == i && nw.col == ci) counted = true;
+      for (size_t at = narrowed_by_part[(size_t)i]; at != SIZE_MAX; at = narrowed[at].prev_of_part) if (narrowed[at].col == ci) counted = true;
       const int64_t saved = counted ? 0 : bs[i]->rows * (int64_t)(4 - w);
       const bool fold = sl.validity != nullptr && scan_cache_folded(*bs[i], (size_t)ci) && !(!late && validity_leaf_reads(R.args, k));
-      narrowed.push_back(Narrowed{i, k, ci, late, sl.values, saved, sl.validity, fold});
+      narrowed.push_back(Narrowed{i, k, ci, late, sl.values, saved, sl.validity, fold, narrowed_by_part[(size_t)i]});
+      narrowed_by_part[(size_t)i] = narrowed.size() - 1;
       sl.values = scan_cache_get(*bs[i], (size_t)ci, P.stream_);
       if (fold) sl.validity = nullptr;
       (late ? R.args.wl4 : R.args.w4)[k] = (uint8_t)w;
@@ -192,7 +231,6 @@
 bool Plan::DenseLaunch::choose_kernel() {
   jit_block = fixed_order ? 256 : sub == 1 ? 512 : sub == 2 ? 256 : sub == 3 ? 1024 : 0;
   if (specialisable()) {
-    JitShape shape;
     bool same = true, first = true;
     const FdbScanArgs& args0 = args(live[0]);
     for (int i : live) {
@@ -207,6 +245,11 @@
     }
     shape.wave_tables = fixed_order;
     shape.uniform_fold = !P.knobs_.no_uniform_fold;
+    if (same && shape.quad && live.size() > 1) {
+      part_fields = jit_part_fields(shape);
+      const int words = jit_part_words(part_fields);
+      if (live.size() * (size_t)words * 8 <= (size_t)P.knobs_.part_table_cap) { shape.part_table = true; ptab_words = words; }
+    }
     if (same) {
       JitDeferScope defer(interp_ok && !fixed_order);
       if (jit_block != 0) { jit_fn = jit_get(shape); if (jit_fn != nullptr) per_cu = jit_blocks_per_cu(jit_fn, jit_block, lds.lds_bytes); }
@@ -215,6 +258,7 @@
       if (pt.on && jit_fn != nullptr) shape_key = shape.key(true);
     }
   }
+  if (jit_fn == nullptr) ptab_words = 0;
   if (slots_ok && jit_fn == nullptr) widen_slots();
   slot_kernel = slots_ok && (jit_fn != nullptr || interp_ok);
   if (fixed_order && jit_fn == nullptr) throw Error(FDB_ERR_UNSUPPORTED, "deterministic float sums need the run-time specialised dense kernel (records of one shape, hiprtc available)");
@@ -260,16 +304,26 @@
 
 void Plan::DenseLaunch::launch_slots() {
   int grid = P.grid_override > 0 ? P.grid_override : (fdb_scan_default_grid(P.device_) / 2) * per_cu;
+  const bool ptab = ptab_words > 0;
   std::vector<FdbScanArgs> parts;
-  parts.reserve(live.size());
-  for (int i : live) parts.push_back(args(i));
-  const int64_t total_tiles = assign_tiles(parts.data(), parts.size(), tile_rows);
+  std::vector<FdbScanArgs*> recs;
+  int64_t total_tiles = 0;
+  if (ptab) {
+    for (int i : live) recs.push_back(&args(i));
+    total_tiles = assign_tiles(recs.data(), recs.size(), tile_rows);
+  } else {
+    parts.reserve(live.size());
+    for (int i : live) parts.push_back(args(i));
+    total_tiles = assign_tiles(parts.data(), parts.size(), tile_rows);
+  }
+  const int n_parts = (int)live.size();
   if (grid > total_tiles) grid = (int)total_tiles;
   unsigned long long* partials = alloc_partials(grid);
-  for (FdbScanArgs& a : parts) a.partials = partials;
+  if (ptab) recs[0]->partials = partials;
+  else for (FdbScanArgs& a : parts) a.partials = partials;
+  FdbScanArgs& a0 = ptab ? *recs[0] : parts[0];
   bool fill_rides = false;
   if (P.state_virgin_ && jit_fn != nullptr && partials != nullptr && (uint64_t)P.slots_alloc_ * (1 + P.aggs_.size()) < (1ull << 32)) {
-    FdbScanArgs& a0 = parts[0];
     a0.fill_state = P.d_state_;
     a0.fill_words = (uint32_t)(P.slots_alloc_ * (1 + P.aggs_.size()));
     a0.fill_alloc = (uint32_t)P.slots_alloc_;
@@ -280,20 +334,29 @@
   }
   P.trace("before scan");
   pt.mark("parts build");
-  const FdbScanArgs* d_parts = (const FdbScanArgs*)P.upload(parts.data(), parts.size() * sizeof(FdbScanArgs));
+  const void* d_parts = nullptr;
+  if (ptab) {
+    std::vector<unsigned long long> table((size_t)n_parts * (size_t)ptab_words);
+    jit_pack_parts(part_fields, ptab_words, recs.data(), recs.size(), table.data());
+    d_parts = P.upload(table.data(), table.size() * 8);
+  } else {
+    d_parts = P.upload(parts.data(), parts.size() * sizeof(FdbScanArgs));
+  }
   P.ctx_->flush_staging();
   pt.mark("parts upload");
   P.trace("after upload");
   if (pt.on) {
-    std::vector<uint32_t> folded(parts.size(), 0u);
+    if (!ptab) for (FdbScanArgs& a : parts) recs.push_back(&a);
+    std::vector<uint32_t> folded(recs.size(), 0u);
     for (const Narrowed& nw : narrowed)
       if (nw.folded) folded[(size_t)(std::find(live.begin(), live.end(), nw.part) - live.begin())] |= 1u << ((nw.late ? 16 : 0) + nw.k);
-    print_dense_launch(jit_fn != nullptr ? "fdb_plan_kernel" : "scan_slots_kernel", shape_key, parts.data(), parts.size(), total_tiles, grid, jit_fn != nullptr ? jit_block : 0, lds.lds_bytes,
-                       two_phase, lds.lds_acc, lds.cache_slots, lut_lds_max, per_cu, tile_rows, fill_rides, partials != nullptr, folded);
+    print_dense_launch(jit_fn != nullptr ? "fdb_plan_kernel" : "scan_slots_kernel", shape_key, recs.data(), recs.size(), total_tiles, grid, jit_fn != nullptr ? jit_block : 0, lds.lds_bytes,
+                       two_phase, lds.lds_acc, lds.cache_slots, lut_lds_max, per_cu, tile_rows, fill_rides, partials != nullptr, folded, ptab_words);
   }
   P.timed([&] {
-    if (jit_fn != nullptr) hip_check(jit_launch(jit_fn, d_parts, (int)parts.size(), total_tiles, parts[0], grid, jit_block, lds.lds_bytes, P.stream_), "scan launch");
-    else hip_check(fdb_launch_scan_slots(d_parts, (int)parts.size(), parts[0], total_tiles, grid, lds.lds_bytes, two_phase, sub, P.stream_), "scan launch");
+    if (ptab) hip_check(jit_launch_ptab(jit_fn, (const unsigned long long*)d_parts, n_parts, total_tiles, a0, grid, jit_block, lds.lds_bytes, P.stream_), "scan launch");
+    else if (jit_fn != nullptr) hip_check(jit_launch(jit_fn, (const FdbScanArgs*)d_parts, n_parts, total_tiles, a0, grid, jit_block, lds.lds_bytes, P.stream_), "scan launch");
+    else hip_check(fdb_launch_scan_slots((const FdbScanArgs*)d_parts, n_parts, a0, total_tiles, grid, lds.lds_bytes, two_phase, sub, P.stream_), "scan launch");
   });
   if (fill_rides) P.state_virgin_ = false;
   P.last_kernel_ = jit_fn != nullptr ? "fdb_plan_kernel" : "scan_slots_kernel";
@@ -314,7 +377,8 @@
     a.n_c4 = a.n_c8 = 0;
     const int grid = fdb_scan_grid(a, lds.base_grid, rpt);
     a.partials = alloc_partials(grid);
-    if (pt.on) print_dense_launch("scan_dense_kernel", "", &a, 1, 0, grid, 0, lds.lds_bytes, 0, lds.lds_acc, lds.cache_slots, lut_lds_max, 0, rpt, false, a.partials != nullptr);
+    const FdbScanArgs* one = &a;
+    if (pt.on) print_dense_launch("scan_dense_kernel", "", &one, 1, 0, grid, 0, lds.lds_bytes, 0, lds.lds_acc, lds.cache_slots, lut_lds_max, 0, rpt, false, a.partials != nullptr);
     P.timed([&] { hip_check(fdb_launch_scan_dense(a, grid, lds.lds_bytes, rpt, P.stream_), "scan launch"); });
     P.last_kernel_ = "scan_dense_kernel";
     P.mirror_valid_ = false;
diff --git a/frostdb_amd/csrc/fdb_jit.cpp b/frostdb_amd/csrc/fdb_jit.cpp
--- a/frostdb_amd/csrc/fdb_jit.cpp
+++ b/frostdb_amd/csrc/fdb_jit.cpp
@@ -291,4 +291,11 @@
   return hipModuleLaunchKernel(fn, (unsigned)grid, 1, 1, (unsigned)block, 1, 1, (unsigned)lds_bytes, stream, args, nullptr);
 }
 
-}
+hipError_t jit_launch_ptab(hipFunction_t fn, const unsigned long long* d_ptab, int n_parts, int64_t total_tiles, const FdbScanArgs& common, int grid, int block,
+                           size_t lds_bytes, hipStream_t stream) {
+  long long tt = total_tiles;
+  void* args[] = {(void*)&d_ptab, (void*)&n_parts, (void*)&tt, (void*)&common};
+  return hipModuleLaunchKernel(fn, (unsigned)grid, 1, 1, (unsigned)block, 1, 1, (unsigned)lds_bytes, stream, args, nullptr);
+}
+
+}
diff --git a/frostdb_amd/csrc/fdb_jit.h b/frostdb_amd/csrc/fdb_jit.h
--- a/frostdb_amd/csrc/fdb_jit.h
+++ b/frostdb_amd/csrc/fdb_jit.h
@@ -32,6 +32,7 @@
   bool wave_tables = false;
   bool uniform_fold = true;
   bool quad = false;
+  bool part_table = false;
   int fuse4 = 0, fuse8 = 0;
   std::vector<int> proj_roots;
   std::string key(bool with_validity = true) const;
@@ -90,6 +91,22 @@
                               unsigned long long* d_nulls, hipStream_t stream);
 
 std::string jit_source(const JitShape& shape);
+
+struct PartField {
+  enum What { TILE_END, TILE_BEGIN, N_ROWS, SLOT_VALUES, SLOT_VALIDITY, LEAF_LIT, LEAF_LUT, LEAF_LEN, LEAF_LDS, LEAF_OP, G_LUT, G_LDS, G_STRIDE, G_LEN, EXPR_LIT, LUT_CLASS };
+  What what;
+  int pool;
+  int index;
+  int bits;
+  int word;
+  int shift;
+};
+std::vector<PartField> jit_part_fields(const JitShape& shape);
+int jit_part_words(const JitShape& shape);
+int jit_part_words(const std::vector<PartField>& fields);
+const char* jit_part_field_name(PartField::What what);
+void jit_pack_parts(const JitShape& shape, const FdbScanArgs* const* args, size_t n, unsigned long long* out);
+void jit_pack_parts(const std::vector<PartField>& fields, int W, const FdbScanArgs* const* args, size_t n, unsigned long long* out);
 class JitDeferScope {
  public:
   explicit JitDeferScope(bool may_defer);
@@ -103,5 +120,7 @@
 hipFunction_t jit_select(JitShape shape, size_t lds_bytes, int row_bytes, bool sorted_input, int* block_out, int* blocks_per_cu_out);
 hipError_t jit_launch(hipFunction_t fn, const FdbScanArgs* d_parts, int n_parts, int64_t total_tiles, const FdbScanArgs& common, int grid, int block,
                       size_t lds_bytes, hipStream_t stream);
+hipError_t jit_launch_ptab(hipFunction_t fn, const unsigned long long* d_ptab, int n_parts, int64_t total_tiles, const FdbScanArgs& common, int grid, int block,
+                           size_t lds_bytes, hipStream_t stream);
 
 }
diff --git a/frostdb_amd/csrc/fdb_jitgen.cpp b/frostdb_amd/csrc/fdb_jitgen.cpp
--- a/frostdb_amd/csrc/fdb_jitgen.cpp
+++ b/frostdb_amd/csrc/fdb_jitgen.cpp
@@ -108,6 +108,12 @@
 __device__ __forceinline__ u32x4 idx2x4(uint32_t lo, uint32_t hi) {
   u32x4 r; r.x = lo & 0xFFFFu; r.y = lo >> 16; r.z = hi & 0xFFFFu; r.w = hi >> 16;
   return r;
+}
+)HIP";
+
+const char* kPartTablePreamble = R"HIP(
+__device__ __forceinline__ unsigned long long ptw(unsigned long long v) {
+  return ((unsigned long long)(uint32_t)__builtin_amdgcn_readfirstlane((int)(uint32_t)(v >> 32)) << 32) | (unsigned long long)(uint32_t)__builtin_amdgcn_readfirstlane((int)(uint32_t)v);
 }
 )HIP";
 
@@ -358,7 +364,31 @@
     const char* var;
     int block;
     bool out_tile;
+    bool ptab = false;
   };
+  std::string part_target(const PartField& f, std::string* cast) const {
+    static const char* pools[4][2] = {{"4", "e"}, {"8", "e"}, {"4", "l"}, {"8", "l"}};
+    const std::string i = std::to_string(f.index);
+    switch (f.what) {
+      case PartField::TILE_END: *cast = "(long long)"; return "tile_end";
+      case PartField::TILE_BEGIN: *cast = "(long long)"; return "tile_begin";
+      case PartField::N_ROWS: *cast = "(long long)"; return "n_rows";
+      case PartField::SLOT_VALUES: *cast = "(const char*)"; return std::string("P_") + pools[f.pool][1] + pools[f.pool][0] + "_" + i + "_v";
+      case PartField::SLOT_VALIDITY: *cast = "(const uint8_t*)"; return std::string("P_") + pools[f.pool][1] + pools[f.pool][0] + "_" + i + "_b";
+      case PartField::LEAF_LIT: *cast = "(long long)"; return "K_lit" + i;
+      case PartField::LEAF_LUT: *cast = "(const uint8_t*)"; return "K_lut" + i;
+      case PartField::LEAF_LEN: *cast = "(uint32_t)"; return "K_len" + i;
+      case PartField::LEAF_LDS: *cast = "(uint32_t)"; return "K_lds" + i;
+      case PartField::LEAF_OP: *cast = "(int)(uint32_t)"; return "K_op" + i;
+      case PartField::G_LUT: *cast = "(const uint32_t*)"; return "G_lut" + i;
+      case PartField::G_LDS: *cast = "(uint32_t)"; return "G_lds" + i;
+      case PartField::G_STRIDE: *cast = "(uint32_t)"; return "G_stride" + i;
+      case PartField::G_LEN: *cast = "(uint32_t)"; return "G_len" + i;
+      case PartField::EXPR_LIT: *cast = "(long long)"; return "K_elit" + i;
+      case PartField::LUT_CLASS: *cast = "(int)(uint32_t)"; return "const int p_class";
+    }
+    return "";
+  }
   template <typename F> void each_slot(const Entry& e, F f) const {
     for (bool late : {false, true}) {
       if (late && !e.late_pools) break;
@@ -376,6 +406,28 @@
   }
   void enter_record(const Entry& e, const std::function<void()>& per_record = nullptr, const std::function<void()>& luts = nullptr, const std::string& leaving = "") {
     o << "    if (part < 0 || " << e.var << " >= tile_end) {\n" << leaving;
+    if (e.ptab) {
+      const std::vector<PartField> fields = jit_part_fields(s);
+      const int W = jit_part_words(fields);
+      o << "      int np = part < 0 ? 0 : part;\n      while (np + 1 < n_parts && " << e.var << " >= (long long)ptw(as_global(ptab)[(size_t)np * " << W << "])) np++;\n      part = np;\n";
+      o << "      const G1 unsigned long long* pw = as_global(ptab) + (size_t)part * " << W << ";\n";
+      for (int w = 0; w < W; w++) o << (w == 0 ? "      const unsigned long long " : ", ") << "w" << w << " = pw[" << w << "]";
+      o << ";\n";
+      for (int w = 0; w < W; w++) o << (w == 0 ? "      const unsigned long long " : ", ") << "s" << w << " = ptw(w" << w << ")";
+      o << ";\n";
+      for (const PartField& f : fields) {
+        std::string cast;
+        const std::string dst = part_target(f, &cast);
+        o << "      " << dst << " = " << cast << "(s" << f.word << (f.bits == 32 && f.shift ? " >> 32" : "") << ");\n";
+      }
+      o << "      if (p_class != lut_class) {\n        lut_class = p_class;\n        __syncthreads();\n";
+      for (size_t l = 0; l < s.leaves.size(); l++)
+        if (s.leaves[l].kind == FDB_LEAF_DICT_LUT && s.leaves[l].lut_in_lds)
+          o << "        for (uint32_t i = tid; i < K_len" << l << "; i += " << e.block << ") smem[K_lds" << l << " + i] = as_global(K_lut" << l << ")[i];\n";
+      if (luts) luts();
+      o << "        __syncthreads();\n      }\n    }\n";
+      return;
+    }
     o << "      int np = part < 0 ? 0 : part;\n      while (np + 1 < n_parts && " << e.var << " >= parts[np].tile_end) np++;\n      part = np;\n";
     o << "      const FdbScanArgs& pa = parts[part];\n      n_rows = pa.n_rows; tile_begin = pa.tile_begin; tile_end = pa.tile_end;" << (e.out_tile ? " out_tile = pa.out_tile_base;" : "") << "\n";
     each_slot(e, [&](const std::string& r, const char* pool, int i) {
@@ -395,16 +447,19 @@
 
   std::string source() {
     const int BLK = s.block;
-    const Entry entry{true, "tile", BLK, false};
+    const Entry entry{true, "tile", BLK, false, s.part_table};
     o << "#include \"fdb_kernels.h\"\n" << kPreamble;
     if (s.quad) o << kQuadPreamble;
-    o << "extern \"C\" __global__ __launch_bounds__(" << BLK << ") void fdb_plan_kernel(const FdbScanArgs* __restrict__ parts, const int n_parts, const long long total_tiles, const FdbScanArgs c) {\n";
+    if (s.part_table) o << kPartTablePreamble;
+    if (s.part_table) o << "extern \"C\" __global__ __launch_bounds__(" << BLK << ") void fdb_plan_kernel(const unsigned long long* __restrict__ ptab, const int n_parts, const long long total_tiles, const FdbScanArgs c) {\n";
+    else o << "extern \"C\" __global__ __launch_bounds__(" << BLK << ") void fdb_plan_kernel(const FdbScanArgs* __restrict__ parts, const int n_parts, const long long total_tiles, const FdbScanArgs c) {\n";
     o << "  extern __shared__ __align__(16) unsigned char smem[];\n  const uint32_t tid = threadIdx.x;\n  const uint32_t n_slots = c.n_slots;\n";
     o << "  if (c.fill_state != nullptr)  // (a fresh table: its identity fill rides on this launch, see FdbScanArgs)\n";
     o << "    for (uint32_t i = blockIdx.x * " << BLK << "u + tid; i < c.fill_words; i += gridDim.x * " << BLK << "u) c.fill_state[i] = c.fill_idents[i / c.fill_alloc];\n";
     table_setup();
     entry_decls(entry, [&] {
       for (size_t g = 0; g < s.gcols.size(); g++) o << "  uint32_t G_lds" << g << " = 0, G_stride" << g << " = 0; const uint32_t* G_lut" << g << " = nullptr;\n";
+      if (s.part_table) for (size_t g = 0; g < s.gcols.size(); g++) if (s.gcols[g].lut_in_lds) o << "  uint32_t G_len" << g << " = 0;\n";
       for (size_t i = 0; i < s.exprs.size(); i++) if (s.exprs[i].kind == 1) o << "  long long K_elit" << i << " = 0;\n";
       for (int t = 0; t < s.reg_slots; t++) {
         o << "  unsigned long long R_cnt" << t << " = 0ull;\n";
@@ -427,7 +482,7 @@
     }, [&] {
       for (size_t g = 0; g < s.gcols.size(); g++)
         if (s.gcols[g].lut_in_lds)
-          o << "        for (uint32_t i = tid; i < pa.gcols[" << g << "].lut_len; i += " << BLK << ") reinterpret_cast<uint32_t*>(smem + G_lds" << g << ")[i] = as_global(G_lut" << g << ")[i];\n";
+          o << "        for (uint32_t i = tid; i < " << (s.part_table ? "G_len" + std::to_string(g) : "pa.gcols[" + std::to_string(g) + "].lut_len") << "; i += " << BLK << ") reinterpret_cast<uint32_t*>(smem + G_lds" << g << ")[i] = as_global(G_lut" << g << ")[i];\n";
     });
     if (!s.quad) {
       tile_header("(tile - tile_begin) * " + std::to_string(BLK * 4) + "LL", "tid");
@@ -1293,7 +1348,7 @@
 
 std::string JitShape::key(bool with_validity) const {
   std::ostringstream k;
-  k << "b" << block << "l" << lds_acc << "c" << need_count << "t" << two_phase << "r" << reg_slots << "h" << cache << (wave_tables ? "w" : "") << (uniform_fold ? "u" : "") << (quad ? "q" : "") << "|";
+  k << "b" << block << "l" << lds_acc << "c" << need_count << "t" << two_phase << "r" << reg_slots << "h" << cache << (wave_tables ? "w" : "") << (uniform_fold ? "u" : "") << (quad ? "q" : "") << (part_table ? "p" : "") << "|";
   auto slots = [&](const JitSlot* p, int n) { for (int i = 0; i < n; i++) { k << (p[i].has_values ? 'v' : '-') << (with_validity ? p[i].has_validity : 0); if (p[i].width != 4) k << 'w' << p[i].width; } k << '|'; };
   slots(c4, n_c4); slots(c8, n_c8); slots(l4, n_l4); slots(l8, n_l8);
   for (const JitLeaf& L : leaves) k << L.kind << ',' << L.slot << ',' << L.wide << ',' << (L.kind >= FDB_LEAF_CMP_I64 && L.kind <= FDB_LEAF_CMP_I64_F64 ? L.op : 0) << ',' << L.lut_in_lds << ';';
@@ -1309,6 +1364,81 @@
 }
 
 std::string jit_source(const JitShape& shape) { return Gen(shape).source(); }
+
+std::vector<PartField> jit_part_fields(const JitShape& s) {
+  std::vector<PartField> f;
+  auto add = [&](PartField::What what, int bits, int pool, int index) { f.push_back(PartField{what, pool, index, bits, 0, 0}); };
+  add(PartField::TILE_END, 64, 0, 0); add(PartField::TILE_BEGIN, 64, 0, 0); add(PartField::N_ROWS, 64, 0, 0);
+  const JitSlot* pools[4] = {s.c4, s.c8, s.l4, s.l8};
+  const int counts[4] = {s.n_c4, s.n_c8, s.n_l4, s.n_l8};
+  for (int p = 0; p < 4; p++)
+    for (int i = 0; i < counts[p]; i++) {
+      if (pools[p][i].has_values) add(PartField::SLOT_VALUES, 64, p, i);
+      if (pools[p][i].has_validity != 0) add(PartField::SLOT_VALIDITY, 64, p, i);
+    }
+  for (int l = 0; l < (int)s.leaves.size(); l++) {
+    const JitLeaf& L = s.leaves[(size_t)l];
+    if (L.kind == FDB_LEAF_CONST || L.kind == FDB_LEAF_VALIDITY) add(PartField::LEAF_OP, 32, 0, l);
+    else if (L.kind == FDB_LEAF_DICT_BITS) { add(PartField::LEAF_LIT, 64, 0, l); add(PartField::LEAF_LEN, 32, 0, l); }
+    else if (L.kind == FDB_LEAF_DICT_LUT) { add(PartField::LEAF_LUT, 64, 0, l); add(PartField::LEAF_LEN, 32, 0, l); if (L.lut_in_lds) add(PartField::LEAF_LDS, 32, 0, l); }
+    else add(PartField::LEAF_LIT, 64, 0, l);
+  }
+  for (int g = 0; g < (int)s.gcols.size(); g++) {
+    add(PartField::G_LUT, 64, 0, g); add(PartField::G_STRIDE, 32, 0, g);
+    if (s.gcols[(size_t)g].lut_in_lds) { add(PartField::G_LDS, 32, 0, g); add(PartField::G_LEN, 32, 0, g); }
+  }
+  for (int i = 0; i < (int)s.exprs.size(); i++) if (s.exprs[(size_t)i].kind == 1) add(PartField::EXPR_LIT, 64, 0, i);
+  add(PartField::LUT_CLASS, 32, 0, 0);
+  int words = 0, half = -1;
+  for (PartField& x : f) {
+    if (x.bits == 64) { x.word = words++; x.shift = 0; }
+    else if (half >= 0) { x.word = half; x.shift = 32; half = -1; }
+    else { x.word = half = words++; x.shift = 0; }
+  }
+  return f;
+}
+int jit_part_words(const std::vector<PartField>& fields) {
+  int w = 0;
+  for (const PartField& x : fields) w = std::max(w, x.word + 1);
+  return w;
+}
+int jit_part_words(const JitShape& s) { return jit_part_words(jit_part_fields(s)); }
+const char* jit_part_field_name(PartField::What what) {
+  static const char* names[] = {"tile_end", "tile_begin", "n_rows", "values", "validity", "leaf.lit", "leaf.lut", "leaf.lut_len", "leaf.lut_lds", "leaf.op",
+                                "gcol.lut", "gcol.lut_lds", "gcol.stride", "gcol.lut_len", "expr.lit", "lut_class"};
+  return names[(int)what];
+}
+static unsigned long long part_field_value(const FdbScanArgs& a, const PartField& f) {
+  const FdbColSlot* pools[4] = {a.c4, a.c8, a.l4, a.l8};
+  switch (f.what) {
+    case PartField::TILE_END: return (unsigned long long)a.tile_end;
+    case PartField::TILE_BEGIN: return (unsigned long long)a.tile_begin;
+    case PartField::N_ROWS: return (unsigned long long)a.n_rows;
+    case PartField::SLOT_VALUES: return (unsigned long long)(uintptr_t)pools[f.pool][f.index].values;
+    case PartField::SLOT_VALIDITY: return (unsigned long long)(uintptr_t)pools[f.pool][f.index].validity;
+    case PartField::LEAF_LIT: return (unsigned long long)a.leaves[f.index].lit;
+    case PartField::LEAF_LUT: return (unsigned long long)(uintptr_t)a.leaves[f.index].lut;
+    case PartField::LEAF_LEN: return a.leaves[f.index].lut_len;
+    case PartField::LEAF_LDS: return a.leaves[f.index].lut_lds;
+    case PartField::LEAF_OP: return (uint32_t)a.leaves[f.index].op;
+    case PartField::G_LUT: return (unsigned long long)(uintptr_t)a.gcols[f.index].lut;
+    case PartField::G_LDS: return a.gcols[f.index].lut_lds;
+    case PartField::G_STRIDE: return a.gcols[f.index].stride;
+    case PartField::G_LEN: return a.gcols[f.index].lut_len;
+    case PartField::EXPR_LIT: return (unsigned long long)a.expr[f.index].lit;
+    case PartField::LUT_CLASS: return (uint32_t)a.lut_class;
+  }
+  return 0;
+}
+void jit_pack_parts(const JitShape& shape, const FdbScanArgs* const* args, size_t n, unsigned long long* out) {
+  const std::vector<PartField> fields = jit_part_fields(shape);
+  jit_pack_parts(fields, jit_part_words(fields), args, n, out);
+}
+void jit_pack_parts(const std::vector<PartField>& fields, int W, const FdbScanArgs* const* args, size_t n, unsigned long long* out) {
+  std::fill(out, out + n * (size_t)W, 0ull);
+  for (size_t k = 0; k < n; k++)
+    for (const PartField& f : fields) out[k * (size_t)W + (size_t)f.word] |= (f.bits == 32 ? part_field_value(*args[k], f) & 0xFFFFFFFFull : part_field_value(*args[k], f)) << f.shift;
+}
 
 JitShape jit_shape(const FdbScanArgs& a, bool two_phase, int block) {
   JitShape s;
diff --git a/frostdb_amd/csrc/fdb_launch_plan.h b/frostdb_amd/csrc/fdb_launch_plan.h
--- a/frostdb_amd/csrc/fdb_launch_plan.h
+++ b/frostdb_amd/csrc/fdb_launch_plan.h
@@ -46,6 +46,16 @@
   return total_tiles;
 }
 
+inline int64_t assign_tiles(FdbScanArgs* const* parts, size_t n, int64_t tile_rows) {
+  int64_t total_tiles = 0;
+  for (size_t k = 0; k < n; k++) {
+    parts[k]->tile_begin = total_tiles;
+    total_tiles += (parts[k]->n_rows + tile_rows - 1) / tile_rows;
+    parts[k]->tile_end = total_tiles;
+  }
+  return total_tiles;
+}
+
 struct FoldFuncs { int32_t f[1 + FDB_MAX_AGGS]; };
 inline FoldFuncs fold_funcs(const int32_t* func, const int32_t* type, size_t n_aggs) {
   FoldFuncs F = {{0}};
diff --git a/frostdb_amd/csrc/fdb_plan.cpp b/frostdb_amd/csrc/fdb_plan.cpp
--- a/frostdb_amd/csrc/fdb_plan.cpp
+++ b/frostdb_amd/csrc/fdb_plan.cpp
@@ -729,7 +729,8 @@
   return t;
 }
 
-static void emit_truth_leaf(const Truth& t, const DeviceBatch& b, int ci, Plan::Resolved* R, FdbLeaf* L) {
+static void emit_truth_leaf(const std::shared_ptr<const Truth>& tp, const DeviceBatch& b, int ci, Plan::Resolved* R, FdbLeaf* L) {
+  const Truth& t = *tp;
   const int li = (int)(L - R->args.leaves);
   const DevColumn& c = b.cols[(size_t)ci];
   L->values = c.d_values;
@@ -748,6 +749,7 @@
   L->kind = FDB_LEAF_DICT_LUT;
   const size_t off = R->blob.add(t.data(), t.size());
   R->luts.push_back(PendingLut{0, li, off, t.size()});
+  R->lut_src.push_back(tp);
 }
 
 static void emit_filter(const std::vector<ExprNode>& nodes, int idx, const DeviceBatch& b, Plan::Resolved* R, int depth, int* max_depth) {
@@ -765,7 +767,7 @@
       L.lut_lds = FDB_NO_LDS;
       L.slot = -1;
       const std::shared_ptr<HostDict>& dict = b.cols[(size_t)col].dict;
-      emit_truth_leaf(*cached_truth(R, idx, dict, [&] { return subtree_truth(nodes, idx, *dict); }), b, col, R, &L);
+      emit_truth_leaf(cached_truth(R, idx, dict, [&] { return subtree_truth(nodes, idx, *dict); }), b, col, R, &L);
       a.code[a.n_code++] = (uint8_t)li;
       return;
     }
@@ -840,7 +842,7 @@
       if (e.lit.type != FDB_LIT_STRING && e.lit.type != FDB_LIT_BINARY)
         throw Error(FDB_ERR_UNSUPPORTED, "unsupported binary operation (column/literal type combination) on " + c.name);
     }
-    emit_truth_leaf(*cached_truth(R, R->cur_node, c.dict, [&] { return leaf_truth(e, *c.dict); }), b, ci, R, L);
+    emit_truth_leaf(cached_truth(R, R->cur_node, c.dict, [&] { return leaf_truth(e, *c.dict); }), b, ci, R, L);
     return;
   }
   if (c.kind == ColKind::DICT) {
@@ -860,7 +862,7 @@
       R->count(b, ci, false);
       return;
     }
-    emit_truth_leaf(*cached_truth(R, R->cur_node, c.dict, [&] { return leaf_truth(e, *c.dict); }), b, ci, R, L);
+    emit_truth_leaf(cached_truth(R, R->cur_node, c.dict, [&] { return leaf_truth(e, *c.dict); }), b, ci, R, L);
     return;
   }
   if (is_regex) throw Error(FDB_ERR_UNSUPPORTED, "ArrayScalarRegexMatch: unsupported type on the device path: " + c.format);
@@ -1009,6 +1011,8 @@
   max_key_bytes = mk != nullptr ? std::max<long long>(1, std::atoll(mk)) : 0x7FFFFFFFll;
   const char* fs = std::getenv("FDB_FINISH_SLICE_SHIFT");
   finish_slice_shift = fs != nullptr ? std::max(6, std::min(20, std::atoi(fs))) : 20;
+  const char* pc = std::getenv("FDB_PART_TABLE_CAP");
+  part_table_cap = pc != nullptr ? std::max<long long>(0, std::min<long long>(std::atoll(pc), 16384)) : 16384;
   const char* en = std::getenv("FDB_TEST_EXACT_NORMALIZE_ROWS");
   exact_normalize_rows = en != nullptr ? std::max<long long>(1024, std::min<long long>(std::atoll(en), (1ll << 31) - (1ll << 24))) : (1ll << 31) - (1ll << 24);
 }
diff --git a/frostdb_amd/csrc/fdb_plan.h b/frostdb_amd/csrc/fdb_plan.h
--- a/frostdb_amd/csrc/fdb_plan.h
+++ b/frostdb_amd/csrc/fdb_plan.h
@@ -303,6 +303,7 @@
     long long present_ids_min_bytes;
     long long max_key_bytes;
     int finish_slice_shift;
+    long long part_table_cap;
     long long exact_normalize_rows;
     Knobs();
   } knobs_;
diff --git a/frostdb_amd/csrc/fdb_plan_internal.h b/frostdb_amd/csrc/fdb_plan_internal.h
--- a/frostdb_amd/csrc/fdb_plan_internal.h
+++ b/frostdb_amd/csrc/fdb_plan_internal.h
@@ -30,20 +30,21 @@
   }
 };
 
-inline void print_dense_launch(const char* kernel, const std::string& shape_key, const FdbScanArgs* parts, size_t n_parts, int64_t total_tiles, int grid, int block,
+inline void print_dense_launch(const char* kernel, const std::string& shape_key, const FdbScanArgs* const* parts, size_t n_parts, int64_t total_tiles, int grid, int block,
                                size_t lds_bytes, int two_phase, int lds_acc, int cache_slots, size_t lut_lds_max, int per_cu, int tile_rows, bool fill_rides, bool partials,
-                               const std::vector<uint32_t>& folded = std::vector<uint32_t>()) {
+                               const std::vector<uint32_t>& folded = std::vector<uint32_t>(), int ptab_words = 0) {
   std::string s;
   for (size_t p = 0; p < n_parts; p++) {
-    s += " " + std::to_string(parts[p].lut_class) + ":";
+    const FdbScanArgs& a = *parts[p];
+    s += " " + std::to_string(a.lut_class) + ":";
     const uint32_t f = p < folded.size() ? folded[p] : 0u;
-    for (int k = 0; k < parts[p].n_c4; k++) s += std::to_string((int)parts[p].w4[k]) + ((f >> k) & 1u ? "n" : "");
+    for (int k = 0; k < a.n_c4; k++) s += std::to_string((int)a.w4[k]) + ((f >> k) & 1u ? "n" : "");
     s += "/";
-    for (int k = 0; k < parts[p].n_l4; k++) s += std::to_string((int)parts[p].wl4[k]) + ((f >> (16 + k)) & 1u ? "n" : "");
+    for (int k = 0; k < a.n_l4; k++) s += std::to_string((int)a.wl4[k]) + ((f >> (16 + k)) & 1u ? "n" : "");
   }
   std::fprintf(stderr, "[fdb] dense launch %s shape=%s parts=%zu total_tiles=%lld grid=%d block=%d lds_bytes=%zu two_phase=%d lds_acc=%d cache_slots=%d lut_lds_max=%zu "
-               "per_cu=%d tile_rows=%d fill=%d partials=%d class:w4/wl4=%s\n", kernel, shape_key.empty() ? "-" : shape_key.c_str(), n_parts, (long long)total_tiles, grid, block,
-               lds_bytes, two_phase, lds_acc, cache_slots, lut_lds_max, per_cu, tile_rows, (int)fill_rides, (int)partials, s.c_str());
+               "per_cu=%d tile_rows=%d fill=%d partials=%d ptab=%d class:w4/wl4=%s\n", kernel, shape_key.empty() ? "-" : shape_key.c_str(), n_parts, (long long)total_tiles, grid, block,
+               lds_bytes, two_phase, lds_acc, cache_slots, lut_lds_max, per_cu, tile_rows, (int)fill_rides, (int)partials, ptab_words, s.c_str());
 }
 
 struct Blob {
@@ -97,6 +98,8 @@
   FdbScanArgs args;
   Blob blob;
   std::vector<PendingLut> luts;
+  std::vector<std::shared_ptr<const void>> lut_src;
+  int lut_like = -1;
   std::vector<char> counted;
   int64_t bytes = 0;
   int leaf_col[FDB_MAX_LEAVES];
@@ -135,6 +138,7 @@
   Blob blob;
   std::vector<size_t> blob_base;
   std::vector<int> cls;
+  void add_like(size_t like) { blob_base.push_back(blob_base[like]); cls.push_back(cls[like]); }
   void add(const Plan::Resolved& R) {
     size_t found = 0;
     while (found < reps_.size() && !same_lut_set(*reps_[found].first, R)) found++;
```

Result: faster. 578.9 billion rows/s (median of 6 runs) (+2.1%).
